# mindspore-lab/minddiffusion

Hardware: AMD Instinct MI355X
Metric: 512x512 txt2img latents/sec (50-step DDIM) (higher is better)
Workload: dtype f16; 1 GPU; SDv2 txt2img 512x512 (64x64 latent), 50-step DDIM, CFG 9.0, batch 1 per GPU (BASELINE.json configs[1]); synthetic seeded weights + synthetic text conditioning; global_batch=1, parallelism=batch-shard x1, hip_graph=True, rccl_world_size=1, broadcast_bytes=0, ddim_steps=50, unet_batch_per_gpu=2, sampler=ddim, cfg_dup_prefix=False

## Files before the change

include/mdx.h:

```cpp
#ifndef MDX_H_
#define MDX_H_

#include <stddef.h>
#include <stdint.h>

#ifdef __cplusplus
extern "C" {
#endif

#define MDX_OK 0
#define MDX_E_INVALID (-1)
#define MDX_E_WORKSPACE (-2)
#define MDX_E_HIP (-3)

typedef void* mdx_stream_t;

int mdx_version(void);
const char* mdx_last_error(void);
int mdx_set_option(const char* name, int value);
int mdx_get_option(const char* name, int* value);

int mdx_nchw_to_nhwc_f16(const float* x, void* y, int B, int C, int H, int W, int Cpad, mdx_stream_t s);
int mdx_nhwc_to_nchw_f32(const void* x, float* y, int B, int C, int H, int W, int Cstride, mdx_stream_t s);

int mdx_srgan_conv_in_f16(const float* x, const void* w, const float* bias, const float* slope, void* out, int B, int H, int W,
                          mdx_stream_t s);
int mdx_srgan_conv_out_f32(const void* x, const void* w, const float* bias, float* out, int B, int H, int W, mdx_stream_t s);

size_t mdx_groupnorm_ws_floats(int B, int HW, int C, int groups);
int mdx_groupnorm_f16(const void* x1, int C1, const void* x2, int C2, const float* gamma, const float* beta,
                      void* y, int B, int HW, int groups, float eps, int silu, float* ws, mdx_stream_t s);

int mdx_groupnorm_colstats_f16(const void* x1, int C1, const float* cs1, int nrb1, const void* x2, int C2, const float* cs2,
                               int nrb2, const float* gamma, const float* beta, const float* scale, const float* shift,
                               int mod_ld, void* y, int B, int HW, int groups, float eps, int silu, mdx_stream_t s);

int mdx_colstats_fold_f32(const float* src, int nrb, float* dst, int nrb2, int B, int C, mdx_stream_t s);

int mdx_groupnorm_scaleshift_f16(const void* x1, int C1, const void* x2, int C2, const float* gamma,
                                 const float* beta, const float* scale, const float* shift, int mod_ld, void* y,
                                 int B, int HW, int groups, float eps, int silu, float* ws, mdx_stream_t s);

int mdx_layernorm_f16(const void* x, const float* gamma, const float* beta, void* y, int rows, int C, float eps,
                      mdx_stream_t s);

typedef struct mdx_gemm_desc {
    const void* a;
    const void* a2;
    int c1, c2;
    const void* w;
    const float* bias;
    const float* rowbias;
    int rowbias_ld;
    const void* residual;
    int residual_ld;
    void* out;
    int out_ld;
    int B, H, W;
    int N;
    int ksize;
    int stride;
    int upsample;
    int epilogue;
    int out_mode;
    int splitk;
    void* workspace;
    size_t workspace_bytes;
    long out_bs;
    void* out2;
    int out2_ld;
    int n_split;
    int asym_pad;
    float* stats_out;
    const float* ln_stats;
    const float* ln_s;
    int ln_nt;
    float ln_eps;
    float* colstats_out;
    int colstats_cap;
    int defer_reduce;
    int tile_m;
    int tile_n;
    const float* gn_colstats;
    const float* gn_gamma;
    const float* gn_beta;
    int gn_nrb;
    int gn_silu;
    float gn_eps;
    const void* skip_a;
    const void* skip_a2;
    int skip_c1, skip_c2;
    const void* skip_w;
    int w_frag;
    int stages;
    const void* w_sub;
    const void* xattn_k;
    const void* xattn_vt;
    int xattn_len;
    int xattn_cap;
    float xattn_scale;
    const float* act_slope;
    int act_slope_n;
} mdx_gemm_desc;

#define MDX_GEMM_WS_HEAD 16384
#define MDX_EPI_NONE 0
#define MDX_EPI_GEGLU 1
#define MDX_EPI_GELU 2
#define MDX_EPI_QUICKGELU 3
#define MDX_EPI_PRELU 4
#define MDX_OUT_ROWMAJOR 0
#define MDX_OUT_TRANSPOSED 1
#define MDX_OUT_D2S2 2

int mdx_gemm_f16(const mdx_gemm_desc* d, mdx_stream_t s);
int mdx_gemm_release_counters(void);
int mdx_gemm_release_workspace(const void* workspace);
int mdx_gemm_bind_counters(const void* workspace, void* counters);
size_t mdx_gemm_workspace_bytes(const mdx_gemm_desc* d);
int mdx_gemm_check(const mdx_gemm_desc* d);
int mdx_gemm_query(const mdx_gemm_desc* d, int* out7);
int mdx_gemm_tune(const mdx_gemm_desc* d, mdx_stream_t s, void* flush, size_t flush_bytes, int reps, int* best4, float* us2);

int mdx_groupnorm_from_splitk_f16(const mdx_gemm_desc* prod, const float* gamma, const float* beta, void* y, int groups,
                                  float eps, int silu, mdx_stream_t s);
int mdx_groupnorm_from_splitk_ok(const mdx_gemm_desc* prod, int groups);

int mdx_attention_f16(const void* q, long q_bs, int q_ld, const void* k, long k_bs, int k_ld, const void* vt,
                      long vt_bs, int vt_ld, void* o, long o_bs, int o_ld, int B, int heads, int D, int Nq, int Nk,
                      float scale, mdx_stream_t s);

size_t mdx_attention_ws_bytes(int B, int heads, int D, int Nq, int Nk);
int mdx_attention_splitkv_f16(const void* q, long q_bs, int q_ld, const void* k, long k_bs, int k_ld, const void* vt,
                              long vt_bs, int vt_ld, void* o, long o_bs, int o_ld, int B, int heads, int D, int Nq, int Nk,
                              float scale, int kv_splits, void* ws, size_t ws_bytes, mdx_stream_t s);

typedef struct mdx_st_tail_desc {
    const void* attn_out;
    const void* tok;
    const void* x_in;
    void* out;
    const void* ctx_k;
    const void* ctx_vt;
    const void* wstream;
    const float* vec;
    float* colstats_out;
    void* debug_out;
    int debug_stage;
    int B, tokens;
    int C, heads, dim_head;
    int ctx_len, ctx_cap;
    float scale;
    float ln_eps;
    int tile_rows;
    int warm;
} mdx_st_tail_desc;
#define MDX_ST_DEBUG_COUNT_BARRIERS 100
int mdx_st_tail_sched_barriers(int C, int tile_rows);
int mdx_st_head_sched_barriers(int C, int tile_rows);
int mdx_st_tail_f16(const mdx_st_tail_desc* d, mdx_stream_t s);
int mdx_st_tail_supported(int C, int heads, int dim_head, int tokens_per_sample, int tile_rows);
size_t mdx_st_tail_stream_bytes(int C);

typedef struct mdx_st_head_desc {
    const void* x;
    const float* colstats;
    int nrb;
    const void* wstream;
    const float* vec;
    void* tok;
    void* qk;
    void* vt;
    int vt_ld;
    void* debug_out;
    int debug_stage;
    int B, tokens, C;
    float gn_eps, ln_eps;
    int tile_rows;
    int warm;
} mdx_st_head_desc;
int mdx_st_head_f16(const mdx_st_head_desc* d, mdx_stream_t s);
int mdx_st_head_supported(int C, int tokens_per_sample, int tile_rows);
size_t mdx_st_head_stream_bytes(int C);

int mdx_timestep_embedding_f32(const float* t, float* out, int M, int dim, float max_period, mdx_stream_t s);

int mdx_dense_small_f32(const float* x, int x_ld, const void* w, const float* b, float* out, int out_ld, int M,
                        int N, int K, int act_in, int act_out, mdx_stream_t s);

int mdx_sampler_step_f32(const float* x, const void* eps_u, const void* eps_c, int eps_ld, float cfg_scale,
                         const float* old1, const float* old2, const float* old3, const float* coef4,
                         float sqrt_at, float sqrt_one_minus_at, float sqrt_a_prev, float dir_coef, float sigma,
                         const float* noise, float* e_t_out, float* x_prev, float* pred_x0, int B, int C, int H,
                         int W, mdx_stream_t s);

int mdx_avgpool2x2_f16(const void* x, void* y, int B, int H, int W, int C, mdx_stream_t s);
int mdx_upsample_nearest2x_f16(const void* x, void* y, int B, int H, int W, int C, mdx_stream_t s);
int mdx_glide_text_embed_f16(const int* tokens, const int* mask, const void* tok_emb, const void* pos,
                             const void* pad, void* out, int B, int T, int width, int n_vocab, mdx_stream_t s);
int mdx_glide_superres_input_f16(const float* x, const float* low, void* out, int B, int S, int s_low,
                                 mdx_stream_t s);
int mdx_glide_step_f32(const float* x, const void* out_c, const void* out_u, int ld, float guidance_scale,
                       const float* coef8, int mode, float noise_scale, const float* noise, float* x_next,
                       float* pred_x0, int B, int H, int W, mdx_stream_t s);

typedef struct mdx_glide_kv_slot {
    const void* src;
    void* dst;
    long src_entry_bytes;
    long dst_batch_bytes;
    long src_pitch, dst_pitch;
    int rows, row_bytes;
} mdx_glide_kv_slot;
int mdx_glide_kv_select_f16(const mdx_glide_kv_slot* slots_dev, int nslots, long entry0, int entry_per_b, int b0, int nb,
                            int blocks_per_copy, mdx_stream_t s);

int mdx_attention_causal_f16(const void* q, long q_bs, int q_ld, const void* k, long k_bs, int k_ld, const void* vt,
                             long vt_bs, int vt_ld, void* o, long o_bs, int o_ld, int B, int heads, int D, int Nq,
                             int Nk, float scale, mdx_stream_t s);

int mdx_pack_b_operand_f16(const void* src, long src_ld, int rows, int K, void* dst, mdx_stream_t s);
int mdx_softmax_rows_f16(void* x, long ld, int rows, int cols, float scale, mdx_stream_t s);

int mdx_vae_gaussian_sample_f32(const void* moments, int ld, const float* noise, float* out, int B, int zc, int HW,
                                mdx_stream_t s);

int mdx_probe_mfma_32x32x16_f16(const void* a, const void* b, float* c, mdx_stream_t s);
int mdx_probe_mfma_16x16x32_f16(const void* a, const void* b, float* c, mdx_stream_t s);
int mdx_probe_dma_stream(const void* src, size_t bytes_per_block, int nblocks, int waves, int per, int ns, int mode,
                         int stride_tiles, float* sink, mdx_stream_t s);

int mdx_probe_l2_stream(const void* src, size_t total_bytes, unsigned bytes_per_wave, int nblocks, int waves, int pf,
                        int shared, float* sink, mdx_stream_t s);

int mdx_probe_gemm_trace(void* buf, size_t bytes);
int mdx_probe_valu_rate(int kind, int iters, int nblocks, float* sink, mdx_stream_t s);
int mdx_probe_mix_rate(int kind, int iters, int nblocks, float* sink, mdx_stream_t s);

#ifdef __cplusplus
}
#endif
#endif
```

minddiffusion_amd/_lib.py:

```python
import ctypes
import os

_HERE = os.path.dirname(os.path.abspath(__file__))
LIB_PATH = os.environ.get("MDX_LIBRARY") or os.path.join(_HERE, "libmdx.so")

c_void_p = ctypes.c_void_p
c_int = ctypes.c_int
c_long = ctypes.c_long
c_float = ctypes.c_float
c_size_t = ctypes.c_size_t


class MdxError(RuntimeError):
    pass


class GemmDesc(ctypes.Structure):
    _fields_ = [
        ("a", c_void_p), ("a2", c_void_p), ("c1", c_int), ("c2", c_int),
        ("w", c_void_p), ("bias", c_void_p), ("rowbias", c_void_p), ("rowbias_ld", c_int),
        ("residual", c_void_p), ("residual_ld", c_int),
        ("out", c_void_p), ("out_ld", c_int),
        ("B", c_int), ("H", c_int), ("W", c_int), ("N", c_int),
        ("ksize", c_int), ("stride", c_int), ("upsample", c_int),
        ("epilogue", c_int), ("out_mode", c_int), ("splitk", c_int),
        ("workspace", c_void_p), ("workspace_bytes", c_size_t),
        ("out_bs", c_long),
        ("out2", c_void_p), ("out2_ld", c_int), ("n_split", c_int), ("asym_pad", c_int),
        ("stats_out", c_void_p), ("ln_stats", c_void_p), ("ln_s", c_void_p), ("ln_nt", c_int), ("ln_eps", c_float),
        ("colstats_out", c_void_p), ("colstats_cap", c_int), ("defer_reduce", c_int),
        ("tile_m", c_int), ("tile_n", c_int),
        ("gn_colstats", c_void_p), ("gn_gamma", c_void_p), ("gn_beta", c_void_p), ("gn_nrb", c_int), ("gn_silu", c_int),
        ("gn_eps", c_float),
        ("skip_a", c_void_p), ("skip_a2", c_void_p), ("skip_c1", c_int), ("skip_c2", c_int), ("skip_w", c_void_p),
        ("w_frag", c_int), ("stages", c_int), ("w_sub", c_void_p),
        ("xattn_k", c_void_p), ("xattn_vt", c_void_p), ("xattn_len", c_int), ("xattn_cap", c_int), ("xattn_scale", c_float),
        ("act_slope", c_void_p), ("act_slope_n", c_int),
    ]


class StTailDesc(ctypes.Structure):
    _fields_ = [
        ("attn_out", c_void_p), ("tok", c_void_p), ("x_in", c_void_p), ("out", c_void_p),
        ("ctx_k", c_void_p), ("ctx_vt", c_void_p), ("wstream", c_void_p), ("vec", c_void_p),
        ("colstats_out", c_void_p), ("debug_out", c_void_p), ("debug_stage", c_int),
        ("B", c_int), ("tokens", c_int), ("C", c_int), ("heads", c_int), ("dim_head", c_int),
        ("ctx_len", c_int), ("ctx_cap", c_int), ("scale", c_float), ("ln_eps", c_float), ("tile_rows", c_int), ("warm", c_int),
    ]


class StHeadDesc(ctypes.Structure):
    _fields_ = [
        ("x", c_void_p), ("colstats", c_void_p), ("nrb", c_int), ("wstream", c_void_p), ("vec", c_void_p),
        ("tok", c_void_p), ("qk", c_void_p), ("vt", c_void_p), ("vt_ld", c_int), ("debug_out", c_void_p), ("debug_stage", c_int),
        ("B", c_int), ("tokens", c_int), ("C", c_int), ("gn_eps", c_float), ("ln_eps", c_float), ("tile_rows", c_int),
        ("warm", c_int),
    ]


EPI_NONE, EPI_GEGLU, EPI_GELU, EPI_QUICKGELU, EPI_PRELU = 0, 1, 2, 3, 4
OUT_ROWMAJOR, OUT_TRANSPOSED, OUT_D2S2 = 0, 1, 2

SIGNATURES = {
    "mdx_version": (c_int, []),
    "mdx_last_error": (ctypes.c_char_p, []),
    "mdx_set_option": (c_int, [ctypes.c_char_p, c_int]),
    "mdx_get_option": (c_int, [ctypes.c_char_p, ctypes.POINTER(c_int)]),
    "mdx_nchw_to_nhwc_f16": (c_int, [c_void_p, c_void_p, c_int, c_int, c_int, c_int, c_int, c_void_p]),
    "mdx_nhwc_to_nchw_f32": (c_int, [c_void_p, c_void_p, c_int, c_int, c_int, c_int, c_int, c_void_p]),
    "mdx_groupnorm_ws_floats": (c_size_t, [c_int, c_int, c_int, c_int]),
    "mdx_groupnorm_f16": (c_int, [c_void_p, c_int, c_void_p, c_int, c_void_p, c_void_p, c_void_p, c_int, c_int,
                                  c_int, c_float, c_int, c_void_p, c_void_p]),
    "mdx_groupnorm_colstats_f16": (c_int, [c_void_p, c_int, c_void_p, c_int, c_void_p, c_int, c_void_p, c_int, c_void_p,
                                           c_void_p, c_void_p, c_void_p, c_int, c_void_p, c_int, c_int, c_int, c_float,
                                           c_int, c_void_p]),
    "mdx_colstats_fold_f32": (c_int, [c_void_p, c_int, c_void_p, c_int, c_int, c_int, c_void_p]),
    "mdx_groupnorm_from_splitk_f16": (c_int, [ctypes.POINTER(GemmDesc), c_void_p, c_void_p, c_void_p, c_int, c_float, c_int,
                                              c_void_p]),
    "mdx_groupnorm_from_splitk_ok": (c_int, [ctypes.POINTER(GemmDesc), c_int]),
    "mdx_groupnorm_scaleshift_f16": (c_int, [c_void_p, c_int, c_void_p, c_int, c_void_p, c_void_p, c_void_p, c_void_p,
                                             c_int, c_void_p, c_int, c_int, c_int, c_float, c_int, c_void_p, c_void_p]),
    "mdx_layernorm_f16": (c_int, [c_void_p, c_void_p, c_void_p, c_void_p, c_int, c_int, c_float, c_void_p]),
    "mdx_gemm_f16": (c_int, [ctypes.POINTER(GemmDesc), c_void_p]),
    "mdx_gemm_workspace_bytes": (c_size_t, [ctypes.POINTER(GemmDesc)]),
    "mdx_gemm_release_workspace": (c_int, [c_void_p]),
    "mdx_gemm_bind_counters": (c_int, [c_void_p, c_void_p]),
    "mdx_st_tail_sched_barriers": (c_int, [c_int, c_int]),
    "mdx_st_head_sched_barriers": (c_int, [c_int, c_int]),
    "mdx_gemm_release_counters": (c_int, []),
    "mdx_gemm_tune": (c_int, [ctypes.POINTER(GemmDesc), c_void_p, c_void_p, c_size_t, c_int, ctypes.POINTER(c_int),
                              ctypes.POINTER(ctypes.c_float)]),
    "mdx_gemm_check": (c_int, [ctypes.POINTER(GemmDesc)]),
    "mdx_gemm_query": (c_int, [ctypes.POINTER(GemmDesc), ctypes.POINTER(c_int)]),
    "mdx_attention_f16": (c_int, [c_void_p, c_long, c_int, c_void_p, c_long, c_int, c_void_p, c_long, c_int,
                                  c_void_p, c_long, c_int, c_int, c_int, c_int, c_int, c_int, c_float, c_void_p]),
    "mdx_attention_ws_bytes": (c_size_t, [c_int, c_int, c_int, c_int, c_int]),
    "mdx_attention_splitkv_f16": (c_int, [c_void_p, c_long, c_int, c_void_p, c_long, c_int, c_void_p, c_long, c_int,
                                          c_void_p, c_long, c_int, c_int, c_int, c_int, c_int, c_int, c_float, c_int, c_void_p,
                                          c_size_t, c_void_p]),
    "mdx_attention_causal_f16": (c_int, [c_void_p, c_long, c_int, c_void_p, c_long, c_int, c_void_p, c_long, c_int,
                                  c_void_p, c_long, c_int, c_int, c_int, c_int, c_int, c_int, c_float, c_void_p]),
    "mdx_st_head_f16": (c_int, [ctypes.POINTER(StHeadDesc), c_void_p]),
    "mdx_st_head_supported": (c_int, [c_int, c_int, c_int]),
    "mdx_st_head_stream_bytes": (c_size_t, [c_int]),
    "mdx_st_tail_f16": (c_int, [ctypes.POINTER(StTailDesc), c_void_p]),
    "mdx_st_tail_supported": (c_int, [c_int, c_int, c_int, c_int, c_int]),
    "mdx_st_tail_stream_bytes": (c_size_t, [c_int]),
    "mdx_timestep_embedding_f32": (c_int, [c_void_p, c_void_p, c_int, c_int, c_float, c_void_p]),
    "mdx_dense_small_f32": (c_int, [c_void_p, c_int, c_void_p, c_void_p, c_void_p, c_int, c_int, c_int, c_int,
                                    c_int, c_int, c_void_p]),
    "mdx_sampler_step_f32": (c_int, [c_void_p, c_void_p, c_void_p, c_int, c_float, c_void_p, c_void_p, c_void_p,
                                     c_void_p, c_float, c_float, c_float, c_float, c_float, c_void_p, c_void_p,
                                     c_void_p, c_void_p, c_int, c_int, c_int, c_int, c_void_p]),
    "mdx_avgpool2x2_f16": (c_int, [c_void_p, c_void_p, c_int, c_int, c_int, c_int, c_void_p]),
    "mdx_upsample_nearest2x_f16": (c_int, [c_void_p, c_void_p, c_int, c_int, c_int, c_int, c_void_p]),
    "mdx_glide_text_embed_f16": (c_int, [c_void_p, c_void_p, c_void_p, c_void_p, c_void_p, c_void_p, c_int, c_int,
                                         c_int, c_int, c_void_p]),
    "mdx_glide_superres_input_f16": (c_int, [c_void_p, c_void_p, c_void_p, c_int, c_int, c_int, c_void_p]),
    "mdx_glide_step_f32": (c_int, [c_void_p, c_void_p, c_void_p, c_int, c_float, c_void_p, c_int, c_float, c_void_p,
                                   c_void_p, c_void_p, c_int, c_int, c_int, c_void_p]),
    "mdx_glide_kv_select_f16": (c_int, [c_void_p, c_int, c_long, c_int, c_int, c_int, c_int, c_void_p]),
    "mdx_pack_b_operand_f16": (c_int, [c_void_p, c_long, c_int, c_int, c_void_p, c_void_p]),
    "mdx_srgan_conv_in_f16": (c_int, [c_void_p, c_void_p, c_void_p, c_void_p, c_void_p, c_int, c_int, c_int, c_void_p]),
    "mdx_srgan_conv_out_f32": (c_int, [c_void_p, c_void_p, c_void_p, c_void_p, c_int, c_int, c_int, c_void_p]),
    "mdx_vae_gaussian_sample_f32": (c_int, [c_void_p, c_int, c_void_p, c_void_p, c_int, c_int, c_int, c_void_p]),
    "mdx_softmax_rows_f16": (c_int, [c_void_p, c_long, c_int, c_int, c_float, c_void_p]),
    "mdx_probe_mfma_32x32x16_f16": (c_int, [c_void_p, c_void_p, c_void_p, c_void_p]),
    "mdx_probe_mfma_16x16x32_f16": (c_int, [c_void_p, c_void_p, c_void_p, c_void_p]),
    "mdx_probe_gemm_trace": (c_int, [c_void_p, c_size_t]),
    "mdx_probe_valu_rate": (c_int, [c_int, c_int, c_int, c_void_p, c_void_p]),
    "mdx_probe_mix_rate": (c_int, [c_int, c_int, c_int, c_void_p, c_void_p]),
    "mdx_probe_l2_stream": (c_int, [c_void_p, c_size_t, ctypes.c_uint, c_int, c_int, c_int, c_int, c_void_p, c_void_p]),
    "mdx_probe_dma_stream": (c_int, [c_void_p, c_size_t, c_int, c_int, c_int, c_int, c_int, c_int, c_void_p, c_void_p]),
}

_lib = None
_ENV_OPTIONS = {
    "MDX_GEMM_TUNED": ("gemm_tuned", int), "MDX_GEMM_BM": ("gemm_bm", int), "MDX_GEMM_BN": ("gemm_bn", int),
    "MDX_GEMM_CFG": ("gemm_ring", lambda v: int(v.split(",")[-1])), "MDX_GEMM_HALO": ("gemm_halo", int),
    "MDX_GEMM_HALO8": ("gemm_halo8", int), "MDX_GEMM_SPLITK_FIXUP_MAX": ("gemm_splitk_fixup_max", int),
    "MDX_GEMM_SPREAD": ("gemm_spread", int), "MDX_HALO_NSB": ("halo_nsb", int), "MDX_GN_MIN_BLOCKS": ("gn_min_blocks", int),
    "MDX_GN_FUSED": ("gn_fused", int), "MDX_GN_COL_CHUNKS": ("gn_col_chunks", int),
    "MDX_GEMM_CONV8P": ("gemm_conv8p", int), "MDX_GEMM_CONV8P_MIN_M": ("gemm_conv8p_min_m", int),
    "MDX_GEMM_SUBPIXEL_MIN_TILES": ("gemm_subpixel_min_tiles", int), "MDX_GEMM_CONV8P_VAR": ("gemm_conv8p_var", int),
    "MDX_ATTN8": ("attn8", int), "MDX_ATTN8_MIN_BLOCKS": ("attn8_min_blocks", int),
    "MDX_GN_WIDE_ROWS": ("gn_wide_rows", int), "MDX_GN_BOOST_MB": ("gn_boost_mb", int), "MDX_ATTN_OCC3": ("attn_occ3", int), "MDX_ATTN_KV_SPLIT": ("attn_kv_split", int),
    "MDX_ATTN_FAST_STAGE": ("attn_fast_stage", int), "MDX_GN_PREFETCH": ("gn_prefetch", int), "MDX_GEMM_LN_PREFETCH": ("gemm_ln_prefetch", int),
    "MDX_GEMM_DENSE_ISSUE": ("gemm_dense_issue", int), "MDX_GEMM_LEAN_DENSE": ("gemm_lean_dense", int),
    "MDX_ATTN_PIPE": ("attn_pipe", int),
}


def load():
    global _lib
    if _lib is not None:
        return _lib
    if not os.path.exists(LIB_PATH):
        raise MdxError(
            f"{LIB_PATH} not found: the HIP extension is required (no CPU fallback). "
            "Build it with `python -c 'import __graft_entry__ as g; g.build()'` or `make -C minddiffusion_amd/csrc`.")
    import torch
    lib = ctypes.CDLL(LIB_PATH)
    for name, (res, args) in SIGNATURES.items():
        fn = getattr(lib, name)
        fn.restype = res
        fn.argtypes = args
    for env, (name, conv) in _ENV_OPTIONS.items():
        if env in os.environ:
            rc = lib.mdx_set_option(name.encode(), conv(os.environ[env]))
            if rc != 0:
                raise MdxError(f"{env}: {lib.mdx_last_error().decode()}")
    _lib = lib
    return lib


def check(rc, what):
    if rc != 0:
        msg = load().mdx_last_error()
        raise MdxError(f"{what} failed (rc={rc}): {msg.decode() if msg else ''}")
```

minddiffusion_amd/csrc/gemm.hip:

```cpp
#include "mdx_common.h"
#include "gemm_internal.h"

#ifndef MDX_HALO_ABLATE
#define MDX_HALO_ABLATE 0
#endif
#ifndef MDX_HALO_LEAN_EPI
#define MDX_HALO_LEAN_EPI 1
#endif
constexpr int HALO_EMODE = MDX_HALO_LEAN_EPI ? 2 : 0;

#include <stdlib.h>

#include <algorithm>
#include <type_traits>
#include <map>
#include <mutex>
#include <utility>
#include <vector>

namespace {


template <int BM, int BN, int BK, int NS, bool SWAP, bool FASTK, int NW, bool GNA = false, bool EXT = false>
__global__ __launch_bounds__(NW * 64, NW == 4 ? 2 : 1) void gemm_kernel(const GemmParams p) {
// ... 674 lines not shown
#pragma unroll
                for (int i = 0; i < TM; ++i) { f16x8 tt; asm volatile("" : "=v"(tt)); af[slot][i] = tt; }
#pragma unroll
                for (int j = 0; j < TN; ++j) { f16x8 tt; asm volatile("" : "=v"(tt)); bf[slot][j] = tt; }
#else
#pragma unroll
                for (int i = 0; i < TM; ++i)
                    af[slot][i] = *reinterpret_cast<const f16x8*>(smem + a_row[i] + (((2 * ks + hi) << 4) ^ a_key[i]));
#pragma unroll
                for (int j = 0; j < TN; ++j)
                    bf[slot][j] = *reinterpret_cast<const f16x8*>(sb + b_row_off + j * 32 * 128 + (((2 * ks + hi) ^ swz_b) << 4));
#endif
            };
            auto mfmas = [&](auto slot_c) {
                constexpr int slot = decltype(slot_c)::value;
#if MDX_HALO_ABLATE == 1
#pragma unroll
                for (int i = 0; i < TM; ++i) { const f16x8 tt = af[slot][i]; asm volatile("" ::"v"(tt)); }
#pragma unroll
                for (int j = 0; j < TN; ++j) { const f16x8 tt = bf[slot][j]; asm volatile("" ::"v"(tt)); }
#else
#pragma unroll
                for (int i = 0; i < TM; ++i)
#pragma unroll
                    for (int j = 0; j < TN; ++j) {
                        if constexpr (SWAP)
                            acc[i][j] = __builtin_amdgcn_mfma_f32_32x32x16_f16(bf[slot][j], af[slot][i], acc[i][j], 0, 0, 0);
                        else
                            acc[i][j] = __builtin_amdgcn_mfma_f32_32x32x16_f16(af[slot][i], bf[slot][j], acc[i][j], 0, 0, 0);
                    }
#endif
            };
            using I0 = std::integral_constant<int, 0>;
            using I1 = std::integral_constant<int, 1>;
            if constexpr (ALLK) {
                using I2 = std::integral_constant<int, 2>;
                using I3 = std::integral_constant<int, 3>;
                rdfrag(I0{}, 0); rdfrag(I1{}, 1); rdfrag(I2{}, 2); rdfrag(I3{}, 3);
                __builtin_amdgcn_sched_barrier(0);
                mfmas(I0{}); mfmas(I1{}); mfmas(I2{}); mfmas(I3{});
            } else {
                rdfrag(I0{}, 0);
                __builtin_amdgcn_sched_barrier(0);
#pragma unroll
                for (int ks = 0; ks < 4; ks += 2) {
                    rdfrag(I1{}, ks + 1);
                    __builtin_amdgcn_sched_barrier(0);
                    mfmas(I0{});
                    __builtin_amdgcn_sched_barrier(0);
                    if (ks + 2 < 4) {
                        rdfrag(I0{}, ks + 2);
                        __builtin_amdgcn_sched_barrier(0);
                    }
                    mfmas(I1{});
                    __builtin_amdgcn_sched_barrier(0);
                }
            }
            rd = (rd + 1 == NSB) ? 0 : rd + 1;
            wr = (wr + 1 == NSB) ? 0 : wr + 1;
        }
    }

    if (p.skip_w) {
        constexpr int SA_BYTES = BM * 128;
        static_assert(2 * SA_BYTES <= 2 * HALO_BYTES && NSB >= 2, "skip tiles reuse the halo / ring areas");
        const __amdgpu_buffer_rsrc_t rs_s1 = make_rsrc(p.skip_a, p.skip_a_bytes);
        const __amdgpu_buffer_rsrc_t rs_s2 = make_rsrc(p.skip_a2 ? p.skip_a2 : p.skip_a, p.skip_a2 ? p.skip_a2_bytes : p.skip_a_bytes);
        const __amdgpu_buffer_rsrc_t rs_sw = make_rsrc(p.skip_w, p.skip_w_bytes);
        const int sk_begin = split * p.skip_kt_per_split, sk_end = min(p.skip_kt, sk_begin + p.skip_kt_per_split);
        constexpr int SAJ = BM / 8 / NW;
        int s_pix[SAJ];
        unsigned s_cb[SAJ];
#pragma unroll
        for (int j = 0; j < SAJ; ++j) {
            const int row = (wave * SAJ + j) * 8 + lrow;
            int pix;
            if constexpr (PW == 16) {
                pix = (pb * p.H + py0 + (row >> 4)) * p.W + px0 + (row & 15);
            } else {
                pix = tile_m * BM + row;
                if (pix >= p.M) pix = -1;
            }
            s_pix[j] = pix;
            s_cb[j] = (unsigned)((lchk ^ ((row >> 1) & 7)) * 16);
        }
        unsigned sb_off[BJ];
        const int skt64 = p.skip_kt;
#pragma unroll
        for (int j = 0; j < BJ; ++j) {
            const int row = (wave * BJ + j) * 8 + lrow;
            const int panel = (n0 >> 6) + (row >> 6);
            sb_off[j] = (unsigned)(((size_t)panel * skt64) * 8192 + ((row & 63) * 8 + lchk) * 16);
        }
        auto stage_skip = [&](int kt, int st) {
            int ci0 = kt * 64;
            const bool second = ci0 >= p.skip_c1;
            const int cs2 = (second ? p.skip_c2 : p.skip_c1) * 2;
            if (second) ci0 -= p.skip_c1;
#pragma unroll
            for (int j = 0; j < SAJ; ++j) {
                const unsigned off = s_pix[j] >= 0 ? (unsigned)(s_pix[j] * cs2) + (unsigned)(ci0 * 2) + s_cb[j] : MDX_OOB;
                void* dst = smem + st * SA_BYTES + (wave * SAJ + j) * 1024;
                if (second)
                    dma16(rs_s2, dst, off);
                else
                    dma16(rs_s1, dst, off);
            }
#pragma unroll
            for (int j = 0; j < BJ; ++j)
                dma16(rs_sw, smem + 2 * HALO_BYTES + st * B_BYTES + (wave * BJ + j) * 1024, sb_off[j] + (unsigned)kt * 8192);
        };
        __syncthreads();
        const int sa_row_off = (wm * WROWS + l31) * 128;
        const int s_swz = (l31 >> 1) & 7;
        if (sk_begin < sk_end) stage_skip(sk_begin, 0);
        for (int kt = sk_begin; kt < sk_end; ++kt) {
            const int st = (kt - sk_begin) & 1;
            asm volatile("s_waitcnt vmcnt(0)" ::: "memory");
            __builtin_amdgcn_s_barrier();
            if (kt + 1 < sk_end) stage_skip(kt + 1, st ^ 1);
            const char* sa = smem + st * SA_BYTES;
            const char* sbk = smem + 2 * HALO_BYTES + st * B_BYTES;
#pragma unroll
            for (int s4 = 0; s4 < 4; ++s4) {
                f16x8 af[TM], bf[TN];
#pragma unroll
                for (int i = 0; i < TM; ++i)
                    af[i] = *reinterpret_cast<const f16x8*>(sa + sa_row_off + i * 32 * 128 + (((2 * s4 + hi) ^ s_swz) << 4));
#pragma unroll
                for (int j = 0; j < TN; ++j)
                    bf[j] = *reinterpret_cast<const f16x8*>(sbk + (b_row_off - 2 * HALO_BYTES) + j * 32 * 128 + (((2 * s4 + hi) ^ swz_b) << 4));
#pragma unroll
                for (int i = 0; i < TM; ++i)
#pragma unroll
                    for (int j = 0; j < TN; ++j) {
                        if constexpr (SWAP)
                            acc[i][j] = __builtin_amdgcn_mfma_f32_32x32x16_f16(bf[j], af[i], acc[i][j], 0, 0, 0);
                        else
                            acc[i][j] = __builtin_amdgcn_mfma_f32_32x32x16_f16(af[i], bf[j], acc[i][j], 0, 0, 0);
                    }
            }
        }
    }

    __syncthreads();
    trace_mark(p, 3);
    if constexpr (PW == 16)
        gemm_epilogue<BM, BN, SWAP, NW, PatchRows, 0, HALO_EMODE>(p, acc, smem, PatchRows{(pb * p.H + py0) * p.W + px0, p.W, pb}, n0, split, bpre,
                                                                  tile_m, tile_id);
    else
        gemm_epilogue<BM, BN, SWAP, NW>(p, acc, smem, LinearRows{tile_m * BM}, n0, split, bpre, tile_m, tile_id);
    trace_mark(p, 4);
    }
}

__device__ __forceinline__ void splitk_sum8(const GemmParams& p, const float* base, const size_t slab, float (&f)[8]) {
    int z = 0;
    for (; z + 4 <= p.nsplit; z += 4) {
        float4 v[4][2];
#pragma unroll
        for (int u = 0; u < 4; ++u) {
            const float4* s = reinterpret_cast<const float4*>(base + (size_t)(z + u) * slab);
            v[u][0] = s[0];
            v[u][1] = s[1];
        }
#pragma unroll
        for (int u = 0; u < 4; ++u) {
            f[0] += v[u][0].x; f[1] += v[u][0].y; f[2] += v[u][0].z; f[3] += v[u][0].w;
            f[4] += v[u][1].x; f[5] += v[u][1].y; f[6] += v[u][1].z; f[7] += v[u][1].w;
        }
    }
    for (; z < p.nsplit; ++z) {
        const float4* s = reinterpret_cast<const float4*>(base + (size_t)z * slab);
        const float4 s0 = s[0], s1 = s[1];
        f[0] += s0.x; f[1] += s0.y; f[2] += s0.z; f[3] += s0.w; f[4] += s1.x; f[5] += s1.y; f[6] += s1.z; f[7] += s1.w;
    }
}

template <bool EXT = false>
__global__ __launch_bounds__(256) void splitk_reduce_kernel(const GemmParams p) {
    mdx_kernarg_touch<sizeof(GemmParams)>();
    const bool geglu = p.epilogue == MDX_EPI_GEGLU;
    const int ncols = geglu ? p.N / 2 : p.N;
    const int cpr = ncols / 8;
    const size_t total = (size_t)p.M * cpr;
    const size_t slab = (size_t)p.M * p.N;
    for (size_t idx = (size_t)blockIdx.x * 256 + threadIdx.x; idx < total; idx += (size_t)gridDim.x * 256) {
        const int m = (int)(idx / cpr);
        const int oc = (int)(idx - (size_t)m * cpr) * 8;
        Row8Extras xtra;
        if (p.out_mode != MDX_OUT_TRANSPOSED) xtra = epilogue_prefetch_row8(p, m, oc);
        const bool ln = p.ln_stats != nullptr;
        float mean = 0.f, rstd = 1.f;
        if (ln) {
            const float2* stp = reinterpret_cast<const float2*>(p.ln_stats) + (size_t)m * p.ln_nt;
            float su = 0.f, sq = 0.f;
            for (int j = threadIdx.x & 7; j < p.ln_nt; j += 8) {
                const float2 v = stp[j];
                su += v.x;
                sq += v.y;
            }
#pragma unroll
            for (int off = 4; off >= 1; off >>= 1) {
                su += __shfl_xor(su, off, 64);
                sq += __shfl_xor(sq, off, 64);
            }
            const float inv = 1.0f / (float)p.K;
            mean = su * inv;
            float var = sq * inv - mean * mean;
            var = var < 0.f ? 0.f : var;
            rstd = rsqrtf(var + p.ln_eps);
        }
        float f[8];
        if (geglu) {
            const int pa = (oc >> 6) * 128 + (oc & 63);
            float a[8], g[8];
#pragma unroll
            for (int e = 0; e < 8; ++e) {
                a[e] = (p.bias && !ln) ? p.bias[pa + e] : 0.f;
                g[e] = (p.bias && !ln) ? p.bias[pa + 64 + e] : 0.f;
            }
            splitk_sum8(p, p.ws + (size_t)m * p.N + pa, slab, a);
            splitk_sum8(p, p.ws + (size_t)m * p.N + pa + 64, slab, g);
            if (ln) {
#pragma unroll
                for (int e = 0; e < 8; ++e) {
                    a[e] = rstd * (a[e] - mean * p.ln_s[pa + e]) + (p.bias ? p.bias[pa + e] : 0.f);
                    g[e] = rstd * (g[e] - mean * p.ln_s[pa + 64 + e]) + (p.bias ? p.bias[pa + 64 + e] : 0.f);
                }
            }
#pragma unroll
            for (int e = 0; e < 8; ++e) f[e] = a[e] * gelu_tanh_f(g[e]);
        } else {
#pragma unroll
            for (int e = 0; e < 8; ++e) f[e] = (p.bias && !ln) ? p.bias[oc + e] : 0.f;
            splitk_sum8(p, p.ws + (size_t)m * p.N + oc, slab, f);
            if (ln) {
#pragma unroll
                for (int e = 0; e < 8; ++e) f[e] = rstd * (f[e] - mean * p.ln_s[oc + e]) + (p.bias ? p.bias[oc + e] : 0.f);
            }
            if (p.epilogue == MDX_EPI_GELU) {
#pragma unroll
                for (int e = 0; e < 8; ++e) f[e] = gelu_tanh_f(f[e]);
            } else if (p.epilogue == MDX_EPI_QUICKGELU) {
#pragma unroll
                for (int e = 0; e < 8; ++e) f[e] = quick_gelu_f(f[e]);
            } else if constexpr (EXT) {
                if (p.epilogue == MDX_EPI_PRELU) {
                    const float* sp = p.act_slope + oc % p.act_slope_n;
#pragma unroll
                    for (int e = 0; e < 8; ++e) f[e] = f[e] > 0.f ? f[e] : sp[e] * f[e];
                }
            }
        }
        if (p.out_mode == MDX_OUT_TRANSPOSED) {
            const int b = m / p.HoWo;
            const int tok = m - b * p.HoWo;
#pragma unroll
            for (int e = 0; e < 8; ++e) p.out[((size_t)b * p.N + oc + e) * p.out_ld + tok] = (f16)f[e];
        } else if (p.n_split && oc >= p.n_split) {
            const int b = m / p.HoWo;
            const int tok = m - b * p.HoWo;
            const int nv = p.N - p.n_split;
#pragma unroll
            for (int e = 0; e < 8; ++e) p.out2[((size_t)b * nv + (oc - p.n_split + e)) * p.out2_ld + tok] = (f16)f[e];
        } else {
            const f16x8 o = epilogue_apply_row8<EXT>(p, f, m, oc, xtra);
            if (p.stats_out) {
                float su = 0.f, sq = 0.f;
#pragma unroll
                for (int e = 0; e < 8; ++e) {
                    const float t = (float)o[e];
                    su += t;
                    sq += t * t;
                }
#pragma unroll
                for (int off = 4; off >= 1; off >>= 1) {
                    su += __shfl_xor(su, off, 64);
                    sq += __shfl_xor(sq, off, 64);
                }
                if ((threadIdx.x & 7) == 0)
                    reinterpret_cast<float2*>(p.stats_out)[(size_t)m * (p.N >> 6) + (oc >> 6)] = make_float2(su, sq);
            }
        }
    }
}

constexpr int CS_ROWS = 64;

__global__ __launch_bounds__(256) void splitk_reduce_colstats_kernel(const GemmParams p) {
    mdx_kernarg_touch<sizeof(GemmParams)>();
    __shared__ float part[32][64][2];
    const int tid = threadIdx.x;
    const int chunk = tid & 7, rl = tid >> 3;
    const int rb = blockIdx.y, n = blockIdx.x * 64 + chunk * 8;
    const size_t slab = (size_t)p.M * p.N;
    float cs[8], cq[8];
#pragma unroll
    for (int e = 0; e < 8; ++e) cs[e] = cq[e] = 0.f;
    if (n < p.N) {
#pragma unroll
        for (int h = 0; h < 2; ++h) {
            const int m = rb * CS_ROWS + rl + 32 * h;
            if (m >= p.M) continue;
            const Row8Extras xtra = epilogue_prefetch_row8(p, m, n);
            float f[8];
// ... 52 lines not shown
    p.bn_hint = d->tile_n;
    p.st_hint = d->stages;
    p.out2_ld = d->out2_ld;
    p.n_split = d->n_split;
    p.ws = (float*)d->workspace;
    p.c1 = d->c1;
    p.c2 = d->c2;
    p.cin = d->c1 + d->c2;
    p.rowbias_ld = d->rowbias_ld;
    p.residual_ld = d->residual_ld;
    p.out_ld = d->out_ld;
    p.out_bs = d->out_bs;
    p.B = d->B;
    p.H = d->H;
    p.W = d->W;
    p.ksize = d->ksize;
    p.stride = d->stride;
    p.upsample = d->upsample ? 1 : 0;
    MDX_REQUIRE(!d->asym_pad || (d->ksize == 3 && d->stride == 2 && !d->upsample),
                "mdx_gemm_f16: asym_pad applies to the 3x3 stride-2 conv only");
    p.pad = d->ksize == 3 ? (d->asym_pad ? 0 : 1) : 0;
    const int pad_hi = d->ksize == 3 ? 1 : 0;
    const int Hs = p.upsample ? 2 * d->H : d->H, Ws = p.upsample ? 2 * d->W : d->W;
    p.Ho = (Hs + p.pad + pad_hi - d->ksize) / d->stride + 1;
    p.Wo = (Ws + p.pad + pad_hi - d->ksize) / d->stride + 1;
    p.HoWo = p.Ho * p.Wo;
    p.M = d->B * p.HoWo;
    p.N = d->N;
    p.K = d->ksize * d->ksize * p.cin;
    p.epilogue = d->epilogue;
    p.out_mode = d->out_mode;
    MDX_REQUIRE(p.epilogue == MDX_EPI_NONE || p.epilogue == MDX_EPI_GEGLU || p.epilogue == MDX_EPI_GELU ||
                    p.epilogue == MDX_EPI_QUICKGELU || p.epilogue == MDX_EPI_PRELU, "mdx_gemm_f16: bad epilogue");
    MDX_REQUIRE(p.out_mode == MDX_OUT_ROWMAJOR || p.out_mode == MDX_OUT_TRANSPOSED || p.out_mode == MDX_OUT_D2S2,
                "mdx_gemm_f16: bad out_mode");
    p.act_slope = d->act_slope;
    p.act_slope_n = d->act_slope_n;
    p.d2s_c = 0;
    if (p.epilogue == MDX_EPI_PRELU) {
        MDX_REQUIRE(p.act_slope && p.act_slope_n > 0 && p.act_slope_n % 8 == 0 && p.N % p.act_slope_n == 0,
                    "mdx_gemm_f16: PReLU needs act_slope and act_slope_n > 0 with act_slope_n %% 8 == 0 and N %% act_slope_n == 0");
        MDX_REQUIRE(p.out_mode != MDX_OUT_TRANSPOSED && !d->rowbias && !d->n_split && !d->xattn_k,
                    "mdx_gemm_f16: PReLU takes a row-major or depth-to-space store with bias (and residual) only");
    }
    if (p.epilogue == MDX_EPI_PRELU || p.out_mode == MDX_OUT_D2S2) {
        MDX_REQUIRE(d->c2 == 0 && d->c1 % 64 == 0 && !d->gn_colstats && !d->skip_w && !d->w_frag && !d->upsample,
                    "mdx_gemm_f16: PReLU / depth-to-space launches take one source with Cin %% 64 == 0 (no fused GroupNorm / skip, "
                    "tile-major weights, no upsample)");
    }
    if (p.out_mode == MDX_OUT_D2S2) {
        MDX_REQUIRE(p.N % 32 == 0 && p.out_ld >= p.N / 4 && (p.epilogue == MDX_EPI_NONE || p.epilogue == MDX_EPI_PRELU),
                    "mdx_gemm_f16: depth-to-space store needs N = 4 C with C %% 8 == 0, out_ld >= C and a plain or PReLU epilogue");
        MDX_REQUIRE(!d->residual && !d->out_bs && !d->n_split && !d->stats_out && !d->colstats_out && !d->ln_stats && !d->xattn_k &&
                        !d->skip_w && !d->defer_reduce,
                    "mdx_gemm_f16: depth-to-space store takes bias / time-embedding row / PReLU only");
        p.d2s_c = p.N / 4;
        p.out_mode = MDX_OUT_ROWMAJOR;
    }
    if (p.epilogue == MDX_EPI_GEGLU) {
        MDX_REQUIRE(p.N % 128 == 0, "mdx_gemm_f16: GEGLU needs N %% 128 == 0");
        MDX_REQUIRE(p.out_mode == MDX_OUT_ROWMAJOR, "mdx_gemm_f16: GEGLU is row-major only");
    }
    if (p.out_mode == MDX_OUT_TRANSPOSED) {
        MDX_REQUIRE(p.out_ld % 8 == 0 && p.out_ld >= p.HoWo, "mdx_gemm_f16: transposed store needs out_ld %% 8 == 0 and out_ld >= tokens");
        MDX_REQUIRE(!p.rowbias && !p.residual, "mdx_gemm_f16: transposed store takes bias only");
    }
    if (p.n_split) {
        MDX_REQUIRE(p.out2 && p.n_split > 0 && p.n_split < p.N && p.n_split % 128 == 0,
                    "mdx_gemm_f16: n_split must be a multiple of 128 inside (0, N) with out2 set");
        MDX_REQUIRE(p.out_mode == MDX_OUT_ROWMAJOR && p.epilogue == MDX_EPI_NONE && !p.rowbias && !p.residual,
                    "mdx_gemm_f16: the split row-major | transposed output takes bias only");
        MDX_REQUIRE(p.out2_ld % 8 == 0 && p.out2_ld >= p.HoWo,
                    "mdx_gemm_f16: transposed part needs out2_ld %% 8 == 0 and out2_ld >= tokens");
    }
    if (p.ln_stats) {
        MDX_REQUIRE(p.ln_s && p.ln_nt * 64 == p.K && p.ksize == 1 && p.c2 == 0 && p.stride == 1 && !p.upsample &&
                        p.out_mode == MDX_OUT_ROWMAJOR && p.N % (p.epilogue == MDX_EPI_GEGLU ? 128 : 64) == 0,
                    "mdx_gemm_f16: LayerNorm fold needs ln_s, ln_nt == K / 64, N %% 64 == 0 and a dense row-major GEMM");
    }
    if (p.stats_out)
        MDX_REQUIRE(p.out_mode == MDX_OUT_ROWMAJOR && p.epilogue != MDX_EPI_GEGLU && !p.n_split && p.N % 64 == 0,
                    "mdx_gemm_f16: row statistics are produced by plain row-major stores with N %% 64 == 0 only");
    if (p.colstats_out)
        MDX_REQUIRE(p.out_mode == MDX_OUT_ROWMAJOR && p.epilogue == MDX_EPI_NONE && !p.n_split && !p.ln_stats && !p.stats_out &&
                        !p.out_bs && p.N % 8 == 0,
                    "mdx_gemm_f16: column statistics come from plain row-major launches only");
    p.gn_cs = d->gn_colstats;
    p.gn_gamma = d->gn_gamma;
    p.gn_beta = d->gn_beta;
    p.gn_nrb = d->gn_nrb;
    p.gn_silu = d->gn_silu ? 1 : 0;
    p.gn_eps = d->gn_eps;
    if (p.gn_cs) {
        MDX_REQUIRE(p.gn_gamma && p.gn_beta && p.gn_nrb > 0, "mdx_gemm_f16: gn_colstats needs gn_gamma, gn_beta and gn_nrb > 0");
        if (p.ksize == 1) {
            MDX_REQUIRE(p.stride == 1 && !p.upsample && p.c2 == 0 && p.cin % 64 == 0 && p.cin <= 2560 && !p.gn_silu &&
                            p.HoWo % 64 == 0,
                        "mdx_gemm_f16: the fused input GroupNorm of a dense launch needs a single source, Cin %% 64 == 0, "
                        "Cin <= 2560, gn_silu = 0 and tokens per sample %% 64 == 0");
        } else {
            MDX_REQUIRE(p.ksize == 3 && p.stride == 1 && !p.upsample && p.c2 == 0 && p.cin % 64 == 0 && p.cin % 32 == 0 &&
                            p.cin <= 640 && !d->w_frag && !(d->H == 8 && d->W == 8),
                        "mdx_gemm_f16: the fused input GroupNorm rides on a single-source 3x3 stride-1 conv with Cin %% 64 == 0, "
                        "Cin <= 640, images larger than 8 x 8 and tile-major weights");
        }
    }
    p.xa_k = (const f16*)d->xattn_k;
    p.xa_vt = (const f16*)d->xattn_vt;
    p.xa_len = d->xattn_len;
    p.xa_cap = d->xattn_cap;
    p.xa_scale_log2 = d->xattn_scale * 1.4426950408889634f;
    if (p.xa_k) {
        const int howo = d->H * d->W;
        MDX_REQUIRE(p.xa_vt && d->xattn_len > 0 && d->xattn_len <= 128 && d->xattn_cap >= d->xattn_len && d->xattn_cap % 8 == 0,
                    "mdx_gemm_f16: cross-attention epilogue needs xattn_vt, 0 < xattn_len <= 128 <= ... xattn_cap (a multiple of 8)");
        MDX_REQUIRE(d->ksize == 1 && d->stride == 1 && !d->upsample && d->c2 == 0 && d->N % 64 == 0 && d->c1 % 64 == 0 &&
                        d->epilogue == MDX_EPI_NONE && d->out_mode == MDX_OUT_ROWMAJOR && !d->residual && !d->rowbias && !d->stats_out &&
                        !d->colstats_out && !d->n_split && !d->out_bs && !d->gn_colstats && !d->defer_reduce,
                    "mdx_gemm_f16: the cross-attention epilogue rides on a plain dense row-major projection (N %% 64 == 0, Cin %% 64 == 0)");
        MDX_REQUIRE(d->tile_n == 64 && d->splitk == 1 && (howo % 128 == 0 || (howo % 64 == 0 && d->tile_m == 64)) &&
                        (d->tile_m == 0 || d->tile_m == 64 || d->tile_m == 128),
                    "mdx_gemm_f16: the cross-attention epilogue needs tile_n = 64 (one head per tile), splitk = 1 and an M tile inside one sample "
                    "(tokens per sample %% 128 == 0, or %% 64 == 0 with tile_m = 64)");
        MDX_REQUIRE((size_t)d->xattn_cap * d->N * 2 <= 0x80000000ull, "mdx_gemm_f16: cross-attention context larger than 2 GiB per sample");
    }
    p.w_sub = (const f16*)d->w_sub;
    p.w_sub_bytes = 0;
    p.c8_sub = 0;
    if (p.w_sub) {
        MDX_REQUIRE(d->upsample && d->ksize == 3 && d->stride == 1, "mdx_gemm_f16: w_sub belongs to the nearest-2x + 3x3 conv (upsample = 1)");
        const size_t sb = (size_t)((4 * (size_t)d->N + 63) / 64) * ((4 * (size_t)(d->c1 + d->c2) + 63) / 64) * 8192;
        MDX_REQUIRE(sb <= 0x80000000ull, "mdx_gemm_f16: sub-pixel weights larger than 2 GiB");
        p.w_sub_bytes = (unsigned)sb;
    }
    p.skip_a = (const f16*)d->skip_a;
    p.skip_a2 = (const f16*)d->skip_a2;
    p.skip_w = (const f16*)d->skip_w;
    p.skip_c1 = d->skip_c1;
    p.skip_c2 = d->skip_c2;
    if (p.skip_w) {
        MDX_REQUIRE(p.skip_a && d->skip_c1 > 0 && d->skip_c1 % 64 == 0 && d->skip_c2 >= 0 && d->skip_c2 % 64 == 0 &&
                        (d->skip_c2 == 0) == (d->skip_a2 == nullptr),
                    "mdx_gemm_f16: fused skip needs skip_a, skip_c1 %% 64 == 0, skip_c2 %% 64 == 0 and skip_a2 iff skip_c2");
        MDX_REQUIRE(p.ksize == 3 && p.stride == 1 && !p.upsample && p.c2 == 0 && p.out_mode == MDX_OUT_ROWMAJOR && !d->w_frag,
                    "mdx_gemm_f16: the fused skip rides on a single-source 3x3 stride-1 row-major conv (tile-major weights)");
        p.skip_kt = (d->skip_c1 + d->skip_c2) / 64;
        const size_t s1 = (size_t)d->B * d->H * d->W * d->skip_c1 * 2, s2 = (size_t)d->B * d->H * d->W * d->skip_c2 * 2;
        const size_t sw = (size_t)((p.N + 63) / 64) * p.skip_kt * 8192;
        MDX_REQUIRE(s1 <= 0x80000000ull && s2 <= 0x80000000ull && sw <= 0x80000000ull, "mdx_gemm_f16: skip operand larger than 2 GiB");
        p.skip_a_bytes = (unsigned)s1;
        p.skip_a2_bytes = (unsigned)s2;
        p.skip_w_bytes = (unsigned)sw;
    }
    if (p.rowbias) MDX_REQUIRE(p.rowbias_ld % 4 == 0, "mdx_gemm_f16: rowbias_ld must be a multiple of 4");
    if (p.residual) MDX_REQUIRE(p.residual_ld % 8 == 0, "mdx_gemm_f16: residual_ld must be a multiple of 8");
    MDX_REQUIRE(p.out_ld % 8 == 0 && p.out_bs % 8 == 0 && p.out_bs >= 0, "mdx_gemm_f16: out_ld / out_bs must be multiples of 8");
    MDX_REQUIRE(!(p.out_bs && p.out_mode == MDX_OUT_TRANSPOSED), "mdx_gemm_f16: out_bs applies to row-major output only");
    const size_t ab = (size_t)d->B * d->H * d->W * d->c1 * 2, a2b = (size_t)d->B * d->H * d->W * d->c2 * 2;
    p.kt64 = (p.K + 63) / 64;
    const size_t wb = (size_t)((p.N + 63) / 64) * p.kt64 * 8192;
    MDX_REQUIRE(ab <= 0x80000000ull && a2b <= 0x80000000ull && wb <= 0x80000000ull,
                "mdx_gemm_f16: operand larger than 2 GiB is not addressable by one buffer descriptor");
    p.a_bytes = (unsigned)ab;
    p.a2_bytes = (unsigned)a2b;
    p.w_bytes = (unsigned)wb;
    return MDX_OK;
}

struct TunedEntry {
    int M, N, K, ksize, bm, bn, ns;
    int var1;
    int st;
};
static const TunedEntry g_tuned[] = {
#include "gemm_tuned.inc"
    {0, 0, 0, 0, 0, 0, 0, 0, 0}};

int tuned_variant(const GemmParams& p) {
    return (p.c2 > 0 ? 1 : 0) | (p.epilogue == MDX_EPI_PRELU ? 2048 : p.epilogue << 1) | (p.n_split ? 8 : 0) | (p.ln_stats ? 16 : 0) |
           (p.stats_out ? 32 : 0) |
           (p.out_mode == MDX_OUT_TRANSPOSED ? 64 : 0) | (p.colstats_out ? 128 : 0) | (p.residual ? 256 : 0) |
           (p.rowbias ? 512 : 0) | (p.d2s_c ? 1024 : 0);
}

bool halo_eligible(const GemmParams& p, int bm);

const TunedEntry* lookup_tuned(const GemmParams& p) {
    const bool use_table = mdx_opt(MDX_OPT_GEMM_TUNED) && !mdx_opt(MDX_OPT_GEMM_BM) && !mdx_opt(MDX_OPT_GEMM_BN);
    if (!use_table || p.bn_hint || p.st_hint || p.stride != 1 || p.upsample) return nullptr;
    if (p.epilogue == MDX_EPI_PRELU || p.d2s_c) return nullptr;
    const int var1 = tuned_variant(p) + 1;
    const TunedEntry* any = nullptr;
    for (const TunedEntry* e = g_tuned; e->M; ++e)
        if (e->M == p.M && e->N == p.N && e->K == p.K && e->ksize == p.ksize) {
            if (e->var1 == var1) {
                any = e;
                break;
            }
            if (e->var1 == 0 && !any) any = e;
        }
    if (!any) return nullptr;
    if (any->bm == 256 && !halo_eligible(p, 256)) return nullptr;
    return (any->bm >= 128 || !halo_eligible(p, 128)) ? any : nullptr;
}

int pick_bn(const GemmParams& p) {
    if (p.epilogue == MDX_EPI_GEGLU) return 128;
    if (p.bn_hint == 64 || p.bn_hint == 128) return p.bn_hint;
    if (const TunedEntry* e = lookup_tuned(p))
        if (e->bn) return e->bn;
    const int optbn = mdx_opt(MDX_OPT_GEMM_BN);
    if (optbn == 64 || optbn == 128) return optbn;
    if (p.N % 128 == 0) return 128;
    if (p.N % 64 == 0 || p.N < 128) return 64;
    return (p.N % 128 > 64) ? 128 : 64;
}

struct GemmCfg {
    int bm, bn, bk, ns;
};

GemmCfg pick_cfg(const GemmParams& p) {
    GemmCfg c;
    c.bm = 128;
    c.bn = pick_bn(p);
    c.bk = 64;
    c.ns = 2;
    const int ring = mdx_opt(MDX_OPT_GEMM_RING);
    if (ring >= 2 && ring <= 5) c.ns = ring;
    return c;
}

bool halo_eligible(const GemmParams& p, int bm);

struct Tiling {
    int bm, ns;
};

Tiling choose_tiling(const GemmParams& p, int bn, int forced_ns, int forced_bm) {
    const int envbm = mdx_opt(MDX_OPT_GEMM_BM);
    if (forced_ns <= 0 && forced_bm <= 0)
        if (const TunedEntry* e = lookup_tuned(p)) return Tiling{e->bm, e->ns};
    const int kt = (p.K + 63) / 64;
    const int chunks = p.cin / 64;
    const double slab_mb = (double)p.M * p.N * 4.0 / 1048576.0;
    const double unique_mb = ((double)p.N * p.K + (double)p.M * p.cin) * 2.0 / 1048576.0;
    Tiling best{128, 1};
    double best_cost = 1e30;
    static const int order[3] = {128, 256, 64};
    for (int oi = 0; oi < 3; ++oi) {
        const int bm = order[oi];
        if (envbm && envbm != bm) continue;
        if (forced_bm > 0 && forced_bm != bm) continue;
        const bool halo = bm >= 128 && halo_eligible(p, bm);
        if (bm == 256 && (!halo || !(envbm || forced_bm == 256))) continue;
        if (bm == 64 && halo_eligible(p, 128) && !envbm && forced_bm <= 0) continue;
        const int tiles = ((p.M + bm - 1) / bm) * ((p.N + bn - 1) / bn);
        const double tau = (halo ? (bm == 256 ? 0.65 : 0.60) : 0.65) * (bm == 64 ? 0.7 : 1.0) * (bn == 64 ? 0.7 : 1.0);
        const int max_ns = forced_ns > 0 ? forced_ns : 16;
        for (int ns = forced_ns > 0 ? forced_ns : 1; ns <= max_ns; ++ns) {
            int kps, eff;
            if (halo) {
                if (ns > chunks && forced_ns <= 0) break;
                const int cps = (chunks + std::min(ns, chunks) - 1) / std::min(ns, chunks);
                kps = cps * 9;
                eff = (chunks + cps - 1) / cps;
            } else {
                if (forced_ns <= 0 && ns > 1 && kt / ns < 4) break;
                kps = (kt + std::min(ns, kt) - 1) / std::min(ns, kt);
                eff = (kt + kps - 1) / kps;
            }
            if (forced_ns <= 0 && eff != ns) continue;
            const int blocks = tiles * eff;
            const double occ = blocks <= 256 ? 1.0 : (bm == 256 ? (blocks + 255) / 256 : 1.15 * ((blocks + 511) / 512));
            const double main_us = std::max(kps * tau * occ, unique_mb / 3.5);
            const double cost = main_us + (eff > 1 ? 3.5 + 0.3 * eff * slab_mb : 0.0);
            if (cost < 0.9 * best_cost) {
                best_cost = cost;
                best = Tiling{bm, ns};
            }
        }
    }
    return best;
}

template <int BM, int BN, int BK, int NS, bool SWAP, bool FASTK, int NW, bool EXT = false>
void launch_one(const GemmParams& p, dim3 grid, hipStream_t st) {
    constexpr size_t ring = (size_t)NS * (BM + BN) * BK * 2;
    constexpr size_t epi = (size_t)(BM > BN ? BM : BN) * ((BM > BN ? BN : BM) + 8) * 2 + 4096;
    constexpr size_t lds = ring > epi ? ring : epi;
    static MdxPerDeviceOnce attr_once;
    if (attr_once.first()) {
        (void)hipFuncSetAttribute(reinterpret_cast<const void*>(&gemm_kernel<BM, BN, BK, NS, SWAP, FASTK, NW, false, EXT>),
                                  hipFuncAttributeMaxDynamicSharedMemorySize, (int)lds);
    }
    hipLaunchKernelGGL((gemm_kernel<BM, BN, BK, NS, SWAP, FASTK, NW, false, EXT>), grid, dim3(NW * 64), lds, st, p);
}

template <int BM, int BN>
void launch_ext(const GemmCfg& c, const GemmParams& p, bool swap, dim3 grid, hipStream_t st) {
    if (c.ns >= 3) {
        if (swap) launch_one<BM, BN, 64, 3, true, true, 4, true>(p, grid, st); else launch_one<BM, BN, 64, 3, false, true, 4, true>(p, grid, st);
    } else {
        if (swap) launch_one<BM, BN, 64, 2, true, true, 4, true>(p, grid, st); else launch_one<BM, BN, 64, 2, false, true, 4, true>(p, grid, st);
    }
}

template <int BM, int BN, int NS, bool SWAP>
void launch_gna_one(const GemmParams& p, dim3 grid, hipStream_t st) {
    constexpr size_t ring = (size_t)NS * (BM + BN) * 64 * 2;
    constexpr size_t epi = (size_t)(BM > BN ? BM : BN) * ((BM > BN ? BN : BM) + 8) * 2 + 4096;
    constexpr size_t lds0 = ring > epi ? ring : epi;
    const size_t lds = lds0 + (size_t)p.cin * 12;
    static MdxPerDeviceOnce attr_once;
    if (attr_once.first()) {
        (void)hipFuncSetAttribute(reinterpret_cast<const void*>(&gemm_kernel<BM, BN, 64, NS, SWAP, true, 4, true>),
                                  hipFuncAttributeMaxDynamicSharedMemorySize, (int)(lds0 + 2560 * 12));
    }
    hipLaunchKernelGGL((gemm_kernel<BM, BN, 64, NS, SWAP, true, 4, true>), grid, dim3(256), lds, st, p);
}

template <int BM, int BN>
void launch_gna(const GemmParams& p, int ns, bool swap, dim3 grid, hipStream_t st) {
    if (ns >= 3) {
        if (swap) launch_gna_one<BM, BN, 3, true>(p, grid, st); else launch_gna_one<BM, BN, 3, false>(p, grid, st);
    } else {
        if (swap) launch_gna_one<BM, BN, 2, true>(p, grid, st); else launch_gna_one<BM, BN, 2, false>(p, grid, st);
    }
}

template <int BM, int BN, int BK, int NS, int NW>
void launch_cfg(const GemmParams& p, bool swap, bool fastk, dim3 grid, hipStream_t st) {
    if (swap) {
        if (fastk)
            launch_one<BM, BN, BK, NS, true, true, NW>(p, grid, st);
        else
            launch_one<BM, BN, BK, NS, true, false, NW>(p, grid, st);
    } else {
        if (fastk)
            launch_one<BM, BN, BK, NS, false, true, NW>(p, grid, st);
        else
            launch_one<BM, BN, BK, NS, false, false, NW>(p, grid, st);
    }
}

template <int BM, int BN>
bool launch_bn(const GemmCfg& c, const GemmParams& p, bool swap, bool fastk, dim3 grid, hipStream_t st, bool nw8 = false) {
    if constexpr (BM == 128) {
        if (nw8 && c.bk == 64 && (c.ns == 2 || c.ns == 3)) {
            if (c.ns == 2) launch_cfg<128, BN, 64, 2, 8>(p, swap, fastk, grid, st); else launch_cfg<128, BN, 64, 3, 8>(p, swap, fastk, grid, st);
            return true;
        }
    }
    if (c.bk == 64 && c.ns == 2) launch_cfg<BM, BN, 64, 2, 4>(p, swap, fastk, grid, st);
    else if (c.bk == 64 && c.ns == 3) launch_cfg<BM, BN, 64, 3, 4>(p, swap, fastk, grid, st);
    else if (BM == 128 && c.bk == 64 && c.ns == 4) launch_cfg<128, BN, 64, 4, 4>(p, swap, fastk, grid, st);
    else if (BM == 128 && c.bk == 64 && c.ns == 5) launch_cfg<128, BN, 64, 5, 4>(p, swap, fastk, grid, st);
    else if (BM == 64 && c.bk == 64 && c.ns == 4) launch_cfg<64, BN, 64, 4, 4>(p, swap, fastk, grid, st);
    else if (BM == 64 && c.bk == 64 && c.ns == 5) launch_cfg<64, BN, 64, 5, 4>(p, swap, fastk, grid, st);
    else if (BM == 64 && c.bk == 64 && c.ns == 6) launch_cfg<64, BN, 64, 6, 4>(p, swap, fastk, grid, st);
    else return false;
    return true;
}

template <int BM, int BN, int NSB, bool SWAP, int PW = 16, bool BDIR = false, bool W4 = false>
void launch_halo(const GemmParams& p, dim3 grid, hipStream_t st) {
    constexpr size_t hinst = ((PW == 16 ? (BM / 16 + 2) * 18 : (BM / 64) * 100) + 7) / 8;
    constexpr size_t ring = 2 * hinst * 1024 + (BDIR ? 0 : (size_t)NSB * BN * 128);
    constexpr size_t epi = (size_t)BM * (BN + 8) * 2 + 4096;
    constexpr size_t lds0 = ring > epi ? ring : epi;
    constexpr size_t gn_tab_max = (BDIR || PW != 16) ? 0 : 640 * 8;
    const size_t lds = lds0 + (p.gn_cs ? (size_t)p.cin * 8 : 0);
    static MdxPerDeviceOnce attr_once;
    if (attr_once.first()) {
        (void)hipFuncSetAttribute(reinterpret_cast<const void*>(&conv3x3_halo_kernel<BM, BN, NSB, SWAP, PW, BDIR, W4>),
                                  hipFuncAttributeMaxDynamicSharedMemorySize, (int)(lds0 + gn_tab_max));
    }
    hipLaunchKernelGGL((conv3x3_halo_kernel<BM, BN, NSB, SWAP, PW, BDIR, W4>), grid, dim3(BM * 2), lds, st, p);
}

template <int BN, int PW>
void launch_halo_bdir(const GemmParams& p, bool swap, dim3 grid, hipStream_t st) {
    if (swap) launch_halo<128, BN, 2, true, PW, true>(p, grid, st); else launch_halo<128, BN, 2, false, PW, true>(p, grid, st);
}
template <int PW>
void launch_halo_bdir_w4(const GemmParams& p, dim3 grid, hipStream_t st) {
    launch_halo<128, 128, 2, false, PW, true, true>(p, grid, st);
}

template <int BM, int BN, int PW = 16>
void launch_halo_cfg(const GemmParams& p, int nsb, bool swap, dim3 grid, hipStream_t st) {
    if (nsb == 4) {
        if (swap) launch_halo<BM, BN, 4, true, PW>(p, grid, st); else launch_halo<BM, BN, 4, false, PW>(p, grid, st);
    } else if (nsb == 3) {
        if (swap) launch_halo<BM, BN, 3, true, PW>(p, grid, st); else launch_halo<BM, BN, 3, false, PW>(p, grid, st);
    } else {
        if (swap) launch_halo<BM, BN, 2, true, PW>(p, grid, st); else launch_halo<BM, BN, 2, false, PW>(p, grid, st);
    }
}

bool halo8_eligible(const GemmParams& p) {
    if (!mdx_opt(MDX_OPT_GEMM_HALO8)) return false;
    return p.H == 8 && p.W == 8;
}

static bool halo_epilogue_ok(const GemmParams& p) {
    if (p.epilogue == MDX_EPI_PRELU || p.d2s_c) return false;
    if (HALO_EMODE == 0) return true;
    return p.epilogue == MDX_EPI_NONE || p.epilogue == MDX_EPI_GEGLU;
}

bool halo_eligible(const GemmParams& p, int bm) {
    if (!mdx_opt(MDX_OPT_GEMM_HALO)) return false;
    if (!halo_epilogue_ok(p)) return false;
    if (!(p.ksize == 3 && p.stride == 1 && !p.upsample && p.c2 == 0 && p.cin % 64 == 0 && p.out_mode == MDX_OUT_ROWMAJOR))
        return false;
    if (p.out_bs) return false;
    if (p.residual && (size_t)p.M * (size_t)p.residual_ld * 2 >= 0x80000000ull) return false;
    if (bm == 128 && halo8_eligible(p)) return true;
    return p.H % (bm / 16) == 0 && p.W % 16 == 0;
}

}

static unsigned long long* g_gemm_trace = nullptr;
static size_t g_gemm_trace_slots = 0;

extern "C" int mdx_probe_gemm_trace(void* buf, size_t bytes) {
    g_gemm_trace = (unsigned long long*)buf;
    g_gemm_trace_slots = buf ? bytes / 64 : 0;
    return MDX_OK;
}

static bool conv8p_wanted(const mdx_gemm_desc* d, const GemmParams& p);

static bool fixup_eligible(const mdx_gemm_desc* d, const GemmParams& p, int bm, int bn, int ns) {
    const int max_ns = mdx_opt(MDX_OPT_GEMM_SPLITK_FIXUP_MAX);
    if (ns > max_ns) return false;
    if (p.out_mode != MDX_OUT_ROWMAJOR || d->defer_reduce) return false;
    const long tiles = (long)((p.M + bm - 1) / bm) * ((p.N + bn - 1) / bn);
    return tiles <= MDX_TICKET_SLOTS;
}

static size_t split_bytes(const mdx_gemm_desc* d, const GemmParams& p, int bm, int bn, int ns, size_t* head) {
    if (fixup_eligible(d, p, bm, bn, ns)) {
        *head = (size_t)MDX_TICKET_SLOTS * sizeof(unsigned);
        return (size_t)((p.M + bm - 1) / bm) * ((p.N + bn - 1) / bn) * bm * bn * sizeof(float);
    }
    *head = (size_t)MDX_TICKET_SLOTS * sizeof(unsigned);
    return (size_t)p.M * p.N * sizeof(float);
}

extern "C" size_t mdx_gemm_workspace_bytes(const mdx_gemm_desc* d) {
    GemmParams p{};
    if (fill_params(d, p) != MDX_OK) return 0;
    if (conv8p_wanted(d, p)) return mdx_conv8p_plan(p, mdx_conv8p_pick_bn(p, d->tile_n), 0, false, true);
    const GemmCfg c = pick_cfg(p);
    const Tiling tl = choose_tiling(p, c.bn, d->splitk, d->tile_m);
    if (tl.ns <= 1) return 0;
    size_t head;
    const size_t per = std::max(split_bytes(d, p, tl.bm, c.bn, 2, &head), split_bytes(d, p, tl.bm, c.bn, 1 << 30, &head));
    return head + (size_t)tl.ns * per;
}

static int mdx_internal_resolve_check(const mdx_gemm_desc* d, GemmParams& p);

extern "C" int mdx_gemm_check(const mdx_gemm_desc* d) {
    GemmParams p{};
    int rc = fill_params(d, p);
    if (rc != MDX_OK) return rc;
    const bool fastk = (p.cin % 64 == 0) && (p.c2 == 0 || p.c1 % 64 == 0);
    MDX_REQUIRE(fastk || p.c2 == 0, "mdx_gemm_f16: two-source input needs c1 %% 64 == 0 and Cin %% 64 == 0");
    return mdx_internal_resolve_check(d, p);
}

struct Resolved {
    GemmCfg c;
    int bn, ns;
    int stages;
    bool halo, tuned;
    bool fixup;
    bool c8;
};

struct TicketPools {
    std::mutex mu;
    std::map<std::pair<int, const void*>, unsigned*> slot;
    std::map<std::pair<int, const void*>, bool> caller_owned;
    struct Dev { char* next = nullptr; int left = 0; hipStream_t zero_stream = nullptr; std::vector<unsigned*> free_slots; };
    std::map<int, Dev> dev;
    std::vector<std::pair<int, void*>> chunks;
};
static TicketPools g_tickets;
constexpr int TICKET_CHUNK_SLOTS = 64;

static int ticket_device_of(const void* ws) {
    hipPointerAttribute_t at;
    if (ws && hipPointerGetAttributes(&at, ws) == hipSuccess) return at.device;
    (void)hipGetLastError();
    int dv = 0;
    (void)hipGetDevice(&dv);
    return dv;
}

static int ticket_slot(const void* ws, unsigned** out) {
    const int dv = ticket_device_of(ws);
    std::lock_guard<std::mutex> lk(g_tickets.mu);
    const auto key = std::make_pair(dv, ws);
    const auto it = g_tickets.slot.find(key);
    if (it != g_tickets.slot.end()) {
        *out = it->second;
        return MDX_OK;
    }
    TicketPools::Dev& d = g_tickets.dev[dv];
    if (!d.free_slots.empty()) {
        unsigned* s = d.free_slots.back();
        d.free_slots.pop_back();
        g_tickets.slot.emplace(key, s);
        *out = s;
        return MDX_OK;
    }
    if (d.left == 0) {
        const size_t bytes = (size_t)TICKET_CHUNK_SLOTS * MDX_GEMM_WS_HEAD;
        int cur = 0;
        (void)hipGetDevice(&cur);
        if (cur != dv) (void)hipSetDevice(dv);
        hipStreamCaptureMode mode = hipStreamCaptureModeRelaxed;
        (void)hipThreadExchangeStreamCaptureMode(&mode);
        void* mem = nullptr;
        hipError_t e = hipMalloc(&mem, bytes);
        if (e == hipSuccess && !d.zero_stream) e = hipStreamCreateWithFlags(&d.zero_stream, hipStreamNonBlocking);
        if (e == hipSuccess) e = hipMemsetAsync(mem, 0, bytes, d.zero_stream);
        if (e == hipSuccess) e = hipStreamSynchronize(d.zero_stream);
        (void)hipThreadExchangeStreamCaptureMode(&mode);
        if (cur != dv) (void)hipSetDevice(cur);
        if (e != hipSuccess) {
            if (mem) (void)hipFree(mem);
            mdx_set_error("mdx_gemm_f16: allocating the split-K arrival counters failed: %s", hipGetErrorString(e));
            return MDX_E_HIP;
        }
        g_tickets.chunks.emplace_back(dv, mem);
        d.next = static_cast<char*>(mem);
        d.left = TICKET_CHUNK_SLOTS;
    }
    unsigned* s = reinterpret_cast<unsigned*>(d.next);
    d.next += MDX_GEMM_WS_HEAD;
    d.left -= 1;
    g_tickets.slot.emplace(key, s);
    *out = s;
    return MDX_OK;
}

extern "C" int mdx_gemm_bind_counters(const void* workspace, void* counters) {
    MDX_REQUIRE(workspace && counters && ((uintptr_t)counters % 16) == 0,
                "mdx_gemm_bind_counters: workspace and a 16-byte aligned counters buffer of MDX_GEMM_WS_HEAD zeroed bytes are required");
    const int dv = ticket_device_of(workspace);
    MDX_REQUIRE(ticket_device_of(counters) == dv, "mdx_gemm_bind_counters: the counters must live on the workspace's device");
    std::lock_guard<std::mutex> lk(g_tickets.mu);
    const auto key = std::make_pair(dv, workspace);
    const auto it = g_tickets.slot.find(key);
    if (it != g_tickets.slot.end()) {
        if (it->second == counters) return MDX_OK;
        if (!g_tickets.caller_owned.count(key)) g_tickets.dev[dv].free_slots.push_back(it->second);
        g_tickets.slot.erase(it);
    }
    g_tickets.slot.emplace(key, static_cast<unsigned*>(counters));
    g_tickets.caller_owned[key] = true;
    return MDX_OK;
}

extern "C" int mdx_gemm_release_workspace(const void* workspace) {
    std::lock_guard<std::mutex> lk(g_tickets.mu);
    int n = 0;
    for (auto it = g_tickets.slot.begin(); it != g_tickets.slot.end();) {
        if (it->first.second == workspace) {
            const auto own = g_tickets.caller_owned.find(it->first);
            if (own != g_tickets.caller_owned.end())
                g_tickets.caller_owned.erase(own);
            else
                g_tickets.dev[it->first.first].free_slots.push_back(it->second);
            it = g_tickets.slot.erase(it);
            ++n;
        } else {
            ++it;
        }
    }
    return n;
}

extern "C" int mdx_gemm_release_counters(void) {
    std::lock_guard<std::mutex> lk(g_tickets.mu);
    int dv = 0;
    (void)hipGetDevice(&dv);
    for (auto& c : g_tickets.chunks) {
        (void)hipSetDevice(c.first);
        (void)hipFree(c.second);
    }
    for (auto& d : g_tickets.dev)
        if (d.second.zero_stream) {
            (void)hipSetDevice(d.first);
            (void)hipStreamDestroy(d.second.zero_stream);
        }
    (void)hipSetDevice(dv);
    g_tickets.chunks.clear();
    g_tickets.slot.clear();
    g_tickets.caller_owned.clear();
    g_tickets.dev.clear();
    return MDX_OK;
}

static bool conv8p_wanted(const mdx_gemm_desc* d, const GemmParams& p) {
    if (d->w_frag || d->defer_reduce || d->splitk > 1 || d->asym_pad) return false;
    if (mdx_opt(MDX_OPT_GEMM_BM) || !mdx_opt(MDX_OPT_GEMM_HALO)) return false;
    if (!mdx_conv8p_eligible(p)) return false;
    if (d->tile_m == 256 && (d->stages == 8 || d->stages == 9)) return true;
    if (!mdx_opt(MDX_OPT_GEMM_CONV8P)) return false;
    if (d->tile_m != 0 || d->stages != 0) return false;
    if (d->tile_n != 0 && d->tile_n != 64 && d->tile_n != 96 && d->tile_n != 128 && d->tile_n != 160 && d->tile_n != 192) return false;
    if (p.upsample) return mdx_conv8p_tiles(p) >= mdx_opt(MDX_OPT_GEMM_SUBPIXEL_MIN_TILES);
    return p.M >= mdx_opt(MDX_OPT_GEMM_CONV8P_MIN_M) && mdx_conv8p_tiles(p) >= 128;
}

static int resolve_launch(const mdx_gemm_desc* d, GemmParams& p, Resolved& r) {
    r.c8 = false;
    if (conv8p_wanted(d, p)) {
        r.c = GemmCfg{256, mdx_conv8p_pick_bn(p, d->tile_n), 64, 3};
        r.bn = r.c.bn;
        r.ns = 1;
        r.stages = 8;
        r.halo = true;
        r.tuned = false;
        r.fixup = false;
        r.c8 = true;
        p.bk = 64;
        p.ktiles = (p.K + 63) / 64;
        p.ktiles_per_split = p.ktiles;
        p.skip_kt_per_split = p.skip_w ? p.skip_kt : 0;
        p.tickets = nullptr;
        (void)mdx_conv8p_plan(p, r.bn, d->workspace_bytes, d->workspace != nullptr, false);
        return MDX_OK;
    }
    r.c = pick_cfg(p);
    const int bn = r.bn = r.c.bn;
    p.bk = r.c.bk;
    p.ktiles = (p.K + r.c.bk - 1) / r.c.bk;
    r.tuned = d->splitk <= 0 && d->tile_m <= 0 && lookup_tuned(p) != nullptr;
    r.stages = p.st_hint;
    if (r.tuned) r.stages = lookup_tuned(p)->st;
    const Tiling tl = choose_tiling(p, bn, d->splitk, d->tile_m);
    r.c.bm = tl.bm;
    int ns = tl.ns;
    if (ns > p.ktiles) ns = p.ktiles;
    if (ns > 1) {
        size_t head;
        const size_t slab = std::max(split_bytes(d, p, tl.bm, bn, 2, &head), split_bytes(d, p, tl.bm, bn, 1 << 30, &head));
        const size_t cap = (d->workspace && d->workspace_bytes > head) ? (d->workspace_bytes - head) / slab : 0;
        if ((size_t)ns > cap) ns = (int)cap;
        if (ns < 1) ns = 1;
        if (d->splitk > 1 && ns != d->splitk) {
            mdx_set_error("mdx_gemm_f16: workspace too small for splitk=%d (need %zu bytes)", d->splitk,
                          head + (size_t)d->splitk * slab);
            return MDX_E_WORKSPACE;
        }
    }
    r.halo = r.c.bm >= 128 && halo_eligible(p, r.c.bm);
    if (r.c.bm == 256 && !r.halo) {
        mdx_set_error("mdx_gemm_f16: tile_m = 256 needs a launch the 16 x 16-patch HALO conv applies to (3x3, stride 1, H %% 16 == 0, "
                      "W %% 16 == 0, Cin %% 64 == 0)");
        return MDX_E_INVALID;
    }
    if (p.gn_cs && p.ksize == 1) {
        if (p.HoWo % r.c.bm != 0) {
            mdx_set_error("mdx_gemm_f16: the fused input GroupNorm of a dense launch needs tokens per sample (%d) %% tile_m (%d) == 0",
                          p.HoWo, r.c.bm);
            return MDX_E_INVALID;
        }
    } else if (p.gn_cs && !(r.halo && r.bn == 64 && !halo8_eligible(p))) {
        mdx_set_error("mdx_gemm_f16: the fused input GroupNorm needs a launch that resolves to the HALO 3x3 kernel with 64-column "
                      "tiles (ask mdx_gemm_query first)");
        return MDX_E_INVALID;
    }
    if (p.skip_w && !r.halo) {
        mdx_set_error("mdx_gemm_f16: the fused skip needs a launch that resolves to the HALO 3x3 kernel (ask mdx_gemm_query first)");
        return MDX_E_INVALID;
    }
    p.nsplit = ns;
    if (r.halo) {
        const int chunks = p.cin / 64;
        if (ns > chunks) ns = chunks;
        const int cps = (chunks + ns - 1) / ns;
        p.ktiles_per_split = cps * 9;
    } else {
        p.ktiles_per_split = (p.ktiles + ns - 1) / ns;
    }
    p.nsplit = (p.ktiles + p.ktiles_per_split - 1) / p.ktiles_per_split;
    r.ns = p.nsplit;
    p.skip_kt_per_split = p.skip_w ? (p.skip_kt + p.nsplit - 1) / p.nsplit : 0;
    r.fixup = r.ns > 1 && fixup_eligible(d, p, r.c.bm, bn, r.ns);
    p.tickets = r.fixup ? reinterpret_cast<unsigned*>(p.ws) : nullptr;
    if (r.ns > 1 && !r.fixup) p.ws += MDX_TICKET_SLOTS;
    return MDX_OK;
}

static int mdx_internal_resolve_check(const mdx_gemm_desc* d, GemmParams& p) {
    Resolved r;
    return resolve_launch(d, p, r);
}

static int colstats_rows(const GemmParams& p, const Resolved& r) {
    if (p.out_mode != MDX_OUT_ROWMAJOR || p.epilogue != MDX_EPI_NONE || p.n_split || p.ln_stats || p.stats_out || p.out_bs ||
        p.d2s_c)
        return 0;
    if (r.ns > 1 && !r.fixup) return p.HoWo % CS_ROWS == 0 ? CS_ROWS : 0;
    if (r.halo) return halo8_eligible(p) && r.c.bm == 128 ? 0 : r.c.bm;
    return p.HoWo % r.c.bm == 0 ? r.c.bm : 0;
}

static bool lean_dense_eligible(const GemmParams& p, bool swap, bool fastk, bool nw8, int ntiles) {
    if (!mdx_opt(MDX_OPT_GEMM_LEAN_DENSE) || !p.dense_issue) return false;
    if (!(p.ksize == 1 && p.stride == 1 && !p.upsample && p.c2 == 0 && fastk && swap && !nw8)) return false;
    if (p.gn_cs || p.rowbias || p.out_bs || p.skip_w || p.d2s_c) return false;
    if (p.epilogue != MDX_EPI_NONE && p.epilogue != MDX_EPI_GEGLU) return false;
    if ((size_t)p.M * (size_t)(p.residual ? p.residual_ld : 0) * 2 >= 0x80000000ull) return false;
    if (p.ln_stats && (size_t)p.M * (size_t)p.ln_nt * 8 >= 0x80000000ull) return false;
    return ntiles < 65536 && p.tiles_m < 65536 && p.tiles_n < 65536;
}

struct LaunchGeom {
    dim3 grid;
    int ntiles, ring, st_req;
    bool fastk, nw8, swap, lean;
};

static bool lean_dense_has(int bm, int bn, int ring) {
    if (ring < 2) return false;
    if (bm == 64) return ring <= 6;
    if (bm == 128 && bn == 64) return ring <= 4;
    return bm == 128 && bn == 128 && ring <= 3;
}

static int launch_geometry(GemmParams& p, const Resolved& rs, LaunchGeom& g) {
    const GemmCfg& c = rs.c;
    const int bn = rs.bn, ns = rs.ns;
    p.tiles_m = (p.M + c.bm - 1) / c.bm;
    p.tiles_n = (p.N + bn - 1) / bn;
    g.fastk = (p.cin % 64 == 0) && (p.c2 == 0 || p.c1 % 64 == 0);
    MDX_REQUIRE(g.fastk || p.c2 == 0, "mdx_gemm_f16: two-source input needs c1 %% 64 == 0 and Cin %% 64 == 0");
    g.ntiles = p.tiles_m * p.tiles_n;
    p.tiles_per_xcd = (g.ntiles + 7) / 8;
    p.inv_tiles_n = p.tiles_n > 1 ? (unsigned)((0x100000000ull + (unsigned)p.tiles_n - 1) / (unsigned)p.tiles_n) : 0u;
    p.inv_tiles_m = p.tiles_m > 1 ? (unsigned)((0x100000000ull + (unsigned)p.tiles_m - 1) / (unsigned)p.tiles_m) : 0u;
    p.res_bytes = p.residual ? (unsigned)std::min<size_t>((size_t)p.M * (size_t)p.residual_ld * 2, 0x7fffffffull) : 0u;
    p.n_fastest = ((size_t)p.M * p.cin >= (size_t)p.N * p.K) ? 1 : 0;
    g.grid = dim3(8 * p.tiles_per_xcd, ns);
    p.spread = (p.tiles_m == 1 && mdx_opt(MDX_OPT_GEMM_SPREAD)) ? 1 : 0;
    if (p.spread) g.grid = dim3(g.ntiles * ns, 1);
    g.ring = c.ns;
    g.nw8 = rs.stages >= 10;
    g.st_req = g.nw8 ? rs.stages - 8 : rs.stages;
    if (!(mdx_opt(MDX_OPT_GEMM_RING) >= 2 && mdx_opt(MDX_OPT_GEMM_RING) <= 5)) {
        g.ring = (g.ntiles * ns <= 256 || c.bm + bn <= 192) ? 3 : 2;
        if (g.st_req >= 2 && g.st_req <= 6) g.ring = g.st_req;
    }
    g.swap = (ns == 1 || rs.fixup) && (p.out_mode == MDX_OUT_ROWMAJOR);
    g.lean = !rs.halo && lean_dense_eligible(p, g.swap, g.fastk, g.nw8, g.ntiles) && lean_dense_has(c.bm, bn, g.ring);
    return MDX_OK;
}

extern "C" int mdx_gemm_query(const mdx_gemm_desc* d, int* out7) {
    GemmParams p{};
    int rc = fill_params(d, p);
    if (rc != MDX_OK) return rc;
    MDX_REQUIRE(out7, "mdx_gemm_query: null output");
    Resolved r;
    rc = resolve_launch(d, p, r);
    if (rc != MDX_OK) return rc;
    out7[0] = r.c.bm;
    out7[1] = r.bn;
    out7[2] = r.ns;
    int form = r.halo ? 1 : 0;
    if (!r.c8 && !r.halo) {
        LaunchGeom lg;
        rc = launch_geometry(p, r, lg);
        if (rc != MDX_OK) return rc;
        if (lg.lean) form = 2;
    }
    out7[3] = form;
    out7[4] = r.tuned ? 1 : 0;
    out7[5] = colstats_rows(p, r);
    out7[6] = r.fixup ? 1 : 0;
    return MDX_OK;
}

int mdx_internal_split_info(const mdx_gemm_desc* d, MdxSplitInfo* info) {
    GemmParams p{};
    int rc = fill_params(d, p);
    if (rc != MDX_OK) return rc;
    Resolved r;
    rc = resolve_launch(d, p, r);
    if (rc != MDX_OK) return rc;
    MDX_REQUIRE(p.out_mode == MDX_OUT_ROWMAJOR && p.epilogue == MDX_EPI_NONE && !p.n_split && !p.ln_stats && !p.stats_out &&
                    !p.out_bs && !p.colstats_out && p.out_ld == p.N && p.N % 8 == 0,
                "deferred split-K reduce: plain dense row-major producers only");
    info->ws = p.ws;
    info->nsplit = r.ns;
    info->M = p.M;
    info->N = p.N;
    info->HoWo = p.HoWo;
    info->B = p.B;
    info->bias = p.bias;
    info->rowbias = p.rowbias;
    info->rowbias_ld = p.rowbias_ld;
    info->residual = p.residual;
    info->residual_ld = p.residual_ld;
    info->out = p.out;
    return MDX_OK;
}

extern "C" int mdx_gemm_f16(const mdx_gemm_desc* d, mdx_stream_t s) {
    GemmParams p{};
    int rc = fill_params(d, p);
    if (rc != MDX_OK) return rc;
    hipStream_t st = (hipStream_t)s;
    Resolved rs;
    rc = resolve_launch(d, p, rs);
    if (rc != MDX_OK) return rc;
    GemmCfg c = rs.c;
    const int bn = rs.bn;
    int ns = rs.ns;
    const bool halo = rs.halo;
    if (p.colstats_out) {
        const int rows = colstats_rows(p, rs);
        MDX_REQUIRE(rows > 0, "mdx_gemm_f16: this launch cannot produce column statistics (ask mdx_gemm_query first)");
        MDX_REQUIRE((p.M + rows - 1) / rows <= d->colstats_cap,
                    "mdx_gemm_f16: colstats_out holds %d row blocks, this launch writes %d (%d rows each)", d->colstats_cap,
                    (p.M + rows - 1) / rows, rows);
    }
    if (rs.c8) {
        if (p.c8_split > 1) {
            MDX_REQUIRE((uintptr_t)p.ws % 16 == 0, "mdx_gemm_f16: workspace must be 16-byte aligned");
            const int trc = ticket_slot(d->workspace, &p.tickets);
            if (trc != MDX_OK) return trc;
        }
        rc = mdx_conv8p_launch(p, bn, st);
        if (rc != MDX_OK) return rc;
        MDX_LAUNCH_CHECK("mdx_gemm_f16(conv8p)");
        return MDX_OK;
    }
    MDX_REQUIRE(!d->defer_reduce || ns > 1, "mdx_gemm_f16: defer_reduce set but the launch does not split K");
    MDX_REQUIRE(!rs.fixup || ((uintptr_t)p.ws % 16 == 0), "mdx_gemm_f16: workspace must be 16-byte aligned");
    if (rs.fixup) {
        const int trc = ticket_slot(d->workspace, &p.tickets);
        if (trc != MDX_OK) return trc;
    }
    LaunchGeom lg;
    rc = launch_geometry(p, rs, lg);
    if (rc != MDX_OK) return rc;
    const bool fastk = lg.fastk, nw8 = lg.nw8, swap = lg.swap;
    const int ntiles = lg.ntiles;
    MDX_REQUIRE(!p.xa_k || (lg.lean && !halo && bn == 64 && ns == 1 && (p.HoWo % c.bm) == 0),
                "mdx_gemm_f16: the cross-attention epilogue needs the lean dense kernel on %d x 64 tiles inside one sample (got tile %d x %d, %d splits)",
                c.bm, c.bm, bn, ns);
    dim3 grid = lg.grid;
    p.trace = (g_gemm_trace && (size_t)grid.x * grid.y <= g_gemm_trace_slots) ? g_gemm_trace : nullptr;
    GemmCfg cc = c;
    cc.ns = lg.ring;
    const int st_req = lg.st_req;
    MDX_REQUIRE(!d->w_frag || halo, "mdx_gemm_f16: fragment-major weights (w_frag) are read by the HALO 3x3 conv only");
    bool ok;
    if (halo) {
        int nsb = (c.bm == 256 || bn == 64) ? 3 : 2;
        if (st_req >= 2 && st_req <= 4) nsb = st_req;
        if (mdx_opt(MDX_OPT_HALO_NSB) >= 2 && mdx_opt(MDX_OPT_HALO_NSB) <= 4) nsb = mdx_opt(MDX_OPT_HALO_NSB);
        if (d->w_frag) {
            MDX_REQUIRE(c.bm == 128, "mdx_gemm_f16: fragment-major weights run on 128-row HALO tiles only (got tile_m %d)", c.bm);
            const bool w4 = bn == 128 && ns > 1 && !rs.fixup && !swap;
            if (halo8_eligible(p)) {
                if (w4) launch_halo_bdir_w4<8>(p, grid, st);
                else if (bn == 128) launch_halo_bdir<128, 8>(p, swap, grid, st); else launch_halo_bdir<64, 8>(p, swap, grid, st);
            } else {
                if (w4) launch_halo_bdir_w4<16>(p, grid, st);
                else if (bn == 128) launch_halo_bdir<128, 16>(p, swap, grid, st); else launch_halo_bdir<64, 16>(p, swap, grid, st);
            }
        } else if (c.bm == 256) {
            if (bn == 128) launch_halo_cfg<256, 128>(p, nsb, swap, grid, st); else launch_halo_cfg<256, 64>(p, nsb, swap, grid, st);
        } else if (halo8_eligible(p)) {
            if (bn == 128) launch_halo_cfg<128, 128, 8>(p, nsb, swap, grid, st); else launch_halo_cfg<128, 64, 8>(p, nsb, swap, grid, st);
        } else {
            if (bn == 128) launch_halo_cfg<128, 128>(p, nsb, swap, grid, st); else launch_halo_cfg<128, 64>(p, nsb, swap, grid, st);
        }
        ok = true;
    } else if (p.gn_cs) {
        MDX_REQUIRE(fastk, "mdx_gemm_f16: the fused input GroupNorm needs Cin %% 64 == 0");
        const int gns = cc.ns >= 3 ? 3 : 2;
        if (cc.bm == 64) {
            if (bn == 128) launch_gna<64, 128>(p, gns, swap, grid, st); else launch_gna<64, 64>(p, gns, swap, grid, st);
        } else {
            if (bn == 128) launch_gna<128, 128>(p, gns, swap, grid, st); else launch_gna<128, 64>(p, gns, swap, grid, st);
        }
        ok = true;
    } else if (p.epilogue == MDX_EPI_PRELU || p.d2s_c) {
        if (cc.bm == 64) {
            if (bn == 128) launch_ext<64, 128>(cc, p, swap, grid, st); else launch_ext<64, 64>(cc, p, swap, grid, st);
        } else {
            if (bn == 128) launch_ext<128, 128>(cc, p, swap, grid, st); else launch_ext<128, 64>(cc, p, swap, grid, st);
        }
        ok = true;
    } else if (lg.lean && mdx_dense_launch(p, cc.bm, bn, cc.ns, grid, st)) {
        ok = true;
    } else if (cc.bm == 64)
        ok = (bn == 128) ? launch_bn<64, 128>(cc, p, swap, fastk, grid, st) : launch_bn<64, 64>(cc, p, swap, fastk, grid, st);
    else
        ok = (bn == 128) ? launch_bn<128, 128>(cc, p, swap, fastk, grid, st, nw8) : launch_bn<128, 64>(cc, p, swap, fastk, grid, st, nw8);
    MDX_REQUIRE(ok, "mdx_gemm_f16: unsupported tile configuration bk=%d ns=%d", c.bk, c.ns);
    MDX_LAUNCH_CHECK("mdx_gemm_f16");
    if (ns > 1 && !d->defer_reduce && !rs.fixup) {
        const int ncols = p.epilogue == MDX_EPI_GEGLU ? p.N / 2 : p.N;
        const size_t total = (size_t)p.M * (ncols / 8);
        int blocks = (int)((total + 255) / 256);
        if (blocks > 2048) blocks = 2048;
        if (p.colstats_out)
            hipLaunchKernelGGL(splitk_reduce_colstats_kernel, dim3((p.N + 63) / 64, (p.M + CS_ROWS - 1) / CS_ROWS), dim3(256), 0,
                               st, p);
        else if (p.epilogue == MDX_EPI_PRELU || p.d2s_c)
            hipLaunchKernelGGL(splitk_reduce_kernel<true>, dim3(blocks), dim3(256), 0, st, p);
        else
            hipLaunchKernelGGL(splitk_reduce_kernel<false>, dim3(blocks), dim3(256), 0, st, p);
        MDX_LAUNCH_CHECK("mdx_gemm_f16(splitk reduce)");
    }
    return MDX_OK;
}

extern "C" int mdx_gemm_tune(const mdx_gemm_desc* d, mdx_stream_t s, void* flush, size_t flush_bytes, int reps, int* best4,
                             float* us2) {
    MDX_REQUIRE(d != nullptr && best4 != nullptr, "mdx_gemm_tune: null argument");
    MDX_REQUIRE(!d->defer_reduce && !d->colstats_out && !d->w_frag,
                "mdx_gemm_tune: descriptors whose consumer depends on the launch form (colstats_out, defer_reduce) or whose weights "
                "are packed for one form (w_frag) keep the library's choice");
    hipStream_t st = reinterpret_cast<hipStream_t>(s);
    if (reps < 1) reps = 5;
    if (reps > 31) reps = 31;
    hipEvent_t e0 = nullptr, e1 = nullptr;
    if (hipEventCreate(&e0) != hipSuccess || hipEventCreate(&e1) != hipSuccess) {
        if (e0) (void)hipEventDestroy(e0);
        mdx_set_error("mdx_gemm_tune: hipEventCreate failed");
        return MDX_E_HIP;
    }
    auto measure = [&](const mdx_gemm_desc& c, float* us) -> int {
        int rc = mdx_gemm_f16(&c, st);
        if (rc != MDX_OK) return rc;
        float t[32];
        for (int r = 0; r < reps; ++r) {
            if (flush && flush_bytes) (void)hipMemsetAsync(flush, r & 1, flush_bytes, st);
            (void)hipEventRecord(e0, st);
            rc = mdx_gemm_f16(&c, st);
            (void)hipEventRecord(e1, st);
            if (rc != MDX_OK) return rc;
            if (hipEventSynchronize(e1) != hipSuccess) {
                mdx_set_error("mdx_gemm_tune: a trial launch failed on the device");
                return MDX_E_HIP;
            }
            float ms = 0.f;
            (void)hipEventElapsedTime(&ms, e0, e1);
            t[r] = ms * 1e3f;
        }
        std::sort(t, t + reps);
        *us = t[reps / 2];
        return MDX_OK;
    };
    mdx_gemm_desc base = *d;
    base.tile_m = base.tile_n = base.splitk = base.stages = 0;
    int q0[7];
    int rc = mdx_gemm_query(&base, q0);
    float t_auto = 0.f;
    if (rc == MDX_OK) rc = measure(base, &t_auto);
    if (rc != MDX_OK) {
        (void)hipEventDestroy(e0);
        (void)hipEventDestroy(e1);
        return rc;
    }
    float t_best = t_auto;
    int best[4] = {0, 0, 0, 0};
    std::vector<long> seen;
    auto form = [](const int* q) { return (long)q[0] | ((long)q[1] << 10) | ((long)q[2] << 20) | ((long)q[3] << 30) | ((long)q[6] << 31); };
    seen.push_back(form(q0));
    static const int BMS[] = {64, 128, 256}, BNS[] = {64, 128}, NSS[] = {1, 2, 3, 4, 6, 8, 12, 16, 20};
    for (int bm : BMS)
        for (int bn : BNS)
            for (int ns : NSS) {
                mdx_gemm_desc c = base;
                c.tile_m = bm;
                c.tile_n = bn;
                c.splitk = ns;
                int q[7];
                if (mdx_gemm_query(&c, q) != MDX_OK) continue;
                if (q[0] != bm || q[1] != bn || q[2] != ns) continue;
                const long f = form(q);
                if (std::find(seen.begin(), seen.end(), f) != seen.end()) continue;
                seen.push_back(f);
                float t = 0.f;
                if (measure(c, &t) != MDX_OK) continue;
                if (t < t_best) {
                    t_best = t;
                    best[0] = bm, best[1] = bn, best[2] = ns, best[3] = 0;
                }
            }
    (void)hipEventDestroy(e0);
    (void)hipEventDestroy(e1);
    if (!(t_best < t_auto * 0.98f)) {
        best[0] = best[1] = best[2] = best[3] = 0;
        t_best = t_auto;
    }
    for (int i = 0; i < 4; ++i) best4[i] = best[i];
    if (us2) us2[0] = t_auto, us2[1] = t_best;
    return MDX_OK;
}
```

minddiffusion_amd/csrc/gemm_internal.h:

```cpp
#pragma once
#include "mdx_common.h"

namespace mdx_int {

struct GemmParams {
    const f16* a;
    const f16* a2;
    const f16* w;
    const float* bias;
    const float* rowbias;
    const f16* residual;
    f16* out;
    f16* out2;
    float* ws;
    unsigned* tickets;
    int c1, c2, cin;
    int rowbias_ld, residual_ld, out_ld, out2_ld, n_split;
    float* stats_out;
    float* colstats_out;
    const float* ln_stats;
    const float* ln_s;
    int ln_nt;
    int bn_hint;
    int st_hint;
    int spread;
    float ln_eps;
    long out_bs;
    int B, H, W, Ho, Wo, HoWo, M, N, K;
    int ksize, stride, upsample, pad;
    int epilogue, out_mode;
    int ktiles, ktiles_per_split, nsplit;
    int tiles_m, tiles_n, tiles_per_xcd, n_fastest;
    int kt64;
    unsigned a_bytes, a2_bytes, w_bytes;
    int bk;
    unsigned long long* trace;
    const float* gn_cs;
    const float* gn_gamma;
    const float* gn_beta;
    int gn_nrb, gn_silu;
    float gn_eps;
    const f16* skip_a;
    const f16* skip_a2;
    const f16* skip_w;
    int skip_c1, skip_c2, skip_kt, skip_kt_per_split;
    unsigned skip_a_bytes, skip_a2_bytes, skip_w_bytes;
    int c8_full, c8_rem, c8_split, c8_cps;
    const f16* w_sub;
    unsigned w_sub_bytes;
    int c8_sub;
    int dense_issue;
    int ln_prefetch;
    unsigned inv_tiles_n, inv_tiles_m;
    unsigned res_bytes;
    const f16* xa_k;
    const f16* xa_vt;
    int xa_len, xa_cap;
    float xa_scale_log2;
    const float* act_slope;
    int act_slope_n;
    int d2s_c;
};

}
using mdx_int::GemmParams;

bool mdx_dense_launch(const GemmParams& p, int bm, int bn, int ns, dim3 grid, hipStream_t st);
bool mdx_conv8p_eligible(const GemmParams& p);
int mdx_conv8p_pick_bn(const GemmParams& p, int bn_hint);
int mdx_conv8p_tiles(const GemmParams& p);
size_t mdx_conv8p_plan(GemmParams& p, int bn, size_t workspace_bytes, bool have_workspace, bool query_only);
int mdx_conv8p_launch(const GemmParams& p, int bn, hipStream_t st);

namespace {


__device__ __forceinline__ f16x4 cvt4(float a, float b, float c, float d) {
    f16x4 v;
    v[0] = (f16)a;
    v[1] = (f16)b;
    v[2] = (f16)c;
    v[3] = (f16)d;
    return v;
}

struct Row8Extras {
    float4 r0, r1;
    f16x8 res;
};

__device__ __forceinline__ Row8Extras epilogue_prefetch_row8(const GemmParams& p, int m, int n) {
    Row8Extras x;
    if (p.rowbias) {
        const int b = m / p.HoWo;
        const float4* rb = reinterpret_cast<const float4*>(p.rowbias + (size_t)b * p.rowbias_ld + n);
        x.r0 = rb[0];
        x.r1 = rb[1];
    }
    if (p.residual) x.res = *reinterpret_cast<const f16x8*>(p.residual + (size_t)m * p.residual_ld + n);
    return x;
}

template <bool EXT = false>
__device__ __forceinline__ f16x8 epilogue_apply_row8(const GemmParams& p, float (&f)[8], int m, int n, const Row8Extras& x) {
    if (p.rowbias) {
        f[0] += x.r0.x; f[1] += x.r0.y; f[2] += x.r0.z; f[3] += x.r0.w;
        f[4] += x.r1.x; f[5] += x.r1.y; f[6] += x.r1.z; f[7] += x.r1.w;
    }
    if (p.residual) {
#pragma unroll
        for (int e = 0; e < 8; ++e) f[e] += (float)x.res[e];
    }
    f16x8 o;
#pragma unroll
    for (int e = 0; e < 8; ++e) o[e] = (f16)f[e];
    size_t row = (size_t)m * p.out_ld;
    if (p.out_bs) {
        const int b = m / p.HoWo;
        row = (size_t)b * p.out_bs + (size_t)(m - b * p.HoWo) * p.out_ld;
    } else if constexpr (EXT) {
        if (p.d2s_c) {
            const int b = m / p.HoWo;
            const int r = m - b * p.HoWo;
            const int y = r / p.Wo, x = r - (r / p.Wo) * p.Wo;
            const int q = n / p.d2s_c;
            n -= q * p.d2s_c;
            row = (((size_t)b * 2 * p.Ho + 2 * y + (q >> 1)) * (size_t)(2 * p.Wo) + 2 * x + (q & 1)) * p.out_ld;
        }
    }
    *reinterpret_cast<f16x8*>(p.out + row + n) = o;
    return o;
}

__device__ __forceinline__ void epilogue_store_row8(const GemmParams& p, float (&f)[8], int m, int n) {
    const Row8Extras x = epilogue_prefetch_row8(p, m, n);
    epilogue_apply_row8(p, f, m, n, x);
}

__device__ __forceinline__ void trace_mark(const GemmParams& p, int slot) {
#ifdef MDX_GEMM_TRACE
    if (p.trace && threadIdx.x == 0)
        p.trace[((size_t)blockIdx.y * gridDim.x + blockIdx.x) * 8 + slot] = __builtin_amdgcn_s_memrealtime();
#endif
}

struct LinearRows {
    int m0;
    __device__ __forceinline__ int operator()(int row) const { return m0 + row; }
    __device__ __forceinline__ int sample() const { return 0; }
};
struct PatchRows {
    int base, W;
    int b;
    __device__ __forceinline__ int operator()(int row) const { return base + (row >> 4) * W + (row & 15); }
    __device__ __forceinline__ int sample() const { return b; }
};

template <int BN, bool SWAP, int NW>
__device__ __forceinline__ void gemm_bias_prefetch(const GemmParams& p, const int n0, float (&bpre)[16]) {
#pragma unroll
    for (int e = 0; e < 16; ++e) bpre[e] = 0.f;
    if constexpr (SWAP) {
        if (!p.bias) return;
        const int tid = threadIdx.x;
        const bool geglu = p.epilogue == MDX_EPI_GEGLU;
        const int n = n0 + (geglu ? (tid & 7) : (tid % (BN / 8))) * 8;
        if (n >= p.N) return;
        const float4* b4 = reinterpret_cast<const float4*>(p.bias + n);
        const float4 x0 = b4[0], x1 = b4[1];
        bpre[0] = x0.x; bpre[1] = x0.y; bpre[2] = x0.z; bpre[3] = x0.w;
        bpre[4] = x1.x; bpre[5] = x1.y; bpre[6] = x1.z; bpre[7] = x1.w;
        if (geglu) {
            const float4 g0 = b4[16], g1 = b4[17];
            bpre[8] = g0.x; bpre[9] = g0.y; bpre[10] = g0.z; bpre[11] = g0.w;
            bpre[12] = g1.x; bpre[13] = g1.y; bpre[14] = g1.z; bpre[15] = g1.w;
        }
    }
}

__device__ __forceinline__ void gemm_ln_row_fold(const GemmParams& p, const int m, float (&mr)[2]) {
    float su = 0.f, sq = 0.f;
    if (m < p.M) {
        const float2* st = reinterpret_cast<const float2*>(p.ln_stats) + (size_t)m * p.ln_nt;
        int j = 0;
        for (; j + 8 <= p.ln_nt; j += 8) {
            float2 v[8];
#pragma unroll
            for (int u = 0; u < 8; ++u) v[u] = st[j + u];
#pragma unroll
            for (int u = 0; u < 8; ++u) {
                su += v[u].x;
                sq += v[u].y;
            }
        }
        for (; j + 2 <= p.ln_nt; j += 2) {
            const float2 v0 = st[j], v1 = st[j + 1];
            su += v0.x; sq += v0.y; su += v1.x; sq += v1.y;
        }
        for (; j < p.ln_nt; ++j) {
            const float2 v = st[j];
            su += v.x;
            sq += v.y;
        }
    }
    const float inv = 1.0f / (float)p.K;
    const float mean = su * inv;
    float var = sq * inv - mean * mean;
    var = var < 0.f ? 0.f : var;
    mr[0] = mean;
    mr[1] = rsqrtf(var + p.ln_eps);
}

constexpr int MDX_TICKET_SLOTS = MDX_GEMM_WS_HEAD / 4;
typedef unsigned u32x4 __attribute__((ext_vector_type(4)));
// ... 513 lines not shown
```

minddiffusion_amd/ldm/modules/diffusionmodules/openaimodel.py:

```python
import ctypes
import math

import os
import weakref

import numpy as np
import torch

from .... import ops
from ...._lib import MdxError
from ....weights import check_state_dict

f16, f32 = torch.float16, torch.float32


def _round_up(x, m):
    return (x + m - 1) // m * m


class _Arena:

    def __init__(self, device):
        self.device = device
        self.free = {}
# ... 178 lines not shown
                    for n in ("norm1", "norm2", "norm3"):
                        s[t + n + ".gamma"] = (inner,)
                        s[t + n + ".beta"] = (inner,)
            elif kind == "down" and self.conv_resample:
                s[pre + "op.conv.weight"] = (layer[1], layer[1], 3, 3)
                s[pre + "op.conv.bias"] = (layer[1],)
            elif kind == "up" and self.conv_resample:
                s[pre + "conv.conv.weight"] = (layer[1], layer[1], 3, 3)
                s[pre + "conv.conv.bias"] = (layer[1],)
        s["out.0.gamma"] = (mc,)
        s["out.0.beta"] = (mc,)
        s["out.2.conv.weight"] = (self.out_channels, mc, 3, 3)
        s["out.2.conv.bias"] = (self.out_channels,)
        if self.n_embed is not None:
            s["id_predictor.0.gamma"] = (mc,)
            s["id_predictor.0.beta"] = (mc,)
            s["id_predictor.1.conv.weight"] = (self.n_embed, mc, 1, 1)
            s["id_predictor.1.conv.bias"] = (self.n_embed,)
        return s

    def _dev(self, a, dtype):
        t = a if isinstance(a, torch.Tensor) else torch.from_numpy(np.ascontiguousarray(a))
        return t.to(device=self.device, dtype=dtype).contiguous()

    def _pack_conv(self, wt, cin_pad=None, cout_pad=None):
        wt = wt if isinstance(wt, torch.Tensor) else torch.from_numpy(np.ascontiguousarray(wt))
        return ops.pack_conv_weight(wt.to(self.device), cin_pad, cout_pad)

    def _pack_dense(self, wt):
        return ops.pack_gemm_weight(self._dev(wt, f16))

    def _pad_vec(self, v, n):
        v = self._dev(v, f32)
        if v.numel() == n:
            return v
        out = torch.zeros(n, dtype=f32, device=self.device)
        out[: v.numel()] = v
        return out

    def load_state_dict(self, params, strict=True):
        shapes = self.parameter_shapes()
        check_state_dict(shapes, {k: v for k, v in params.items() if strict or k in shapes}, True, "UNetModel.load_state_dict")
        P = params
        w = {}
        w["te0.w"] = self._dev(P["time_embed.0.weight"], f16)
        w["te0.b"] = self._dev(P["time_embed.0.bias"], f32)
        w["te2.w"] = self._dev(P["time_embed.2.weight"], f16)
        w["te2.b"] = self._dev(P["time_embed.2.bias"], f32)
        if self.num_classes is not None:
            w["label_emb"] = self._dev(P["label_emb.embedding_table"], f32)
        emb_w, emb_b, self._emb_off = [], [], {}
        off = 0
        for pre, layer in self._named_layers():
            kind = layer[0]
            if kind == "conv":
                w[pre + "w"] = self._pack_conv(P[pre + "conv.weight"], cin_pad=self.cin_pad)
                w[pre + "b"] = self._dev(P[pre + "conv.bias"], f32)
            elif kind in ("res", "resdown", "resup"):
                cin, cout = layer[1], layer[2]
                for n in ("in_layers_norm", "out_layers_norm"):
                    w[pre + n + ".g"] = self._dev(P[pre + n + ".gamma"], f32)
                    w[pre + n + ".b"] = self._dev(P[pre + n + ".beta"], f32)
                w[pre + "conv1.w"] = self._pack_conv(P[pre + "in_layers_conv.conv.weight"])
                w[pre + "conv1.b"] = self._dev(P[pre + "in_layers_conv.conv.bias"], f32)
                w[pre + "conv2.w"] = self._pack_conv(P[pre + "out_layers_conv.conv.weight"])
                w[pre + "conv2.b"] = self._dev(P[pre + "out_layers_conv.conv.bias"], f32)
                if cin != cout:
                    w[pre + "skip.w"] = self._pack_conv(P[pre + "skip_connection.conv.weight"])
                    w[pre + "skip.b"] = self._dev(P[pre + "skip_connection.conv.bias"], f32)
                emb_w.append(self._dev(P[pre + "emb_layers.1.weight"], f16))
                emb_b.append(self._dev(P[pre + "emb_layers.1.bias"], f32))
                self._emb_off[pre] = off
                off += cout * (2 if self.use_scale_shift_norm else 1)
            elif kind == "st":
                inner = layer[2] * layer[3]
                w[pre + "norm.g"] = self._dev(P[pre + "norm.gamma"], f32)
                w[pre + "norm.b"] = self._dev(P[pre + "norm.beta"], f32)
                for n in ("proj_in", "proj_out"):
                    wt = self._dev(P[pre + n + ".weight"], f16)
                    w[pre + n + ".w"] = self._pack_dense(wt.reshape(wt.shape[0], wt.shape[1]))
                    w[pre + n + ".b"] = self._dev(P[pre + n + ".bias"], f32)
                for k in range(self.transformer_depth):
                    t = pre + f"transformer_blocks.{k}."
                    wq, wk, wv = (self._dev(P[t + f"attn1.to_{n}.weight"], f16) for n in "qkv")
                    for n in ("norm1", "norm2", "norm3"):
                        w[t + n + ".g"] = self._dev(P[t + n + ".gamma"], f32)
                        w[t + n + ".b"] = self._dev(P[t + n + ".beta"], f32)
                    fold = inner % 64 == 0 and os.environ.get("MDX_UNET_LN_FOLD", "1") != "0"

                    def put(name, wt, norm, bias=None):
                        if fold:
                            wt, w[name + ".s"], w[name + ".cb"] = ops.fold_layernorm(wt, w[t + norm + ".g"], w[t + norm + ".b"], bias)
                        w[name + ".w"] = self._pack_dense(wt)
                    if (2 * wq.shape[0]) % 128 == 0 and os.environ.get("MDX_UNET_QKV_MERGE", "1") != "0":
                        put(t + "attn1.qkv", torch.cat([wq, wk, wv], 0), "norm1")
                    else:
                        w[t + "attn1.qk.w"] = self._pack_dense(torch.cat([wq, wk], 0))
                        w[t + "attn1.v.w"] = self._pack_dense(wv)
                    put(t + "attn2.q", self._dev(P[t + "attn2.to_q.weight"], f16), "norm2")
                    w[t + "attn2.k.w"] = self._pack_dense(P[t + "attn2.to_k.weight"])
                    w[t + "attn2.v.w"] = self._pack_dense(P[t + "attn2.to_v.weight"])
                    for a in ("attn1", "attn2"):
                        w[t + a + ".o.w"] = self._pack_dense(P[t + a + ".to_out.0.weight"])
                        w[t + a + ".o.b"] = self._dev(P[t + a + ".to_out.0.bias"], f32)
                    gw = self._dev(P[t + "ff.net.0.proj.weight"], f16)
                    gb = self._dev(P[t + "ff.net.0.proj.bias"], f32)
                    half = 4 * inner
                    assert half % 64 == 0
                    nt = half // 64
                    w[t + "ff1.b"] = torch.stack([gb[:half].reshape(nt, 64), gb[half:].reshape(nt, 64)], 1).reshape(-1).contiguous()
                    put(t + "ff1", torch.stack([gw[:half].reshape(nt, 64, inner), gw[half:].reshape(nt, 64, inner)], 1)
                        .reshape(2 * half, inner), "norm3", w[t + "ff1.b"])
                    w[t + "ff2.w"] = self._pack_dense(P[t + "ff.net.2.weight"])
                    w[t + "ff2.b"] = self._dev(P[t + "ff.net.2.bias"], f32)
                    if (self.transformer_depth == 1 and inner == layer[1]
                            and ops.st_tail_supported(inner, layer[2], layer[3], 64, 64)):
                        po = self._dev(P[pre + "proj_out.weight"], f16)
                        w[t + "tail.stream"], w[t + "tail.vec"] = ops.pack_st_tail(
                            self._dev(P[t + "attn1.to_out.0.weight"], f16), self._dev(P[t + "attn2.to_q.weight"], f16),
                            self._dev(P[t + "attn2.to_out.0.weight"], f16), gw, self._dev(P[t + "ff.net.2.weight"], f16),
                            po.reshape(po.shape[0], po.shape[1]),
                            w[t + "attn1.o.b"], w[t + "norm2.g"], w[t + "norm2.b"], w[t + "attn2.o.b"], w[t + "norm3.g"],
                            w[t + "norm3.b"], gb, w[t + "ff2.b"], w[pre + "proj_out.b"])
                        if ops.st_head_supported(inner, 64, 64):
                            pi = self._dev(P[pre + "proj_in.weight"], f16)
                            w[t + "head.stream"], w[t + "head.vec"] = ops.pack_st_head(
                                pi.reshape(pi.shape[0], pi.shape[1]), wq, wk, wv, w[pre + "norm.g"], w[pre + "norm.b"],
                                w[pre + "proj_in.b"], w[t + "norm1.g"], w[t + "norm1.b"])
            elif kind == "down" and self.conv_resample:
                w[pre + "w"] = self._pack_conv(P[pre + "op.conv.weight"])
                w[pre + "b"] = self._dev(P[pre + "op.conv.bias"], f32)
            elif kind == "up" and self.conv_resample:
                w[pre + "w"] = self._pack_conv(P[pre + "conv.conv.weight"])
                w[pre + "b"] = self._dev(P[pre + "conv.conv.bias"], f32)
                if layer[1] % 64 == 0 and ops.get_option("unet_subpixel_upsample"):
                    wt = P[pre + "conv.conv.weight"]
                    wt = wt if isinstance(wt, torch.Tensor) else torch.from_numpy(np.ascontiguousarray(wt))
                    w[pre + "wsub"] = ops.pack_subpixel_conv_weight(wt.to(self.device))
        w["emb.w"] = torch.cat(emb_w, 0).contiguous()
        w["emb.b"] = torch.cat(emb_b, 0).contiguous()
        self._emb_total = off
        if self.n_embed is None:
            w["out.g"] = self._dev(P["out.0.gamma"], f32)
            w["out.b"] = self._dev(P["out.0.beta"], f32)
            w["out.w"] = self._pack_conv(P["out.2.conv.weight"], cout_pad=self.cout_pad)
            w["out.cb"] = self._pad_vec(P["out.2.conv.bias"], self.cout_pad)
        else:
            w["out.g"] = self._dev(P["id_predictor.0.gamma"], f32)
            w["out.b"] = self._dev(P["id_predictor.0.beta"], f32)
            w["out.w"] = self._pack_conv(P["id_predictor.1.conv.weight"], cout_pad=self.cout_pad)
            w["out.cb"] = self._pad_vec(P["id_predictor.1.conv.bias"], self.cout_pad)
        self.w = w
        self._frag_w = {}
        self._plans = {}
        self._ctx_key = None
        self._ctx_ref = None
        return self

    def weight_bytes(self):
        return sum(t.numel() * t.element_size() for t in self.w.values())

    class _Plan:
        pass

    def _plan(self, B, H, W, _fuse_head=True, _selfctx=False):
        key = (B, H, W, "selfctx") if _selfctx else (B, H, W)
        if key in self._plans:
            return self._plans[key]
        if self.w is None:
            raise MdxError("UNetModel: load_state_dict() must be called before the first forward")
        for lvl in range(len(self.channel_mult) - 1):
            if (H >> lvl) % 2 or (W >> lvl) % 2:
                raise MdxError(f"UNetModel: latent {H}x{W} is not divisible by 2^{len(self.channel_mult) - 1}")
        dev = self.device
        w = self.w
        P = UNetModel._Plan()
        A = _Arena(dev)
        main, ctxops, descs = [], [], []
        meta = []
        gn_need = [0]

        def emit(fn, kind, flops=0, launches=1, info=""):
            main.append(fn)
            meta.append({"kind": kind, "flops": int(flops), "launches": launches, "info": info})
        P.x_static = torch.zeros((B, self.in_channels, H, W), dtype=f32, device=dev)
        P.t_static = torch.zeros((B,), dtype=f32, device=dev)
        TC = self.max_context_len
        P.B, P.H, P.W = B, H, W

        producer = {}
        _arena_get = A.get

        def _get(shape, dtype=f16):
            t = _arena_get(shape, dtype)
            producer.pop(t.data_ptr(), None)
            return t
        A.get = _get
        op_index = {}

        def add_gemm(oplist, **kw):
            d = ops.make_gemm_desc(**kw)
            d._w_tensor = kw["w"]
            descs.append(d)
            if oplist is main:
                producer[kw["out"].data_ptr()] = d
                op_index[ctypes.addressof(d)] = len(main)
            fn = (lambda d=d: ops.gemm_run(d))
            if oplist is main:
                ks, st, up = kw.get("ksize", 1), kw.get("stride", 1), kw.get("upsample", 0)
                hs_, ws2 = (2 * kw["H"], 2 * kw["W"]) if up else (kw["H"], kw["W"])
                pad = 1 if ks == 3 else 0
                m_rows = kw["B"] * ((hs_ + 2 * pad - ks) // st + 1) * ((ws2 + 2 * pad - ks) // st + 1)
                kdim = ks * ks * (kw["c1"] + kw.get("c2", 0))
                emit(fn, "gemm", 2 * m_rows * kw["N"] * kdim, 1, f"M={m_rows} N={kw['N']} K={kdim} k{ks}s{st}u{up}")
                meta[-1]["desc"] = d
            else:
                oplist.append(fn)

        gn_calls = []

        def add_gn(x1, x2, g, b, eps, silu, out, scale=None, shift=None):
            Bq, HW, C1 = x1.shape
            C2 = 0 if x2 is None else x2.shape[2]
            gn_need[0] = max(gn_need[0], ops.groupnorm_ws_floats(Bq, HW, C1 + C2))
            call = dict(x1=x1, x2=x2, g=g, b=b, eps=eps, silu=silu, out=out, cs=None, meta=len(meta), film=scale is not None,
                        prod=(producer.get(x1.data_ptr()), None if x2 is None else producer.get(x2.data_ptr())))
            producer.pop(out.data_ptr(), None)
            gn_calls.append(call)

            def run(c=call):
                if c.get("fs") is not None:
                    return ops.groupnorm_from_splitk(c["fs"], c["g"], c["b"], c["eps"], c["silu"], c["out"])
                if c["cs"] is not None:
                    cs1, n1, cs2, n2 = c["cs"]
                    return ops.groupnorm_colstats(c["x1"], cs1, n1, c["x2"], cs2, n2, c["g"], c["b"], c["eps"], c["silu"],
                                                  out=c["out"], scale=scale, shift=shift,
                                                  mod_ld=self._emb_total if scale is not None else 0)
                if scale is not None:
                    return ops.groupnorm_scaleshift(c["x1"], c["x2"], c["g"], c["b"], scale, shift, self._emb_total, c["eps"],
                                                    c["silu"], ws=P.gn_ws, out=c["out"])
                return ops.groupnorm(c["x1"], c["x2"], c["g"], c["b"], c["eps"], c["silu"], ws=P.gn_ws, out=c["out"])
            emit(run, "groupnorm", 0, 2, f"B={Bq} HW={HW} C={C1 + C2}")

        mc, ted = self.model_channels, self.time_embed_dim
        t_emb = torch.empty((B, mc), dtype=f32, device=dev)
        e1 = torch.empty((B, ted), dtype=f32, device=dev)
        emb = torch.empty((B, ted), dtype=f32, device=dev)
        P.emb_all = torch.empty((B, self._emb_total), dtype=f32, device=dev)
        emit(lambda: ops.timestep_embedding(P.t_static, mc, out=t_emb), "small")
        emit(lambda: ops.dense_small(t_emb, w["te0.w"], w["te0.b"], act_out=True, out=e1), "small", 2 * B * mc * ted)
        emit(lambda: ops.dense_small(e1, w["te2.w"], w["te2.b"], out=emb), "small", 2 * B * ted * ted)
        if self.num_classes is not None:
            P.y_static = torch.zeros((B,), dtype=torch.long, device=dev)
            emit(lambda: emb.add_(w["label_emb"].index_select(0, P.y_static)), "small")
        emit(lambda: ops.dense_small(emb, w["emb.w"], w["emb.b"], act_in=True, out=P.emb_all), "small",
             2 * B * ted * self._emb_total)
        P.temb_ops = len(main)

        xin = A.get((B, H * W, self.cin_pad))
        emit(lambda: ops.nchw_to_nhwc(P.x_static, self.cin_pad, out=xin), "small")
        ck = {"xin": xin}

        P.ctx_pad = None
        P.attn_ws = None
        attn_ws_need = [0]
        ctx_kv = {}
        xattn_descs = []

        def conv3(src, cin, cout, wt, bias, h, wd, stride=1, upsample=0, rowbias=None, residual=None, src2=None, c2=0,
                  skip=None, gn=None, wsub=None):
            hs, ws_ = (2 * h, 2 * wd) if upsample else (h, wd)
            ho, wo = (hs + 2 - 3) // stride + 1, (ws_ + 2 - 3) // stride + 1
            out = A.get((B, ho * wo, cout))
            kw = {}
            if skip is not None:
                kw = dict(skip_a=skip[0], skip_a2=skip[1], skip_c1=skip[2], skip_c2=skip[3], skip_w=skip[4])
            if gn is not None:
                kw.update(gn_gamma=gn[0], gn_beta=gn[1], gn_eps=gn[2], gn_silu=1)
            if wsub is not None:
                kw["w_sub"] = wsub
            add_gemm(main, a=src, w=wt, N=cout, B=B, H=h, W=wd, c1=cin - c2, out=out, out_ld=cout, a2=src2, c2=c2,
                     bias=bias, rowbias=rowbias, rowbias_ld=self._emb_total if rowbias is not None else 0,
                     residual=residual, residual_ld=cout if residual is not None else 0, ksize=3, stride=stride,
                     upsample=upsample, **kw)
            if skip is not None:
                meta[-1]["flops"] += 2 * B * ho * wo * cout * (skip[2] + skip[3])
                meta[-1]["info"] += f" +skip1x1 K={skip[2] + skip[3]}"
            if gn is not None:
                dd = descs[-1]
                gn_convs.append(dd)
                meta[-1]["info"] += " +groupnorm(in)"
                gn_calls.append(dict(x1=src, x2=None, conv=dd, meta=len(meta) - 1, film=False,
                                     prod=(producer.get(src.data_ptr()), None)))
            return out, ho, wo

        def dense(oplist, src, rows_b, tokens, cin, nout, wt, bias=None, residual=None, epilogue=ops.EPI_NONE,
                  out=None, out_ld=None, out_mode=ops.OUT_ROWMAJOR, src2=None, c2=0, arena=True, **fold):
            cols = nout // 2 if epilogue == ops.EPI_GEGLU else nout
            if out is None:
                out = A.get((rows_b, tokens, cols))
                out_ld = cols
            add_gemm(oplist, a=src, w=wt, N=nout, B=rows_b, H=tokens, W=1, c1=cin - c2, out=out, out_ld=out_ld,
                     a2=src2, c2=c2, bias=bias, residual=residual, residual_ld=cols if residual is not None else 0,
                     epilogue=epilogue, out_mode=out_mode, **fold)
            return out

        ln_stats = {}
        tails = []

        def tail_rows(t, n, heads, dh):
            if (t + "tail.stream") not in w or self.transformer_depth != 1 or _selfctx:
                return 0
            if TC > 96 or TC % 8:
                return 0
            forced = ops.get_option("unet_st_tail")
            cands = [forced] if forced in (32, 64) else ([] if forced == 0 else [64, 32])
            for r in cands:
                if not ops.st_tail_supported(heads * dh, heads, dh, n, r):
                    continue
                blocks = B * n // r
                if forced in (32, 64) or (r == 64 and blocks >= 512) or (r == 32 and blocks >= 192):
                    return r
            return 0

        heads_fused = []

        def head_rows(t, x, n, heads, dh):
            if not _fuse_head or (t + "head.stream") not in w or ops.get_option("unet_st_head") == 0:
                return 0
            r = tail_rows(t, n, heads, dh)
            if not r or not ops.st_head_supported(heads * dh, n, r) or producer.get(x.data_ptr()) is None:
                return 0
            return r

        def fused_tail(t, rows_t, o, tok, x, ch, inner, heads, dh, n):
            kc = torch.zeros((B, TC, inner), dtype=f16, device=dev)
            vtc = torch.zeros((B, inner, TC), dtype=f16, device=dev)
            ctx_kv[t] = (kc, vtc)
            out = A.get((B, n, ch))
            td = ops.make_st_tail_desc(o, tok, x, out, kc, vtc, w[t + "tail.stream"], w[t + "tail.vec"], B, n, ch, heads,
                                       dh, 1, TC, tile_rows=rows_t)
            tails.append(td)
            td._bufs = (o, tok, x, out, kc, vtc)
            producer[out.data_ptr()] = td

            def run_tail(td=td):
                td.ctx_len = P.ctx_len
                ops.st_tail_run(td)
            emit(run_tail, "gemm", 2 * B * n * 16 * inner * inner + 4 * B * heads * n * 77 * dh, 1,
                 f"st_tail M={B * n} C={inner} rows={rows_t} (to_out1..proj_out fused)")
            return out

        def stats_buf(rows, width):
            if (rows, width) not in ln_stats:
                ln_stats[(rows, width)] = torch.zeros((rows, width // 64, 2), dtype=f32, device=dev)
# ... 178 lines not shown
                first = "op" not in ck and "conv_in" in ck and len(hs) == 1
                rows_t = tail_rows(t, n, heads, dh)
                if first:
                    ck.update(op=main[-1], live=(x, tok, o))
                if rows_t:
                    out = fused_tail(t, rows_t, o, tok, x, ch, inner, heads, dh, n)
                    A.release(qk); vt_release(vt); A.release(tok); A.release(ln)
                    return out
                tok2 = dense(main, o, B, n, inner, inner, w[t + "attn1.o.w"], bias=w[t + "attn1.o.b"], residual=tok,
                             stats_out=st)
                if first:
                    ck.update(op2=main[-1], live2=(x, tok2) + (() if st is None else (st,)))
                A.release(qk); vt_release(vt); A.release(tok)
                xfuse = (ops.get_option("unet_xattn_fuse") and not _selfctx and dh == 64 and TC <= 128 and TC % 8 == 0
                         and n % 64 == 0)
                if xfuse:
                    kc = torch.zeros((B, TC, inner), dtype=f16, device=dev)
                    vtc = torch.zeros((B, inner, TC), dtype=f16, device=dev)
                    ctx_kv[t] = (kc, vtc)
                    xkw = dict(tile_n=64, splitk=1, tile_m=0 if n % 128 == 0 else 64, xattn_k=kc, xattn_vt=vtc, xattn_len=TC, xattn_cap=TC, xattn_scale=scale, out=o,
                               out_ld=inner)
                if st is None:
                    emit(lambda ln=ln, tok2=tok2, t=t: ops.layernorm(tok2, w[t + "norm2.g"], w[t + "norm2.b"], 1e-5, out=ln),
                         "layernorm")
                    q2 = dense(main, ln, B, n, inner, inner, w[t + "attn2.q.w"], **(xkw if xfuse else {}))
                else:
                    q2 = dense(main, tok2, B, n, inner, inner, w[t + "attn2.q.w"], **consumer(t + "attn2.q"), **(xkw if xfuse else {}))
                    if _selfctx:
                        emit(lambda ln=ln, tok2=tok2, t=t: ops.layernorm(tok2, w[t + "norm2.g"], w[t + "norm2.b"], 1e-5, out=ln),
                             "layernorm")
                if xfuse:
                    xattn_descs.append(descs[-1])
                    meta[-1]["flops"] += 4 * B * heads * n * 77 * dh
                    meta[-1]["info"] += f" +cross-attention h={heads} d={dh}"
                    q2 = None
                if _selfctx:
                    k2 = dense(main, ln, B, n, inner, inner, w[t + "attn2.k.w"])
                    v2t = vt_buffer(n, inner)
                    nv2 = v2t.shape[2]
                    dense(main, ln, B, n, inner, inner, w[t + "attn2.v.w"], out=v2t, out_ld=nv2, out_mode=ops.OUT_TRANSPOSED)
                    attn_ws_need[0] = max(attn_ws_need[0], ops.attention_ws_bytes(B, heads, dh, n, n))
                    emit(lambda q2=q2, k2=k2, v2t=v2t, o=o, nv2=nv2: ops.attention(
                        q2.data_ptr(), k2.data_ptr(), v2t.data_ptr(), o.data_ptr(), B, heads, dh, n, n, scale,
                        n * inner, inner, n * inner, inner, inner * nv2, nv2, n * inner, inner, ws=P.attn_ws),
                        "attention", 4 * B * heads * n * n * dh, 1, f"attn2-self B={B} h={heads} N={n} d={dh}")
                    A.release(k2); vt_release(v2t)
                elif not xfuse:
                    kc = torch.zeros((B, TC, inner), dtype=f16, device=dev)
                    vtc = torch.zeros((B, inner, TC), dtype=f16, device=dev)
                    ctx_kv[t] = (kc, vtc)
                    emit(lambda q2=q2, kc=kc, vtc=vtc, o=o: ops.attention(
                        q2.data_ptr(), kc.data_ptr(), vtc.data_ptr(), o.data_ptr(), B, heads, dh, n, P.ctx_len, scale,
                        n * inner, inner, TC * inner, inner, inner * TC, TC, n * inner, inner),
                        "attention", 4 * B * heads * n * 77 * dh, 1, f"cross B={B} h={heads} N={n} d={dh}")
                tok3 = dense(main, o, B, n, inner, inner, w[t + "attn2.o.w"], bias=w[t + "attn2.o.b"], residual=tok2,
                             stats_out=st)
                if q2 is not None:
                    A.release(q2)
                A.release(tok2)
                if st is None:
                    emit(lambda ln=ln, tok3=tok3, t=t: ops.layernorm(tok3, w[t + "norm3.g"], w[t + "norm3.b"], 1e-5, out=ln),
                         "layernorm")
                    g = dense(main, ln, B, n, inner, 8 * inner, w[t + "ff1.w"], bias=w[t + "ff1.b"], epilogue=ops.EPI_GEGLU)
                else:
                    g = dense(main, tok3, B, n, inner, 8 * inner, w[t + "ff1.w"], epilogue=ops.EPI_GEGLU, **consumer(t + "ff1"))
                tok = dense(main, g, B, n, 4 * inner, inner, w[t + "ff2.w"], bias=w[t + "ff2.b"], residual=tok3,
                            stats_out=st if (fold1 and not last) else None)
                A.release(g); A.release(tok3); A.release(ln)
            out = dense(main, tok, B, n, inner, ch, w[pre + "proj_out.w"], bias=w[pre + "proj_out.b"], residual=x)
            A.release(tok)
            return out

        P.ctx_pad = torch.zeros((B, TC, self.context_dim), dtype=f16, device=dev)
        P.ctx_len = 0

        h, wd = H, W
        hs = []
        cur = None

        def held(t):
            return any(t is s_[0] for s_ in hs)

        def layer_op(pre, layer, cur, skip, h, wd):
            kind = layer[0]
            if kind == "res":
                return resblock(pre, cur, skip, layer[1], layer[2], h, wd)
            if kind in ("resdown", "resup"):
                return resblock(pre, cur, None, layer[1], layer[2], h, wd, mode=kind[3:])
            if kind == "st":
                return transformer(pre, cur, layer[1], layer[2], layer[3], h, wd), h, wd
            if kind == "down":
                if self.conv_resample:
                    return conv3(cur, layer[1], layer[1], w[pre + "w"], w[pre + "b"], h, wd, stride=2)
                new = A.get((B, (h // 2) * (wd // 2), layer[1]))
                emit(lambda cur=cur, new=new: ops.avgpool2x2(cur, B, h, wd, layer[1], out=new), "small")
                return new, h // 2, wd // 2
            if kind == "up":
                if self.conv_resample:
                    return conv3(cur, layer[1], layer[1], w[pre + "w"], w[pre + "b"], h, wd, upsample=1, wsub=w.get(pre + "wsub"))
                new = A.get((B, 4 * h * wd, layer[1]))
                emit(lambda cur=cur, new=new: ops.upsample_nearest2x(cur, B, h, wd, layer[1], out=new), "small")
                return new, 2 * h, 2 * wd
            raise ValueError(kind)

        for i, blk in enumerate(self.input_blocks):
            for j, layer in enumerate(blk):
                pre = f"input_blocks.{i}.{j}."
                if layer[0] == "conv":
                    cur, h, wd = conv3(xin, self.cin_pad, layer[2], w[pre + "w"], w[pre + "b"], h, wd)
                    ck["conv_in"] = main[-1]
                    A.release(xin)
                    continue
                new, h2, w2 = layer_op(pre, layer, cur, None, h, wd)
                if not held(cur):
                    A.release(cur)
                cur, h, wd = new, h2, w2
            hs.append((cur, h, wd))
        ck.setdefault("op", None)
        for j, layer in enumerate(self.middle_block):
            new, h, wd = layer_op(f"middle_block.{j}.", layer, cur, None, h, wd)
            if not held(cur):
                A.release(cur)
            cur = new
        for i, blk in enumerate(self.output_blocks):
            skip, sh, sw = hs.pop()
            assert (sh, sw) == (h, wd)
            for j, layer in enumerate(blk):
                new, h, wd = layer_op(f"output_blocks.{i}.{j}.", layer, cur, skip if j == 0 else None, h, wd)
                A.release(cur)
                if j == 0:
                    A.release(skip)
                cur = new
        a = A.get((B, h * wd, mc))
        add_gn(cur, None, w["out.g"], w["out.b"], 1e-5, self.n_embed is None, a)
        P.eps_nhwc = torch.empty((B, h * wd, self.cout_pad), dtype=f16, device=dev)
        add_gemm(main, a=a, w=w["out.w"], N=self.cout_pad, B=B, H=h, W=wd, c1=mc, out=P.eps_nhwc, out_ld=self.cout_pad,
                 bias=w["out.cb"], ksize=3 if self.n_embed is None else 1)

        for t, (kc, vtc) in ctx_kv.items():
            inner = kc.shape[2]
            add_gemm(ctxops, a=P.ctx_pad, w=w[t + "attn2.k.w"], N=inner, B=B, H=TC, W=1, c1=self.context_dim, out=kc,
                     out_ld=inner)
            add_gemm(ctxops, a=P.ctx_pad, w=w[t + "attn2.v.w"], N=inner, B=B, H=TC, W=1, c1=self.context_dim, out=vtc,
                     out_ld=TC, out_mode=ops.OUT_TRANSPOSED)

        need = max([ops.gemm_workspace_bytes(d) for d in descs] + [0])
        P.gemm_ws = ops.new_gemm_workspace(need, dev)
        for d in descs:
            d.workspace = P.gemm_ws.data_ptr()
            d.workspace_bytes = P.gemm_ws.numel() * 4
        P.gn_ws = torch.empty(max(gn_need[0], 4), dtype=f32, device=dev)
        if attn_ws_need[0]:
            P.attn_ws = ops.attention_workspace(attn_ws_need[0], dev)
        if ops.get_option("unet_conv_stream"):
            for d in descs:
                M = d.B * d.H * d.W
                if not (d.ksize == 3 and d.stride == 1 and not d.upsample and d.c2 == 0 and d.c1 % 64 == 0 and d.N % 64 == 0
                        and M <= ops.get_option("unet_conv_stream") and d.out_mode == ops.OUT_ROWMAJOR and not d.skip_w
                        and not d.gn_gamma):
                    continue
                q = ops.gemm_query(d)
                w4 = ops.get_option("unet_conv_stream_w4")
                if w4 and q[3] == 1 and d.N % 128 == 0 and d.c1 // 64 >= 5 and not d.colstats_out and not d.defer_reduce:
                    keep = (d.tile_m, d.tile_n, d.splitk)
                    d.tile_m, d.tile_n, d.splitk = 128, 128, min(d.c1 // 64, w4)
                    q = ops.gemm_query(d)
                    if not (q[0] == 128 and q[1] == 128 and q[3] == 1 and q[2] > 4 and not q[6]):
                        d.tile_m, d.tile_n, d.splitk = keep
                        q = ops.gemm_query(d)
                if not (q[0] == 128 and q[1] in (64, 128) and q[3] == 1):
                    continue
                if q[1] == 128 and not (q[2] > 1 and not q[6]):
                    continue
                wkey = d._w_tensor.data_ptr()
                if wkey not in self._frag_w:
                    self._frag_w[wkey] = ops.pack_frag_weight(ops.unpack_gemm_weight(d._w_tensor, d.N, 9 * d.c1)).reshape(-1)
                d.w, d.w_frag = self._frag_w[wkey].data_ptr(), 1
        P.colstats = {}
        fuse_hw = ops.get_option("unet_gn_splitk_fuse")
        if fuse_hw:
            for c in gn_calls:
                if c.get("head") is not None or c.get("conv") is not None or c.get("proj") is not None:
                    continue
                _, HW, C1 = c["x1"].shape
                if HW > fuse_hw:
                    continue
                cpg = C1 // 32
                L = cpg // math.gcd(cpg, 8)
                d = c["prod"][0]
                if (c["x2"] is None and not c["film"] and L <= 64 and HW * L * 16 <= (64 << 10) and isinstance(d, ops.GemmDesc)
                        and d.N == C1
                        and d.out_ld == C1 and op_index.get(ctypes.addressof(d)) == c["meta"] - 1
                        and ops.gemm_query(d)[2] > 1 and ops.groupnorm_from_splitk_ok(d)):
                    d.defer_reduce = 1
                    c["fs"] = d
                    meta[c["meta"] - 1]["launches"] = 1
        if os.environ.get("MDX_UNET_GN_COLSTATS", "1") != "0":
            ops.wire_groupnorm_colstats(gn_calls, meta, B, dev, P.colstats)
        else:
            ops.wire_groupnorm_colstats([], meta, B, dev, P.colstats)
            for c in gn_calls:
                _, HW, C1 = c["x1"].shape
                cpg = (C1 + (0 if c["x2"] is None else c["x2"].shape[2])) // 32
                L = cpg // math.gcd(cpg, 8)
                if L <= 64 and HW * L * 16 <= (64 << 10):
                    meta[c["meta"]]["launches"] = 1
        if any(not hd.colstats for hd in heads_fused) or any(not dd.gn_colstats for dd in gn_convs):
            return self._plan(B, H, W, _fuse_head=False, _selfctx=_selfctx)
        if any(m.get("dead") for m in meta):
            keep = [i for i, m in enumerate(meta) if not m.get("dead")]
            main[:] = [main[i] for i in keep]
            meta[:] = [meta[i] for i in keep]
        if ops.get_option("unet_tune_first_use"):
            tws = ops.new_gemm_workspace(256 << 20, dev)
            for d in descs:
                d.workspace, d.workspace_bytes = tws.data_ptr(), tws.numel() * 4
            P.tuned_shapes = ops.tune_untuned(descs)
            torch.cuda.synchronize()
            del tws
            ops.release_tune_scratch()
            for d in descs:
                d.workspace, d.workspace_bytes = P.gemm_ws.data_ptr(), P.gemm_ws.numel() * 4
        need2 = max([ops.gemm_workspace_bytes(d) for d in descs] + [0])
        if need2 > P.gemm_ws.numel() * 4:
            P.gemm_ws = ops.new_gemm_workspace(need2, dev)
            for d in descs:
                d.workspace = P.gemm_ws.data_ptr()
                d.workspace_bytes = P.gemm_ws.numel() * 4
        ops.check_colstats_wiring(descs)
        ops.account_gemm_launches(meta)
        P.main, P.ctxops, P.descs, P.meta = main, ctxops, descs, meta
        assert len(main) == len(meta)
        P.arena_bytes = A.total
        P.ln_stats = ln_stats
        P.arena = A
        P.tails = tails
        P.ragged_vt = ragged_vt
        P.heads_fused = heads_fused
        P.ctx_kv = ctx_kv
        P.xattn_descs = xattn_descs
        P.ck = ck if (ck.get("op") is not None and not _selfctx) else None
        P.graph = None
        P.dup_graph = None
        P.graph_failed = False
        self._plans[key] = P
        return P

    def _ensure_context(self, P, context):
        key = (context.data_ptr(), context._version, tuple(context.shape), context.dtype, id(P))
        alive = self._ctx_ref() if self._ctx_ref is not None else None
        if key == self._ctx_key and alive is context:
            return
        Bc, T, Dc = context.shape
        if Bc != P.B or Dc != self.context_dim:
            raise MdxError(f"context shape {tuple(context.shape)} does not match batch {P.B} / context_dim {self.context_dim}")
        if T > self.max_context_len:
            raise MdxError(f"context length {T} > max_context_len={self.max_context_len}")
        P.ctx_pad.zero_()
        P.ctx_pad[:, :T].copy_(context)
        P.ctx_len = T
        for d in getattr(P, "xattn_descs", ()):
            d.xattn_len = T
        for op in P.ctxops:
            op()
        self._ctx_key = key
        self._ctx_ref = weakref.ref(context)
        if getattr(P, "graph_ctx_len", None) != T:
            P.graph = None
            P.dup_graph = None

    def time_embedding_table(self, t):
        if self.w is None:
            raise MdxError("UNetModel: load_state_dict() must be called before time_embedding_table()")
        if self.num_classes is not None:
            raise MdxError("UNetModel: a class-conditional UNet adds label_emb(y) before the ResBlock projections; "
                           "there is no timestep-only table")
        t = torch.as_tensor(t, dtype=f32).to(self.device).reshape(-1).contiguous()
        w = self.w
        e0 = ops.timestep_embedding(t, self.model_channels)
        e1 = ops.dense_small(e0, w["te0.w"], w["te0.b"], act_out=True)
        e2 = ops.dense_small(e1, w["te2.w"], w["te2.b"])
        return ops.dense_small(e2, w["emb.w"], w["emb.b"], act_in=True)

    def forward_nhwc(self, x, timesteps, context=None, temb=None, y=None, cfg_dup=False):
        if (y is not None) != (self.num_classes is not None):
            raise MdxError("UNetModel: must specify y if and only if the model is class-conditional")
        if y is not None and temb is not None:
            raise MdxError("UNetModel: time_embedding_table() rows do not carry the label embedding; pass timesteps with y")
        if not (isinstance(x, torch.Tensor) and x.is_cuda):
            raise MdxError("UNetModel: x must be a CUDA(HIP) tensor (no CPU fallback)")
        B, C, H, W = x.shape
        if C != self.in_channels:
            raise MdxError(f"UNetModel: expected {self.in_channels} input channels, got {C}")
        if context is None:
            if getattr(self, "_selfctx_bad", None) is None:
                self._selfctx_bad = sorted({l[2] * l[3] for _, l in self._named_layers()
                                            if l[0] == "st" and l[2] * l[3] != self.context_dim})
            bad = self._selfctx_bad
            if bad:
                raise MdxError(f"UNetModel: context=None makes attn2 attend to its own input (attention.py:133), which needs "
                               f"context_dim == transformer width; context_dim={self.context_dim}, widths {bad}")
            P = self._plan(B, H, W, _selfctx=True)
        else:
            P = self._plan(B, H, W)
            self._ensure_context(P, context)
        P.x_static.copy_(x)
# ... 95 lines not shown
```

minddiffusion_amd/ops.py:

```python
import ctypes
import os

import torch

from . import _lib
from ._lib import GemmDesc, EPI_NONE, EPI_GEGLU, EPI_GELU, EPI_QUICKGELU, OUT_ROWMAJOR, OUT_TRANSPOSED
from ._lib import EPI_PRELU, OUT_D2S2

f16 = torch.float16
f32 = torch.float32


_OPTIONS = {"unet_st_tail": int(os.environ.get("MDX_UNET_ST_TAIL", "-1")),
            "unet_st_head": int(os.environ.get("MDX_UNET_ST_HEAD", "-1")),
            "unet_conv_stream": int(os.environ.get("MDX_UNET_CONV_STREAM", "128")),
            "gn_colstats_fold": int(os.environ.get("MDX_GN_COLSTATS_FOLD", "0")),
            "unet_gn_splitk_fuse": int(os.environ.get("MDX_UNET_GN_SPLITK_FUSE", "256")),
            "unet_conv_stream_w4": int(os.environ.get("MDX_UNET_CONV_STREAM_W4", "0")),
            "unet_skip_fuse": int(os.environ.get("MDX_UNET_SKIP_FUSE", "1")),
            "unet_gn_conv_fuse": int(os.environ.get("MDX_UNET_GN_CONV_FUSE", "0")),
            "unet_tune_first_use": int(os.environ.get("MDX_UNET_TUNE_FIRST_USE", "0")),
            "unet_subpixel_upsample": int(os.environ.get("MDX_UNET_SUBPIXEL_UPSAMPLE", "1")),
            "unet_gn_proj_fuse": int(os.environ.get("MDX_UNET_GN_PROJ_FUSE", "0")),
            "unet_xattn_fuse": int(os.environ.get("MDX_UNET_XATTN_FUSE", "1")),
            "unet_cfg_dup": int(os.environ.get("MDX_UNET_CFG_DUP", "4")),
            "unet_cfg_dup_check": int(os.environ.get("MDX_UNET_CFG_DUP_CHECK", "0")),
            "glide_qkv_merge": int(os.environ.get("MDX_GLIDE_QKV_MERGE", "1")),
            "glide_gn_qkv_fuse": int(os.environ.get("MDX_GLIDE_GN_QKV_FUSE", "0"))}


def set_option(name, value):
    if name in _OPTIONS:
        _OPTIONS[name] = int(value)
        return
    _lib.check(_lib.load().mdx_set_option(name.encode(), int(value)), "mdx_set_option")


def get_option(name):
    if name in _OPTIONS:
        return _OPTIONS[name]
    out = ctypes.c_int(0)
    _lib.check(_lib.load().mdx_get_option(name.encode(), ctypes.byref(out)), "mdx_get_option")
    return int(out.value)


def capture_graph(ops_list):
    import gc
    g = torch.cuda.CUDAGraph()
    gc.collect()
    was_enabled = gc.isenabled()
    gc.disable()
    try:
        with torch.cuda.graph(g):
            for op in ops_list:
                op()
    finally:
        if was_enabled:
            gc.enable()
    return g


def _stream():
    return ctypes.c_void_p(torch.cuda.current_stream().cuda_stream)


def _ptr(t):
    return None if t is None else ctypes.c_void_p(t.data_ptr())


def _chk(t, dtype, name):
    if t is None:
        return
    if not t.is_cuda:
        raise _lib.MdxError(f"{name}: tensor must live on the GPU (no CPU fallback)")
    if t.dtype != dtype:
        raise _lib.MdxError(f"{name}: expected {dtype}, got {t.dtype}")
    if not t.is_contiguous():
        raise _lib.MdxError(f"{name}: tensor must be contiguous")


def nchw_to_nhwc(x, cpad, out=None):
    _chk(x, f32, "x")
    B, C, H, W = x.shape
    if out is None:
        out = torch.empty((B, H * W, cpad), dtype=f16, device=x.device)
    _lib.check(_lib.load().mdx_nchw_to_nhwc_f16(_ptr(x), _ptr(out), B, C, H, W, cpad, _stream()), "mdx_nchw_to_nhwc_f16")
    return out


def nhwc_to_nchw(x, C, H, W, out=None):
    _chk(x, f16, "x")
    B, HW, Cs = x.shape
    assert HW == H * W
    if out is None:
        out = torch.empty((B, C, H, W), dtype=f32, device=x.device)
    _lib.check(_lib.load().mdx_nhwc_to_nchw_f32(_ptr(x), _ptr(out), B, C, H, W, Cs, _stream()), "mdx_nhwc_to_nchw_f32")
    return out


def groupnorm_ws_floats(B, HW, C, groups=32):
    return int(_lib.load().mdx_groupnorm_ws_floats(B, HW, C, groups))


def groupnorm(x1, x2, gamma, beta, eps, silu, ws=None, out=None, groups=32):
    _chk(x1, f16, "x1"); _chk(x2, f16, "x2"); _chk(gamma, f32, "gamma"); _chk(beta, f32, "beta")
    B, HW, C1 = x1.shape
    C2 = 0 if x2 is None else x2.shape[2]
    C = C1 + C2
    if ws is None:
        ws = torch.empty(groupnorm_ws_floats(B, HW, C, groups), dtype=f32, device=x1.device)
    if out is None:
        out = torch.empty((B, HW, C), dtype=f16, device=x1.device)
    _lib.check(_lib.load().mdx_groupnorm_f16(_ptr(x1), C1, _ptr(x2), C2, _ptr(gamma), _ptr(beta), _ptr(out), B, HW,
                                             groups, float(eps), int(bool(silu)), _ptr(ws), _stream()),
               "mdx_groupnorm_f16")
    return out


class FoldedColStats:

    def __init__(self, raw, nrb, batch):
        f = (nrb + 63) // 64
        self.raw, self.nrb, self.batch = raw, nrb, batch
        self.nrb2 = (nrb + f - 1) // f
        self.folded = torch.zeros((batch * self.nrb2, raw.shape[1], 2), dtype=f32, device=raw.device)

    def data_ptr(self):
        return self.raw.data_ptr()

    def fold(self):
        _lib.check(_lib.load().mdx_colstats_fold_f32(_ptr(self.raw), self.nrb, _ptr(self.folded), self.nrb2, self.batch,
                                                     self.raw.shape[1], _stream()), "mdx_colstats_fold_f32")
        return self.folded, self.nrb2


def groupnorm_colstats(x1, cs1, nrb1, x2, cs2, nrb2, gamma, beta, eps, silu, out=None, groups=32, scale=None, shift=None,
                       mod_ld=0):
    if isinstance(cs1, FoldedColStats):
        cs1, nrb1 = cs1.fold()
    if isinstance(cs2, FoldedColStats):
        cs2, nrb2 = cs2.fold()
    B, HW, C1 = x1.shape
    C2 = 0 if x2 is None else x2.shape[2]
    if out is None:
        out = torch.empty((B, HW, C1 + C2), dtype=f16, device=x1.device)
    _lib.check(_lib.load().mdx_groupnorm_colstats_f16(_ptr(x1), C1, _ptr(cs1), int(nrb1), _ptr(x2), C2, _ptr(cs2), int(nrb2),
                                                      _ptr(gamma), _ptr(beta), _ptr(scale), _ptr(shift), int(mod_ld),
                                                      _ptr(out), B, HW, groups, float(eps), int(bool(silu)), _stream()),
               "mdx_groupnorm_colstats_f16")
    return out


def groupnorm_from_splitk_ok(desc, groups=32):
    return bool(_lib.load().mdx_groupnorm_from_splitk_ok(ctypes.byref(desc), groups))


def groupnorm_from_splitk(desc, gamma, beta, eps, silu, out, groups=32):
    _lib.check(_lib.load().mdx_groupnorm_from_splitk_f16(ctypes.byref(desc), _ptr(gamma), _ptr(beta), _ptr(out), groups,
                                                         float(eps), int(bool(silu)), _stream()),
               "mdx_groupnorm_from_splitk_f16")
    return out


def groupnorm_scaleshift(x1, x2, gamma, beta, scale, shift, mod_ld, eps, silu, ws=None, out=None, groups=32):
    _chk(x1, f16, "x1"); _chk(x2, f16, "x2")
    B, HW, C1 = x1.shape
    C2 = 0 if x2 is None else x2.shape[2]
    C = C1 + C2
    if ws is None:
        ws = torch.empty(groupnorm_ws_floats(B, HW, C, groups), dtype=f32, device=x1.device)
    if out is None:
        out = torch.empty((B, HW, C), dtype=f16, device=x1.device)
    _lib.check(_lib.load().mdx_groupnorm_scaleshift_f16(
        _ptr(x1), C1, _ptr(x2), C2, _ptr(gamma), _ptr(beta), _ptr(scale), _ptr(shift), int(mod_ld), _ptr(out), B, HW,
        groups, float(eps), int(bool(silu)), _ptr(ws), _stream()), "mdx_groupnorm_scaleshift_f16")
    return out


def avgpool2x2(x, B, H, W, C, out=None):
    if out is None:
        out = torch.empty((B, (H // 2) * (W // 2), C), dtype=f16, device=x.device)
    _lib.check(_lib.load().mdx_avgpool2x2_f16(_ptr(x), _ptr(out), B, H, W, C, _stream()), "mdx_avgpool2x2_f16")
    return out


def upsample_nearest2x(x, B, H, W, C, out=None):
    if out is None:
        out = torch.empty((B, 4 * H * W, C), dtype=f16, device=x.device)
    _lib.check(_lib.load().mdx_upsample_nearest2x_f16(_ptr(x), _ptr(out), B, H, W, C, _stream()),
               "mdx_upsample_nearest2x_f16")
    return out


def glide_text_embed(tokens, mask, tok_emb, pos, pad, out=None):
    B, T = tokens.shape
    width = pos.shape[1]
    if out is None:
        out = torch.empty((B, T, width), dtype=f16, device=tokens.device)
    _lib.check(_lib.load().mdx_glide_text_embed_f16(_ptr(tokens), _ptr(mask), _ptr(tok_emb), _ptr(pos), _ptr(pad),
                                                    _ptr(out), B, T, width, tok_emb.shape[0], _stream()),
               "mdx_glide_text_embed_f16")
    return out


def glide_superres_input(x, low, out=None):
    B, _, S, _ = x.shape
    if out is None:
        out = torch.empty((B, S * S, 8), dtype=f16, device=x.device)
    _lib.check(_lib.load().mdx_glide_superres_input_f16(_ptr(x), _ptr(low), _ptr(out), B, S, low.shape[2], _stream()),
               "mdx_glide_superres_input_f16")
    return out


def glide_step(x, out_c, out_u, ld, scale, coef8, mode, noise_scale, noise, x_next, pred_x0):
    B, _, H, W = x.shape
    c8 = (ctypes.c_float * 8)(*[float(v) for v in coef8])
    _lib.check(_lib.load().mdx_glide_step_f32(_ptr(x), _ptr(out_c), _ptr(out_u), int(ld), float(scale),
                                              ctypes.cast(c8, ctypes.c_void_p), int(mode), float(noise_scale),
                                              _ptr(noise), _ptr(x_next), _ptr(pred_x0), B, H, W, _stream()),
               "mdx_glide_step_f32")


def glide_kv_slots(entries, device):
    import numpy as np
    rows = []
    for src, dst, seb, dbb, sp, dp, r, rb in entries:
        for v in (src.data_ptr(), dst.data_ptr(), seb, dbb, sp, dp, rb):
            if v % 16:
                raise _lib.MdxError("glide_kv_slots: pointers and byte counts must be multiples of 16")
        rows.append([src.data_ptr(), dst.data_ptr(), seb, dbb, sp, dp, (int(r) & 0xffffffff) | (int(rb) << 32)])
    return torch.from_numpy(np.asarray(rows, dtype=np.int64)).to(device), len(rows)


def glide_kv_select(slots, nslots, entry0, entry_per_b, b0, nb, blocks_per_copy=8):
    _lib.check(_lib.load().mdx_glide_kv_select_f16(_ptr(slots), int(nslots), int(entry0), int(entry_per_b), int(b0), int(nb),
                                                   int(blocks_per_copy), _stream()), "mdx_glide_kv_select_f16")


def layernorm(x, gamma, beta, eps, out=None):
    _chk(x, f16, "x"); _chk(gamma, f32, "gamma"); _chk(beta, f32, "beta")
    C = x.shape[-1]
    rows = x.numel() // C
    if out is None:
        out = torch.empty_like(x)
    _lib.check(_lib.load().mdx_layernorm_f16(_ptr(x), _ptr(gamma), _ptr(beta), _ptr(out), rows, C, float(eps), _stream()),
               "mdx_layernorm_f16")
    return out


def pack_gemm_weight(w2d):
    N, K = w2d.shape
    dev = w2d.device
    Np, Kp = (N + 63) // 64 * 64, (K + 63) // 64 * 64
    wp = torch.zeros((Np, Kp), dtype=f16, device=dev)
    wp[:N, :K] = w2d
    t = wp.view(Np // 64, 64, Kp // 64, 8, 8).permute(0, 2, 1, 3, 4)
    r = torch.arange(64, device=dev)
    src = torch.arange(8, device=dev)[None, :] ^ ((r >> 1) & 7)[:, None]
    idx = src[None, None, :, :, None].expand(Np // 64, Kp // 64, 64, 8, 8)
    return torch.gather(t, 3, idx).contiguous().view(-1)


def conv_weight_k_order(w4d, cin_pad=None, cout_pad=None):
    w4d = w4d.to(torch.float32)
    co, ci, kh, kw = w4d.shape
    cip = cin_pad or ci
    cop = cout_pad or co
    if cip % 64 == 0:
        assert cip == ci
        p = torch.zeros((cop, ci // 64, kh * kw, 64), dtype=torch.float32, device=w4d.device)
        p[:co] = w4d.reshape(co, ci // 64, 64, kh * kw).permute(0, 1, 3, 2)
        return p.reshape(cop, kh * kw * ci)
    p = torch.zeros((cop, kh * kw, cip), dtype=torch.float32, device=w4d.device)
    p[:co, :, :ci] = w4d.permute(0, 2, 3, 1).reshape(co, kh * kw, ci)
    return p.reshape(cop, kh * kw * cip)


def pack_conv_weight(w4d, cin_pad=None, cout_pad=None):
    return pack_gemm_weight(conv_weight_k_order(w4d, cin_pad, cout_pad))


def subpixel_conv_weight(w4d):
    w = w4d.to(torch.float32)
    rows = {0: (w[:, :, 0], w[:, :, 1] + w[:, :, 2]), 1: (w[:, :, 0] + w[:, :, 1], w[:, :, 2])}
    out = []
    for dy in (0, 1):
        for dx in (0, 1):
            taps = []
            for a in (0, 1):
                r = rows[dy][a]
                cols = (r[:, :, 0], r[:, :, 1] + r[:, :, 2]) if dx == 0 else (r[:, :, 0] + r[:, :, 1], r[:, :, 2])
                taps.append(torch.stack(cols, -1))
            out.append(torch.stack(taps, 2))
    return torch.cat(out, 0)


def pack_subpixel_conv_weight(w4d):
    assert w4d.shape[0] % 64 == 0 and w4d.shape[1] % 64 == 0
    return pack_conv_weight(subpixel_conv_weight(w4d))


def pack_conv_weight_frag(w4d):
    co, ci = w4d.shape[0], w4d.shape[1]
    assert co % 64 == 0 and ci % 64 == 0
    return pack_frag_weight(conv_weight_k_order(w4d).to(f16)).reshape(-1)


def unpack_gemm_weight(packed, N, K):
    Np, Kp = (N + 63) // 64 * 64, (K + 63) // 64 * 64
    t = packed.view(Np // 64, Kp // 64, 64, 8, 8)
    r = torch.arange(64, device=packed.device)
    src = torch.arange(8, device=packed.device)[None, :] ^ ((r >> 1) & 7)[:, None]
    inv = torch.argsort(src, 1)
    idx = inv[None, None, :, :, None].expand(Np // 64, Kp // 64, 64, 8, 8)
    return torch.gather(t, 3, idx).permute(0, 2, 1, 3, 4).reshape(Np, Kp)[:N, :K].contiguous()


def make_gemm_desc(a, w, N, B, H, W, c1, out, out_ld, a2=None, c2=0, bias=None, rowbias=None, rowbias_ld=0,
                   residual=None, residual_ld=0, ksize=1, stride=1, upsample=0, epilogue=EPI_NONE,
                   out_mode=OUT_ROWMAJOR, splitk=0, workspace=None, out_bs=0, out2=None, out2_ld=0, n_split=0, asym_pad=0,
                   stats_out=None, ln_stats=None, ln_s=None, ln_eps=1e-5, tile_m=0, tile_n=0, colstats_out=None, stages=0,
                   w_frag=0, skip_a=None, skip_a2=None, skip_c1=0, skip_c2=0, skip_w=None, gn_colstats=None, gn_nrb=0,
                   gn_gamma=None, gn_beta=None, gn_eps=1e-5, gn_silu=1, w_sub=None, xattn_k=None, xattn_vt=None, xattn_len=0,
                   xattn_cap=0, xattn_scale=0.0, act_slope=None):
    d = GemmDesc()
    d.a = a.data_ptr()
    d.a2 = 0 if a2 is None else a2.data_ptr()
    d.c1, d.c2 = int(c1), int(c2)
    d.w = w.data_ptr()
    d.bias = 0 if bias is None else bias.data_ptr()
    d.rowbias = 0 if rowbias is None else rowbias.data_ptr()
    d.rowbias_ld = int(rowbias_ld)
    d.residual = 0 if residual is None else residual.data_ptr()
    d.residual_ld = int(residual_ld)
    d.out = out.data_ptr()
    d.out_ld = int(out_ld)
    d.B, d.H, d.W, d.N = int(B), int(H), int(W), int(N)
    d.ksize, d.stride, d.upsample = int(ksize), int(stride), int(upsample)
    d.epilogue, d.out_mode, d.splitk = int(epilogue), int(out_mode), int(splitk)
    d.workspace = 0 if workspace is None else workspace.data_ptr()
    d.workspace_bytes = 0 if workspace is None else workspace.numel() * workspace.element_size()
    d.out_bs = int(out_bs)
    d.out2 = 0 if out2 is None else out2.data_ptr()
    d.out2_ld, d.n_split, d.asym_pad = int(out2_ld), int(n_split), int(asym_pad)
    d.stats_out = 0 if stats_out is None else stats_out.data_ptr()
    d.ln_stats = 0 if ln_stats is None else ln_stats.data_ptr()
    d.ln_s = 0 if ln_s is None else ln_s.data_ptr()
    d.ln_nt = 0 if ln_stats is None else (int(c1) + int(c2)) // 64
    d.ln_eps = float(ln_eps)
    d.tile_m, d.tile_n, d.stages, d.w_frag = int(tile_m), int(tile_n), int(stages), int(w_frag)
    d.gn_colstats = 0 if gn_colstats is None else gn_colstats.data_ptr()
    d.gn_gamma = 0 if gn_gamma is None else gn_gamma.data_ptr()
    d.gn_beta = 0 if gn_beta is None else gn_beta.data_ptr()
    d.gn_nrb, d.gn_silu, d.gn_eps = int(gn_nrb), int(gn_silu), float(gn_eps)
    d.skip_a = 0 if skip_a is None else skip_a.data_ptr()
    d.skip_a2 = 0 if skip_a2 is None else skip_a2.data_ptr()
    d.skip_c1, d.skip_c2 = int(skip_c1), int(skip_c2)
    d.skip_w = 0 if skip_w is None else skip_w.data_ptr()
    d.colstats_out = 0 if colstats_out is None else colstats_out.data_ptr()
    d.colstats_cap = 0 if colstats_out is None else int(colstats_out.shape[0])
    d.w_sub = 0 if w_sub is None else w_sub.data_ptr()
    if xattn_k is not None:
        d.xattn_k, d.xattn_vt = xattn_k.data_ptr(), xattn_vt.data_ptr()
        d.xattn_len, d.xattn_cap, d.xattn_scale = int(xattn_len), int(xattn_cap), float(xattn_scale)
    if act_slope is not None:
        d.act_slope, d.act_slope_n = act_slope.data_ptr(), int(act_slope.numel())
    return d


def fold_layernorm(wt, gamma, beta, bias=None):
    w32 = wt.to(torch.float64)
    wg = (w32 * gamma.to(torch.float64)[None, :]).to(f16)
    s = wg.to(torch.float64).sum(1).to(f32).contiguous()
    cb = w32 @ beta.to(torch.float64)
    if bias is not None:
        cb = cb + bias.to(torch.float64)
    return wg.contiguous(), s, cb.to(f32).contiguous()


def gemm_workspace_bytes(desc):
    return int(_lib.load().mdx_gemm_workspace_bytes(ctypes.byref(desc)))


_WS_HEAD = 16384


def new_gemm_workspace(nbytes, device):
    import weakref
    base = torch.zeros((_WS_HEAD + max(int(nbytes), 16)) // 4 + 1, dtype=f32, device=device)
    ws = base[_WS_HEAD // 4:]
    lib = _lib.load()
    _lib.check(lib.mdx_gemm_bind_counters(ctypes.c_void_p(ws.data_ptr()), ctypes.c_void_p(base.data_ptr())),
               "mdx_gemm_bind_counters")
    weakref.finalize(ws, lib.mdx_gemm_release_workspace, ctypes.c_void_p(ws.data_ptr()))
    return ws


def gemm_query(desc):
    out = (ctypes.c_int * 7)()
    _lib.check(_lib.load().mdx_gemm_query(ctypes.byref(desc), out), "mdx_gemm_query")
    return tuple(int(v) for v in out)


def account_gemm_launches(meta):
    for m in meta:
        d = m.get("desc")
        if d is None:
            continue
        q = gemm_query(d)
        m["launches"] = 2 if (q[2] > 1 and not q[6] and not d.defer_reduce) else 1
        m["info"] = m["info"].split(" split=")[0] + f" split={q[2] if q[2] > 1 else 0}" + ("i" if q[6] else "")


tune_cache = {}
_tune_flush = {}


def gemm_shape_key(d):
    var = ((1 if d.c2 > 0 else 0) | (d.epilogue << 1) | (8 if d.n_split else 0) | (16 if d.ln_stats else 0)
           | (32 if d.stats_out else 0) | (64 if d.out_mode == 1 else 0) | (128 if d.colstats_out else 0)
           | (256 if d.residual else 0) | (512 if d.rowbias else 0) | (1024 if d.skip_w else 0) | (2048 if d.gn_gamma else 0)
           | (4096 if d.w_sub else 0))
    return (d.B * d.H * d.W, d.N, d.ksize * d.ksize * (d.c1 + d.c2), d.ksize, d.stride, d.upsample, var, d.B, d.H, d.W)


def gemm_tune(desc, reps=5, cold=True):
    flush, nbytes = None, 0
    if cold:
        dev = torch.cuda.current_device()
        if dev not in _tune_flush:
            _tune_flush[dev] = torch.empty(512 << 20, dtype=torch.uint8, device=f"cuda:{dev}")
        flush, nbytes = ctypes.c_void_p(_tune_flush[dev].data_ptr()), _tune_flush[dev].numel()
    best, us = (ctypes.c_int * 4)(), (ctypes.c_float * 2)()
    _lib.check(_lib.load().mdx_gemm_tune(ctypes.byref(desc), _stream(), flush, nbytes, int(reps), best, us), "mdx_gemm_tune")
    return tuple(int(v) for v in best) + (float(us[0]), float(us[1]))


def tune_untuned(descs, reps=5):
    measured = 0
    for d in descs:
        if (d.colstats_out or d.defer_reduce or d.w_frag or d.skip_w or d.gn_gamma or d.tile_m or d.tile_n or d.splitk
                or d.stages):
            continue
        key = gemm_shape_key(d)
        if key not in tune_cache:
            if gemm_query(d)[4]:
                continue
            tune_cache[key] = gemm_tune(d, reps)
            measured += 1
        tm, tn, sk, stg = tune_cache[key][:4]
        old = (d.tile_m, d.tile_n, d.splitk, d.stages)
        d.tile_m, d.tile_n, d.splitk, d.stages = tm, tn, sk, stg
        if _lib.load().mdx_gemm_check(ctypes.byref(d)) != 0:
            d.tile_m, d.tile_n, d.splitk, d.stages = old
    return measured


def release_tune_scratch():
    _tune_flush.clear()


TUNE_CACHE_VERSION = 2


def save_tune_cache(path):
    import json
    with open(path, "w") as f:
        json.dump({"version": TUNE_CACHE_VERSION, "key_fields": 10,
                   "entries": [[list(k), list(v)] for k, v in sorted(tune_cache.items())]}, f)


def load_tune_cache(path):
    import json
    import warnings
    with open(path) as f:
        data = json.load(f)
    if not isinstance(data, dict) or data.get("version") != TUNE_CACHE_VERSION:
        warnings.warn(f"load_tune_cache: {path} was written under another key layout (version "
                      f"{data.get('version') if isinstance(data, dict) else 'none'}, this build: {TUNE_CACHE_VERSION}); ignored")
        return 0
    n = 0
    for k, v in data["entries"]:
        if len(k) != 10:
            continue
        tune_cache[tuple(k)] = tuple(v)
        n += 1
    return n


def gemm_run(desc):
    _lib.check(_lib.load().mdx_gemm_f16(ctypes.byref(desc), _stream()), "mdx_gemm_f16")


def gemm(a, w, N, B, H, W, c1, out=None, **kw):
    _chk(a, f16, "a"); _chk(w, f16, "w")
    ksize, stride, upsample = kw.get("ksize", 1), kw.get("stride", 1), kw.get("upsample", 0)
    Hs, Ws = (2 * H, 2 * W) if upsample else (H, W)
    pad = 1 if ksize == 3 else 0
    Ho = (Hs + 2 * pad - ksize) // stride + 1
    Wo = (Ws + 2 * pad - ksize) // stride + 1
    M = B * Ho * Wo
    epi = kw.get("epilogue", EPI_NONE)
    out_mode = kw.get("out_mode", OUT_ROWMAJOR)
    if out is None:
        if out_mode == OUT_TRANSPOSED:
            ld = kw.pop("out_ld", Ho * Wo)
            out = torch.zeros((B, N, ld), dtype=f16, device=a.device)
        elif out_mode == OUT_D2S2:
            ld = kw.pop("out_ld", N // 4)
            out = torch.empty((B, 2 * Ho, 2 * Wo, ld), dtype=f16, device=a.device)
        else:
            cols = N // 2 if epi == EPI_GEGLU else N
            ld = kw.pop("out_ld", cols)
            out = torch.empty((M, ld), dtype=f16, device=a.device)
    else:
        ld = kw.pop("out_ld")
    d = make_gemm_desc(a, w, N, B, H, W, c1, out, ld, **kw)
# ... 313 lines not shown
```

Before: 5.327 latents/s.

## Add 128x80 HALO 3x3 conv kernel with 80-column weight packing for UNet convs

```diff
diff --git a/include/mdx.h b/include/mdx.h
--- a/include/mdx.h
+++ b/include/mdx.h
@@ -101,6 +101,8 @@
     float xattn_scale;
     const float* act_slope;
     int act_slope_n;
+    const void* w80;
+    const void* skip_w80;
 } mdx_gemm_desc;
 
 #define MDX_GEMM_WS_HEAD 16384
diff --git a/minddiffusion_amd/_lib.py b/minddiffusion_amd/_lib.py
--- a/minddiffusion_amd/_lib.py
+++ b/minddiffusion_amd/_lib.py
@@ -36,6 +36,7 @@
         ("w_frag", c_int), ("stages", c_int), ("w_sub", c_void_p),
         ("xattn_k", c_void_p), ("xattn_vt", c_void_p), ("xattn_len", c_int), ("xattn_cap", c_int), ("xattn_scale", c_float),
         ("act_slope", c_void_p), ("act_slope_n", c_int),
+        ("w80", c_void_p), ("skip_w80", c_void_p),
     ]
 
 
diff --git a/minddiffusion_amd/csrc/gemm.hip b/minddiffusion_amd/csrc/gemm.hip
--- a/minddiffusion_amd/csrc/gemm.hip
+++ b/minddiffusion_amd/csrc/gemm.hip
@@ -850,6 +850,406 @@
         gemm_epilogue<BM, BN, SWAP, NW>(p, acc, smem, LinearRows{tile_m * BM}, n0, split, bpre, tile_m, tile_id);
     trace_mark(p, 4);
     }
+}
+
+template <int NSB>
+__global__ __launch_bounds__(256, 1) void conv3x3_halo80_kernel(const GemmParams p) {
+    constexpr int BM = 128, BN = 80, NW = 4;
+    constexpr int HROWS = 180, HINST = 23, HALO_BYTES = HINST * 1024, HJ = 6;
+    constexpr int B_BYTES = BN * 128;
+    constexpr int BINST = BN / 8;
+    constexpr int BJ = (BINST + NW - 1) / NW;
+    constexpr int TM = 2, TN = 5;
+    static_assert(NSB == 4, "the tap pipeline waits for tile t + 1 with tile t + 2 in flight");
+    extern __shared__ __attribute__((aligned(16))) char smem[];
+    mdx_kernarg_touch<sizeof(GemmParams)>();
+
+    const int tid = threadIdx.x;
+    const int lane = tid & 63;
+    const int wave = __builtin_amdgcn_readfirstlane(tid >> 6);
+    const int l15 = lane & 15, kq = lane >> 4;
+
+    const int ntiles = p.tiles_m * p.tiles_n;
+    const int tile_id = p.spread ? (int)blockIdx.x : (blockIdx.x & 7) * p.tiles_per_xcd + (blockIdx.x >> 3);
+    if (tile_id >= ntiles) return;
+    int tile_m, tile_n;
+    if (p.n_fastest) {
+        tile_m = tile_id / p.tiles_n;
+        tile_n = tile_id - tile_m * p.tiles_n;
+    } else {
+        tile_n = tile_id / p.tiles_m;
+        tile_m = tile_id - tile_n * p.tiles_m;
+    }
+    trace_mark(p, 0);
+    const int n0 = tile_n * BN;
+    const int pw = p.W >> 4, ph = p.H >> 3;
+    const int pb = tile_m / (ph * pw);
+    const int prem = tile_m - pb * (ph * pw);
+    const int py0 = (prem / pw) * 8, px0 = (prem % pw) * 16;
+    const int nt = p.ktiles;
+    const int c_end = nt / 9;
+
+    const __amdgpu_buffer_rsrc_t rs_a = make_rsrc(p.a, p.a_bytes);
+    const __amdgpu_buffer_rsrc_t rs_w = make_rsrc(p.w80, p.w80_bytes);
+
+    const int lrow = lane >> 3, lchk = lane & 7;
+    unsigned hal_off[HJ];
+    const unsigned row_bytes = (unsigned)p.cin * 2;
+#pragma unroll
+    for (int q = 0; q < HJ; ++q) {
+        const int hp = (wave * HJ + q) * 8 + lrow;
+        const int hr = hp / 18, hc = hp - hr * 18;
+        const int y = py0 - 1 + hr, x = px0 - 1 + hc;
+        const bool ok = hp < HROWS && y >= 0 && y < p.H && x >= 0 && x < p.W;
+        hal_off[q] = ok ? (unsigned)((pb * p.H + y) * p.W + x) * row_bytes + (unsigned)((lchk ^ ((hc >> 1) & 7)) * 16) : MDX_OOB;
+    }
+    const unsigned b_off = (unsigned)((size_t)tile_n * p.kt64 * B_BYTES) + (unsigned)lane * 16u;
+    auto dma_halo = [&](int q, int chunk, int hb) {
+        if (wave * HJ + q >= HINST) return;
+        const unsigned off = hal_off[q] == MDX_OOB ? MDX_OOB : hal_off[q] + (unsigned)chunk * 128u;
+        dma16(rs_a, smem + hb * HALO_BYTES + (wave * HJ + q) * 1024, off);
+    };
+    auto dma_b = [&](int kt, int stage) {
+        char* sb = smem + 2 * HALO_BYTES + stage * B_BYTES;
+#pragma unroll
+        for (int j = 0; j < BJ; ++j)
+            if (wave + NW * j < BINST)
+                dma16s(rs_w, sb + (wave + NW * j) * 1024, b_off + (unsigned)((wave + NW * j) * 1024), (unsigned)kt * (unsigned)B_BYTES);
+    };
+    auto wait_but_one_tile = [&]() {
+        if (wave < BINST - NW * (BJ - 1))
+            asm volatile("s_waitcnt vmcnt(%0)" ::"n"(BJ) : "memory");
+        else
+            asm volatile("s_waitcnt vmcnt(%0)" ::"n"(BJ - 1) : "memory");
+    };
+
+    f32x4 acc[TM][TN];
+#pragma unroll
+    for (int i = 0; i < TM; ++i)
+#pragma unroll
+        for (int j = 0; j < TN; ++j)
+#pragma unroll
+            for (int r = 0; r < 4; ++r) acc[i][j][r] = 0.f;
+
+    int hp0[TM];
+#pragma unroll
+    for (int i = 0; i < TM; ++i) hp0[i] = (wave * 2 + i) * 18 + l15;
+    const int swz_b = (l15 >> 1) & 7;
+    const int b_row_off = 2 * HALO_BYTES + l15 * 128;
+
+    constexpr int CPR = BN / 8, RPP = 16, NST = CPR * RPP;
+    const int chunk = tid % CPR, r0 = tid / CPR;
+    float bb[8];
+#pragma unroll
+    for (int e = 0; e < 8; ++e) bb[e] = 0.f;
+    if (p.bias && tid < NST) {
+        const float4* b4 = reinterpret_cast<const float4*>(p.bias + n0 + chunk * 8);
+        const float4 x0 = b4[0], x1 = b4[1];
+        bb[0] = x0.x; bb[1] = x0.y; bb[2] = x0.z; bb[3] = x0.w;
+        bb[4] = x1.x; bb[5] = x1.y; bb[6] = x1.z; bb[7] = x1.w;
+    }
+
+    float2* gn_tab = reinterpret_cast<float2*>(smem + 2 * HALO_BYTES + NSB * B_BYTES);
+    if (p.gn_cs) {
+        float2* csum = reinterpret_cast<float2*>(smem);
+        const int cpg = p.cin >> 5;
+        const float2* src = reinterpret_cast<const float2*>(p.gn_cs) + (size_t)pb * p.gn_nrb * p.cin;
+        for (int c = tid; c < p.cin; c += NW * 64) {
+            float su = 0.f, sq = 0.f;
+            int k = 0;
+            for (; k + 8 <= p.gn_nrb; k += 8) {
+                float2 v[8];
+#pragma unroll
+                for (int e = 0; e < 8; ++e) v[e] = src[(size_t)(k + e) * p.cin + c];
+#pragma unroll
+                for (int e = 0; e < 8; ++e) {
+                    su += v[e].x;
+                    sq += v[e].y;
+                }
+            }
+            for (; k < p.gn_nrb; ++k) {
+                const float2 v = src[(size_t)k * p.cin + c];
+                su += v.x;
+                sq += v.y;
+            }
+            csum[c] = make_float2(su, sq);
+        }
+        __syncthreads();
+        for (int c = tid; c < p.cin; c += NW * 64) {
+            const int g = c / cpg;
+            float su = 0.f, sq = 0.f;
+            for (int e = 0; e < cpg; ++e) {
+                const float2 v = csum[g * cpg + e];
+                su += v.x;
+                sq += v.y;
+            }
+            const float inv = 1.0f / ((float)cpg * (float)(p.H * p.W));
+            const float mean = su * inv;
+            float var = sq * inv - mean * mean;
+            var = var < 0.f ? 0.f : var;
+            const float a = p.gn_gamma[c] * rsqrtf(var + p.gn_eps);
+            gn_tab[c] = make_float2(a, p.gn_beta[c] - mean * a);
+        }
+        __syncthreads();
+    }
+    auto gn_transform = [&](int chunk_c, int hb) {
+#pragma unroll
+        for (int q = 0; q < HJ; ++q) {
+            if (wave * HJ + q >= HINST || hal_off[q] == MDX_OOB) continue;
+            char* pc = smem + hb * HALO_BYTES + (wave * HJ + q) * 1024 + lane * 16;
+            const int ch0 = chunk_c * 64 + (int)((hal_off[q] >> 4) & 7u) * 8;
+            const f16x8 x = *reinterpret_cast<const f16x8*>(pc);
+            f16x8 y;
+#pragma unroll
+            for (int e = 0; e < 8; ++e) {
+                const float2 t = gn_tab[ch0 + e];
+                const float v = (float)x[e] * t.x + t.y;
+                y[e] = (f16)(p.gn_silu ? silu_f(v) : v);
+            }
+            *reinterpret_cast<f16x8*>(pc) = y;
+        }
+    };
+
+    f16x8 af[2][2][TM], bf[2][2][TN];
+    auto rdfrag = [&](auto slot_c, const int hb, const int tap, const int stage) {
+        constexpr int slot = decltype(slot_c)::value;
+        const int ky = tap / 3, kx = tap - ky * 3;
+        const int a_key = (((l15 + kx) >> 1) & 7) << 4;
+        const char* sb = smem + stage * B_BYTES + b_row_off;
+#pragma unroll
+        for (int ks = 0; ks < 2; ++ks) {
+#pragma unroll
+            for (int i = 0; i < TM; ++i)
+                af[slot][ks][i] = *reinterpret_cast<const f16x8*>(smem + hb * HALO_BYTES + (hp0[i] + ky * 18 + kx) * 128 + (((4 * ks + kq) << 4) ^ a_key));
+#pragma unroll
+            for (int j = 0; j < TN; ++j)
+                bf[slot][ks][j] = *reinterpret_cast<const f16x8*>(sb + j * 16 * 128 + (((4 * ks + kq) ^ swz_b) << 4));
+        }
+    };
+    auto mfmas = [&](auto slot_c) {
+        constexpr int slot = decltype(slot_c)::value;
+#pragma unroll
+        for (int ks = 0; ks < 2; ++ks)
+#pragma unroll
+            for (int i = 0; i < TM; ++i)
+#pragma unroll
+                for (int j = 0; j < TN; ++j)
+                    acc[i][j] = __builtin_amdgcn_mfma_f32_16x16x32_f16(bf[slot][ks][j], af[slot][ks][i], acc[i][j], 0, 0, 0);
+    };
+    using I0 = std::integral_constant<int, 0>;
+    using I1 = std::integral_constant<int, 1>;
+
+#pragma unroll
+    for (int q = 0; q < HJ; ++q) dma_halo(q, 0, 0);
+#pragma unroll
+    for (int i = 0; i < NSB - 1; ++i) dma_b(i, i);
+    trace_mark(p, 1);
+    if (wave < BINST - NW * (BJ - 1))
+        asm volatile("s_waitcnt vmcnt(%0)" ::"n"(2 * BJ) : "memory");
+    else
+        asm volatile("s_waitcnt vmcnt(%0)" ::"n"(2 * BJ - 2) : "memory");
+    if (p.gn_cs) {
+        gn_transform(0, 0);
+        asm volatile("s_waitcnt lgkmcnt(0)" ::: "memory");
+    }
+    __builtin_amdgcn_s_barrier();
+    trace_mark(p, 2);
+    rdfrag(I0{}, 0, 0, 0);
+
+    int t = 0;
+    for (int c = 0; c < c_end; ++c) {
+        const int hb = c & 1;
+        const bool more = c + 1 < c_end;
+        auto tap_step = [&](auto cur_c, auto nxt_c, auto tap_c) {
+            constexpr int tap = decltype(tap_c)::value;
+            if (t + 2 < nt)
+                wait_but_one_tile();
+            else
+                asm volatile("s_waitcnt vmcnt(0)" ::: "memory");
+            if (tap == 8 && more && p.gn_cs) {
+                gn_transform(c + 1, hb ^ 1);
+                asm volatile("s_waitcnt lgkmcnt(0)" ::: "memory");
+            }
+            __builtin_amdgcn_s_barrier();
+            if (more && tap < HJ) dma_halo(tap, c + 1, hb ^ 1);
+            if (t + NSB - 1 < nt) dma_b(t + NSB - 1, (t + NSB - 1) & (NSB - 1));
+            __builtin_amdgcn_sched_barrier(0);
+            if (tap < 8)
+                rdfrag(nxt_c, hb, tap + 1, (t + 1) & (NSB - 1));
+            else if (more)
+                rdfrag(nxt_c, hb ^ 1, 0, (t + 1) & (NSB - 1));
+            __builtin_amdgcn_sched_barrier(0);
+            mfmas(cur_c);
+            __builtin_amdgcn_sched_barrier(0);
+            ++t;
+        };
+#define MDX_TAP(n) std::integral_constant<int, n>{}
+        tap_step(I0{}, I1{}, MDX_TAP(0)); tap_step(I1{}, I0{}, MDX_TAP(1)); tap_step(I0{}, I1{}, MDX_TAP(2));
+        tap_step(I1{}, I0{}, MDX_TAP(3)); tap_step(I0{}, I1{}, MDX_TAP(4)); tap_step(I1{}, I0{}, MDX_TAP(5));
+        tap_step(I0{}, I1{}, MDX_TAP(6)); tap_step(I1{}, I0{}, MDX_TAP(7)); tap_step(I0{}, I1{}, MDX_TAP(8));
+#undef MDX_TAP
+        if (more) {
+#pragma unroll
+            for (int ks = 0; ks < 2; ++ks) {
+#pragma unroll
+                for (int i = 0; i < TM; ++i) af[0][ks][i] = af[1][ks][i];
+#pragma unroll
+                for (int j = 0; j < TN; ++j) bf[0][ks][j] = bf[1][ks][j];
+            }
+        }
+    }
+
+    if (p.skip_w80) {
+        constexpr int SA_BYTES = BM * 128;
+        static_assert(2 * SA_BYTES <= 2 * HALO_BYTES, "skip tiles reuse the halo area");
+        const __amdgpu_buffer_rsrc_t rs_s1 = make_rsrc(p.skip_a, p.skip_a_bytes);
+        const __amdgpu_buffer_rsrc_t rs_s2 = make_rsrc(p.skip_a2 ? p.skip_a2 : p.skip_a, p.skip_a2 ? p.skip_a2_bytes : p.skip_a_bytes);
+        const __amdgpu_buffer_rsrc_t rs_sw = make_rsrc(p.skip_w80, p.skip_w80_bytes);
+        constexpr int SAJ = BM / 8 / NW;
+        int s_pix[SAJ];
+        unsigned s_cb[SAJ];
+#pragma unroll
+        for (int j = 0; j < SAJ; ++j) {
+            const int row = (wave * SAJ + j) * 8 + lrow;
+            s_pix[j] = (pb * p.H + py0 + (row >> 4)) * p.W + px0 + (row & 15);
+            s_cb[j] = (unsigned)((lchk ^ ((row >> 1) & 7)) * 16);
+        }
+        const unsigned sb_off = (unsigned)((size_t)tile_n * p.skip_kt * B_BYTES) + (unsigned)lane * 16u;
+        auto stage_skip = [&](int kt, int st) {
+            int ci0 = kt * 64;
+            const bool second = ci0 >= p.skip_c1;
+            const int cs2 = (second ? p.skip_c2 : p.skip_c1) * 2;
+            if (second) ci0 -= p.skip_c1;
+#pragma unroll
+            for (int j = 0; j < SAJ; ++j) {
+                const unsigned off = (unsigned)(s_pix[j] * cs2) + (unsigned)(ci0 * 2) + s_cb[j];
+                void* dst = smem + st * SA_BYTES + (wave * SAJ + j) * 1024;
+                if (second)
+                    dma16(rs_s2, dst, off);
+                else
+                    dma16(rs_s1, dst, off);
+            }
+#pragma unroll
+            for (int j = 0; j < BJ; ++j)
+                if (wave + NW * j < BINST)
+                    dma16(rs_sw, smem + 2 * HALO_BYTES + st * B_BYTES + (wave + NW * j) * 1024,
+                          sb_off + (unsigned)((wave + NW * j) * 1024) + (unsigned)kt * (unsigned)B_BYTES);
+        };
+        __syncthreads();
+        const int s_swz = (l15 >> 1) & 7;
+        if (p.skip_kt > 0) stage_skip(0, 0);
+        for (int kt = 0; kt < p.skip_kt; ++kt) {
+            const int st = kt & 1;
+            asm volatile("s_waitcnt vmcnt(0)" ::: "memory");
+            __builtin_amdgcn_s_barrier();
+            if (kt + 1 < p.skip_kt) stage_skip(kt + 1, st ^ 1);
+            const char* sa = smem + st * SA_BYTES + (wave * 32 + l15) * 128;
+            const char* sbk = smem + st * B_BYTES + b_row_off;
+#pragma unroll
+            for (int ks = 0; ks < 2; ++ks) {
+                f16x8 a2[TM], b2[TN];
+#pragma unroll
+                for (int i = 0; i < TM; ++i) a2[i] = *reinterpret_cast<const f16x8*>(sa + i * 16 * 128 + (((4 * ks + kq) ^ s_swz) << 4));
+#pragma unroll
+                for (int j = 0; j < TN; ++j) b2[j] = *reinterpret_cast<const f16x8*>(sbk + j * 16 * 128 + (((4 * ks + kq) ^ swz_b) << 4));
+#pragma unroll
+                for (int i = 0; i < TM; ++i)
+#pragma unroll
+                    for (int j = 0; j < TN; ++j) acc[i][j] = __builtin_amdgcn_mfma_f32_16x16x32_f16(b2[j], a2[i], acc[i][j], 0, 0, 0);
+            }
+        }
+    }
+
+    __syncthreads();
+    trace_mark(p, 3);
+    constexpr int SLD = BN + 8;
+    constexpr int PASSES = BM / RPP;
+    f16* stg = reinterpret_cast<f16*>(smem);
+    const int n = n0 + chunk * 8;
+    const bool storer = tid < NST;
+    const int mbase = (pb * p.H + py0) * p.W + px0;
+    u32x4 lrb[2] = {};
+    f16x8 lres[PASSES];
+    {
+        const __amdgpu_buffer_rsrc_t rs_rb = make_rsrc(p.rowbias, p.rowbias ? (unsigned)p.B * (unsigned)p.rowbias_ld * 4u : 0u);
+        const unsigned off = storer ? ((unsigned)pb * (unsigned)p.rowbias_ld + (unsigned)n) * 4u : MDX_OOB;
+        lrb[0] = __builtin_amdgcn_raw_buffer_load_b128(rs_rb, off, 0, 0);
+        lrb[1] = __builtin_amdgcn_raw_buffer_load_b128(rs_rb, off, 16, 0);
+        const __amdgpu_buffer_rsrc_t rs_res = make_rsrc(p.residual, p.residual ? p.res_bytes : 0u);
+#pragma unroll
+        for (int pass = 0; pass < PASSES; ++pass) {
+            const int row = r0 + pass * RPP;
+            const int m = mbase + (row >> 4) * p.W + (row & 15);
+            const unsigned roff = storer ? ((unsigned)m * (unsigned)p.residual_ld + (unsigned)n) * 2u : MDX_OOB;
+            lres[pass] = __builtin_bit_cast(f16x8, __builtin_amdgcn_raw_buffer_load_b128(rs_res, roff, 0, 0));
+        }
+    }
+#pragma unroll
+    for (int i = 0; i < TM; ++i)
+#pragma unroll
+        for (int j = 0; j < TN; ++j)
+            *reinterpret_cast<f16x4*>(&stg[(wave * 32 + i * 16 + l15) * SLD + j * 16 + kq * 4]) =
+                cvt4(acc[i][j][0], acc[i][j][1], acc[i][j][2], acc[i][j][3]);
+    __syncthreads();
+    trace_mark(p, 5);
+    const bool colstats = p.colstats_out != nullptr;
+    float cs[8], cq[8];
+#pragma unroll
+    for (int e = 0; e < 8; ++e) cs[e] = cq[e] = 0.f;
+    if (storer) {
+        const bool has_rb = p.rowbias != nullptr, has_res = p.residual != nullptr;
+        f16x8 sv[PASSES];
+#pragma unroll
+        for (int pass = 0; pass < PASSES; ++pass) sv[pass] = *reinterpret_cast<const f16x8*>(&stg[(r0 + pass * RPP) * SLD + chunk * 8]);
+#pragma unroll
+        for (int pass = 0; pass < PASSES; ++pass) {
+            const int row = r0 + pass * RPP;
+            const int m = mbase + (row >> 4) * p.W + (row & 15);
+            float f[8];
+#pragma unroll
+            for (int e = 0; e < 8; ++e) f[e] = (float)sv[pass][e] + bb[e];
+            if (has_rb) {
+                const f32x4 q0 = __builtin_bit_cast(f32x4, lrb[0]), q1 = __builtin_bit_cast(f32x4, lrb[1]);
+                f[0] += q0[0]; f[1] += q0[1]; f[2] += q0[2]; f[3] += q0[3];
+                f[4] += q1[0]; f[5] += q1[1]; f[6] += q1[2]; f[7] += q1[3];
+            }
+            if (has_res) {
+#pragma unroll
+                for (int e = 0; e < 8; ++e) f[e] += (float)lres[pass][e];
+            }
+            f16x8 o;
+#pragma unroll
+            for (int e = 0; e < 8; ++e) o[e] = (f16)f[e];
+            *reinterpret_cast<f16x8*>(p.out + (size_t)m * p.out_ld + n) = o;
+            if (colstats) {
+#pragma unroll
+                for (int e = 0; e < 8; ++e) {
+                    const float tv = (float)o[e];
+                    cs[e] += tv;
+                    cq[e] += tv * tv;
+                }
+            }
+        }
+    }
+    if (colstats) {
+        __syncthreads();
+        float* part = reinterpret_cast<float*>(smem);
+        if (storer) {
+#pragma unroll
+            for (int e = 0; e < 8; ++e) {
+                part[((size_t)r0 * BN + chunk * 8 + e) * 2] = cs[e];
+                part[((size_t)r0 * BN + chunk * 8 + e) * 2 + 1] = cq[e];
+            }
+        }
+        __syncthreads();
+        for (int i = tid; i < BN * 2; i += NW * 64) {
+            const int cc = i >> 1;
+            float a = 0.f;
+            for (int r = 0; r < RPP; ++r) a += part[((size_t)r * BN + cc) * 2 + (i & 1)];
+            p.colstats_out[((size_t)tile_m * p.N + n0 + cc) * 2 + (i & 1)] = a;
+        }
+    }
+    trace_mark(p, 4);
 }
 
 __device__ __forceinline__ void splitk_sum8(const GemmParams& p, const float* base, const size_t slab, float (&f)[8]) {
@@ -1208,6 +1608,21 @@
         p.skip_a2_bytes = (unsigned)s2;
         p.skip_w_bytes = (unsigned)sw;
     }
+    p.w80 = (const f16*)d->w80;
+    p.skip_w80 = (const f16*)d->skip_w80;
+    p.w_frag_flag = d->w_frag ? 1 : 0;
+    if (d->tile_n != 80 && ((d->tile_m != 0 && d->tile_m != 128) || d->splitk > 1 || d->defer_reduce)) p.w80 = p.skip_w80 = nullptr;
+    p.w80_bytes = p.skip_w80_bytes = 0;
+    if (p.w80 || d->tile_n == 80) {
+        MDX_REQUIRE(p.w80 && p.ksize == 3 && p.N % 80 == 0 && p.cin % 64 == 0,
+                    "mdx_gemm_f16: tile_n = 80 / w80 belong to 3x3 convs with N %% 80 == 0 and Cin %% 64 == 0 whose 80-column weight copy (w80) is set");
+        MDX_REQUIRE(!p.skip_w || p.skip_w80, "mdx_gemm_f16: w80 with a fused skip needs skip_w80 as well");
+        const size_t wb80 = (size_t)(p.N / 80) * ((size_t)9 * p.cin / 64) * 10240;
+        const size_t sw80 = p.skip_w ? (size_t)(p.N / 80) * p.skip_kt * 10240 : 0;
+        MDX_REQUIRE(wb80 <= 0x80000000ull && sw80 <= 0x80000000ull, "mdx_gemm_f16: w80 larger than 2 GiB");
+        p.w80_bytes = (unsigned)wb80;
+        p.skip_w80_bytes = (unsigned)sw80;
+    }
     if (p.rowbias) MDX_REQUIRE(p.rowbias_ld % 4 == 0, "mdx_gemm_f16: rowbias_ld must be a multiple of 4");
     if (p.residual) MDX_REQUIRE(p.residual_ld % 8 == 0, "mdx_gemm_f16: residual_ld must be a multiple of 8");
     MDX_REQUIRE(p.out_ld % 8 == 0 && p.out_bs % 8 == 0 && p.out_bs >= 0, "mdx_gemm_f16: out_ld / out_bs must be multiples of 8");
@@ -1231,6 +1646,8 @@
 static const TunedEntry g_tuned[] = {
 #include "gemm_tuned.inc"
     {0, 0, 0, 0, 0, 0, 0, 0, 0}};
+static const TunedEntry g_tuned80[] = {
+    {0, 0, 0, 0, 0, 0, 0, 0, 0}};
 
 int tuned_variant(const GemmParams& p) {
     return (p.c2 > 0 ? 1 : 0) | (p.epilogue == MDX_EPI_PRELU ? 2048 : p.epilogue << 1) | (p.n_split ? 8 : 0) | (p.ln_stats ? 16 : 0) |
@@ -1240,11 +1657,15 @@
 }
 
 bool halo_eligible(const GemmParams& p, int bm);
+bool halo80_eligible(const GemmParams& p);
 
 const TunedEntry* lookup_tuned(const GemmParams& p) {
     const bool use_table = mdx_opt(MDX_OPT_GEMM_TUNED) && !mdx_opt(MDX_OPT_GEMM_BM) && !mdx_opt(MDX_OPT_GEMM_BN);
     if (!use_table || p.bn_hint || p.st_hint || p.stride != 1 || p.upsample) return nullptr;
     if (p.epilogue == MDX_EPI_PRELU || p.d2s_c) return nullptr;
+    if (p.ksize == 3 && halo80_eligible(p))
+        for (const TunedEntry* e = g_tuned80; e->M; ++e)
+            if (e->M == p.M && e->N == p.N && e->K == p.K) return e;
     const int var1 = tuned_variant(p) + 1;
     const TunedEntry* any = nullptr;
     for (const TunedEntry* e = g_tuned; e->M; ++e)
@@ -1262,7 +1683,7 @@
 
 int pick_bn(const GemmParams& p) {
     if (p.epilogue == MDX_EPI_GEGLU) return 128;
-    if (p.bn_hint == 64 || p.bn_hint == 128) return p.bn_hint;
+    if (p.bn_hint == 64 || p.bn_hint == 128 || p.bn_hint == 80) return p.bn_hint;
     if (const TunedEntry* e = lookup_tuned(p))
         if (e->bn) return e->bn;
     const int optbn = mdx_opt(MDX_OPT_GEMM_BN);
@@ -1435,6 +1856,17 @@
     hipLaunchKernelGGL((conv3x3_halo_kernel<BM, BN, NSB, SWAP, PW, BDIR, W4>), grid, dim3(BM * 2), lds, st, p);
 }
 
+void launch_halo80(const GemmParams& p, dim3 grid, hipStream_t st) {
+    constexpr size_t lds0 = 2 * 23 * 1024 + 4 * 80 * 128;
+    const size_t lds = lds0 + (p.gn_cs ? (size_t)p.cin * 8 : 0);
+    static MdxPerDeviceOnce attr_once;
+    if (attr_once.first()) {
+        (void)hipFuncSetAttribute(reinterpret_cast<const void*>(&conv3x3_halo80_kernel<4>), hipFuncAttributeMaxDynamicSharedMemorySize,
+                                  (int)(lds0 + 640 * 8));
+    }
+    hipLaunchKernelGGL((conv3x3_halo80_kernel<4>), grid, dim3(256), lds, st, p);
+}
+
 template <int BN, int PW>
 void launch_halo_bdir(const GemmParams& p, bool swap, dim3 grid, hipStream_t st) {
     if (swap) launch_halo<128, BN, 2, true, PW, true>(p, grid, st); else launch_halo<128, BN, 2, false, PW, true>(p, grid, st);
@@ -1475,6 +1907,15 @@
     if (p.residual && (size_t)p.M * (size_t)p.residual_ld * 2 >= 0x80000000ull) return false;
     if (bm == 128 && halo8_eligible(p)) return true;
     return p.H % (bm / 16) == 0 && p.W % 16 == 0;
+}
+
+bool halo80_eligible(const GemmParams& p) {
+    if (!p.w80 || p.N % 80 != 0 || p.w_frag_flag) return false;
+    if (!halo_eligible(p, 128)) return false;
+    if (!(p.H % 8 == 0 && p.W % 16 == 0)) return false;
+    if (p.epilogue != MDX_EPI_NONE || p.stats_out || p.n_split || p.ln_stats) return false;
+    if (p.skip_w && !p.skip_w80) return false;
+    return true;
 }
 
 }
@@ -1719,6 +2160,15 @@
             return MDX_E_WORKSPACE;
         }
     }
+    if (bn == 80) {
+        if (!halo80_eligible(p) || d->splitk > 1 || (d->tile_m != 0 && d->tile_m != 128) || d->defer_reduce) {
+            mdx_set_error("mdx_gemm_f16: tile_n = 80 needs a launch the 128 x 80 HALO conv applies to (3x3, stride 1, one source, H %% 8 == 0, "
+                          "W %% 16 == 0, Cin %% 64 == 0, N %% 80 == 0, w80 set, plain row-major epilogue, tile_m 0 | 128, splitk <= 1)");
+            return MDX_E_INVALID;
+        }
+        r.c.bm = 128;
+        ns = 1;
+    }
     r.halo = r.c.bm >= 128 && halo_eligible(p, r.c.bm);
     if (r.c.bm == 256 && !r.halo) {
         mdx_set_error("mdx_gemm_f16: tile_m = 256 needs a launch the 16 x 16-patch HALO conv applies to (3x3, stride 1, H %% 16 == 0, "
@@ -1731,7 +2181,7 @@
                           p.HoWo, r.c.bm);
             return MDX_E_INVALID;
         }
-    } else if (p.gn_cs && !(r.halo && r.bn == 64 && !halo8_eligible(p))) {
+    } else if (p.gn_cs && !(r.halo && (r.bn == 64 || r.bn == 80) && !halo8_eligible(p))) {
         mdx_set_error("mdx_gemm_f16: the fused input GroupNorm needs a launch that resolves to the HALO 3x3 kernel with 64-column "
                       "tiles (ask mdx_gemm_query first)");
         return MDX_E_INVALID;
@@ -1928,7 +2378,9 @@
         int nsb = (c.bm == 256 || bn == 64) ? 3 : 2;
         if (st_req >= 2 && st_req <= 4) nsb = st_req;
         if (mdx_opt(MDX_OPT_HALO_NSB) >= 2 && mdx_opt(MDX_OPT_HALO_NSB) <= 4) nsb = mdx_opt(MDX_OPT_HALO_NSB);
-        if (d->w_frag) {
+        if (bn == 80) {
+            launch_halo80(p, grid, st);
+        } else if (d->w_frag) {
             MDX_REQUIRE(c.bm == 128, "mdx_gemm_f16: fragment-major weights run on 128-row HALO tiles only (got tile_m %d)", c.bm);
             const bool w4 = bn == 128 && ns > 1 && !rs.fixup && !swap;
             if (halo8_eligible(p)) {
@@ -2040,7 +2492,7 @@
     std::vector<long> seen;
     auto form = [](const int* q) { return (long)q[0] | ((long)q[1] << 10) | ((long)q[2] << 20) | ((long)q[3] << 30) | ((long)q[6] << 31); };
     seen.push_back(form(q0));
-    static const int BMS[] = {64, 128, 256}, BNS[] = {64, 128}, NSS[] = {1, 2, 3, 4, 6, 8, 12, 16, 20};
+    static const int BMS[] = {64, 128, 256}, BNS[] = {64, 80, 128}, NSS[] = {1, 2, 3, 4, 6, 8, 12, 16, 20};
     for (int bm : BMS)
         for (int bn : BNS)
             for (int ns : NSS) {
diff --git a/minddiffusion_amd/csrc/gemm_internal.h b/minddiffusion_amd/csrc/gemm_internal.h
--- a/minddiffusion_amd/csrc/gemm_internal.h
+++ b/minddiffusion_amd/csrc/gemm_internal.h
@@ -60,6 +60,10 @@
     const float* act_slope;
     int act_slope_n;
     int d2s_c;
+    const f16* w80;
+    const f16* skip_w80;
+    unsigned w80_bytes, skip_w80_bytes;
+    int w_frag_flag;
 };
 
 }
diff --git a/minddiffusion_amd/ldm/modules/diffusionmodules/openaimodel.py b/minddiffusion_amd/ldm/modules/diffusionmodules/openaimodel.py
--- a/minddiffusion_amd/ldm/modules/diffusionmodules/openaimodel.py
+++ b/minddiffusion_amd/ldm/modules/diffusionmodules/openaimodel.py
@@ -354,6 +354,7 @@
             w["out.cb"] = self._pad_vec(P["id_predictor.1.conv.bias"], self.cout_pad)
         self.w = w
         self._frag_w = {}
+        self._t80_w = {}
         self._plans = {}
         self._ctx_key = None
         self._ctx_ref = None
@@ -403,6 +404,7 @@
         def add_gemm(oplist, **kw):
             d = ops.make_gemm_desc(**kw)
             d._w_tensor = kw["w"]
+            d._skip_w_tensor = kw.get("skip_w")
             descs.append(d)
             if oplist is main:
                 producer[kw["out"].data_ptr()] = d
@@ -887,6 +889,26 @@
         P.gn_ws = torch.empty(max(gn_need[0], 4), dtype=f32, device=dev)
         if attn_ws_need[0]:
             P.attn_ws = ops.attention_workspace(attn_ws_need[0], dev)
+        if ops.get_option("unet_conv_t80"):
+            for d in descs:
+                if not (d.ksize == 3 and d.stride == 1 and not d.upsample and d.c2 == 0 and d.c1 % 64 == 0 and d.N % 80 == 0
+                        and d.out_mode == ops.OUT_ROWMAJOR and not (d.tile_m or d.tile_n or d.splitk or d.stages or d.w_frag)):
+                    continue
+                d.w80 = d.w
+                d.skip_w80 = d.skip_w
+                ok = ops.gemm_query(d)[1] == 80
+                d.w80 = d.skip_w80 = None
+                if not ok:
+                    continue
+
+                def t80(packed, K):
+                    key = packed.data_ptr()
+                    if key not in self._t80_w:
+                        self._t80_w[key] = ops.pack_gemm_weight_t80(ops.unpack_gemm_weight(packed, d.N, K))
+                    return self._t80_w[key].data_ptr()
+                d.w80 = t80(d._w_tensor, 9 * d.c1)
+                if d.skip_w:
+                    d.skip_w80 = t80(d._skip_w_tensor, d.skip_c1 + d.skip_c2)
         if ops.get_option("unet_conv_stream"):
             for d in descs:
                 M = d.B * d.H * d.W
diff --git a/minddiffusion_amd/ops.py b/minddiffusion_amd/ops.py
--- a/minddiffusion_amd/ops.py
+++ b/minddiffusion_amd/ops.py
@@ -16,6 +16,7 @@
             "unet_conv_stream": int(os.environ.get("MDX_UNET_CONV_STREAM", "128")),
             "gn_colstats_fold": int(os.environ.get("MDX_GN_COLSTATS_FOLD", "0")),
             "unet_gn_splitk_fuse": int(os.environ.get("MDX_UNET_GN_SPLITK_FUSE", "256")),
+            "unet_conv_t80": int(os.environ.get("MDX_UNET_CONV_T80", "1")),
             "unet_conv_stream_w4": int(os.environ.get("MDX_UNET_CONV_STREAM_W4", "0")),
             "unet_skip_fuse": int(os.environ.get("MDX_UNET_SKIP_FUSE", "1")),
             "unet_gn_conv_fuse": int(os.environ.get("MDX_UNET_GN_CONV_FUSE", "0")),
@@ -306,6 +307,23 @@
     return pack_frag_weight(conv_weight_k_order(w4d).to(f16)).reshape(-1)
 
 
+def pack_gemm_weight_t80(w2d):
+    N, K = w2d.shape
+    assert N % 80 == 0 and K % 64 == 0
+    dev = w2d.device
+    t = w2d.to(f16).view(N // 80, 80, K // 64, 8, 8).permute(0, 2, 1, 3, 4)
+    r = torch.arange(80, device=dev)
+    src = torch.arange(8, device=dev)[None, :] ^ ((r >> 1) & 7)[:, None]
+    idx = src[None, None, :, :, None].expand(N // 80, K // 64, 80, 8, 8)
+    return torch.gather(t, 3, idx).contiguous().view(-1)
+
+
+def pack_conv_weight_t80(w4d):
+    co, ci = w4d.shape[0], w4d.shape[1]
+    assert co % 80 == 0 and ci % 64 == 0
+    return pack_gemm_weight_t80(conv_weight_k_order(w4d).to(f16))
+
+
 def unpack_gemm_weight(packed, N, K):
     Np, Kp = (N + 63) // 64 * 64, (K + 63) // 64 * 64
     t = packed.view(Np // 64, Kp // 64, 64, 8, 8)
@@ -322,7 +340,7 @@
                    stats_out=None, ln_stats=None, ln_s=None, ln_eps=1e-5, tile_m=0, tile_n=0, colstats_out=None, stages=0,
                    w_frag=0, skip_a=None, skip_a2=None, skip_c1=0, skip_c2=0, skip_w=None, gn_colstats=None, gn_nrb=0,
                    gn_gamma=None, gn_beta=None, gn_eps=1e-5, gn_silu=1, w_sub=None, xattn_k=None, xattn_vt=None, xattn_len=0,
-                   xattn_cap=0, xattn_scale=0.0, act_slope=None):
+                   xattn_cap=0, xattn_scale=0.0, act_slope=None, w80=None, skip_w80=None):
     d = GemmDesc()
     d.a = a.data_ptr()
     d.a2 = 0 if a2 is None else a2.data_ptr()
@@ -363,6 +381,8 @@
     if xattn_k is not None:
         d.xattn_k, d.xattn_vt = xattn_k.data_ptr(), xattn_vt.data_ptr()
         d.xattn_len, d.xattn_cap, d.xattn_scale = int(xattn_len), int(xattn_cap), float(xattn_scale)
+    d.w80 = 0 if w80 is None else w80.data_ptr()
+    d.skip_w80 = 0 if skip_w80 is None else skip_w80.data_ptr()
     if act_slope is not None:
         d.act_slope, d.act_slope_n = act_slope.data_ptr(), int(act_slope.numel())
     return d
```

Result: no change. 5.326 latents/s (median of 4 runs) (-0.0%).
